# kepengxu/PGTFormer

Hardware: NVIDIA H100
Metric: clips_per_s (higher is better)
Workload: dtype bf16

## Files before the change

### include/pgt_b200.h

```cpp
#ifndef PGT_B200_H_
#define PGT_B200_H_

#include <stdint.h>

#ifdef __cplusplus
extern "C" {
#endif

typedef enum pgt_status {
  PGT_OK = 0,
  PGT_ERR_INVALID = -1,
  PGT_ERR_CUDA = -2,
  PGT_ERR_UNSUPPORTED = -3,
  PGT_ERR_DRIVER = -4
} pgt_status;

enum { PGT_BF16 = 0, PGT_F32 = 1 };
enum { PGT_ACT_NONE = 0, PGT_ACT_GELU = 1, PGT_ACT_SILU = 2, PGT_ACT_LRELU02 = 3, PGT_ACT_RELU = 4,
       PGT_ACT_SIGMOID = 5 };
enum { PGT_EPI_PLAIN = 0,
       PGT_EPI_SFT = 1 };
enum { PGT_OUT_NHWC = 0, PGT_OUT_NCHW = 1 };
enum { PGT_EPI_FLAG_RELU_AFTER_RESIDUAL = 1 };

typedef struct pgt_epilogue {
  const float* bias;
  int32_t act;
  int32_t mode;
  const void* residual;
  int32_t ldr;
  int32_t res_dtype;
  const void* aux;
  int32_t ldaux;
  float sft_w;
  void* out;
  int32_t ldo;
  int32_t out_dtype;
  int32_t out_layout;
  int32_t flags;
  float* gn_stats;
  const float* sft_wf;
} pgt_epilogue;

const char* pgt_strerror(int status);
const char* pgt_last_cuda_error(void);
int pgt_version(void);
int64_t pgt_launch_count(void);
void pgt_reset_launch_count(void);
void pgt_tmap_cache_stats(int64_t* hits, int64_t* misses);

enum { PGT_PROF_GEMM = 0, PGT_PROF_WINDOW_ATTN = 1, PGT_PROF_MHA = 2, PGT_PROF_ARGMAX = 3, PGT_PROF_ARGMIN = 4,
       PGT_PROF_NORM = 5, PGT_PROF_MOVE = 6, PGT_PROF_LAYERNORM = 7, PGT_PROF_CLASSES = 8 };
int pgt_profile_begin(void);
int pgt_profile_end(double* work, double* ms, int64_t* launches);
int pgt_profile_end_csv(const char* path, double* work, double* ms, int64_t* launches);

int pgt_linear_bf16(const void* A, int lda, const void* W, int ldw, int M, int N, int K,
                    const pgt_epilogue* ep, void* stream);

int pgt_conv_bf16(const void* x, int F, int Hin, int Win, int Cin, int ldx, const void* Wp, int ldw,
                  int Cout, int ksize, int stride, int pad_lo, const pgt_epilogue* ep, void* stream);

int pgt_conv_out_gn(const void* x, int F, int H, int W, int Cin, int ldx, const float* gn_ab, const void* Wp, int ldw,
                    int Cout, const float* bias, float* out, void* stream);
int pgt_conv_out_gn_act(const void* x, int F, int H, int W, int Cin, int ldx, const float* gn_ab, const void* Wp, int ldw,
                        int Cout, const float* bias, float* out, int silu, void* stream);

int pgt_conv_up2x_bf16(const void* x, int F, int Hin, int Win, int Cin, int ldx, const void* Wp4, int ldw,
                       int Cout, const pgt_epilogue* ep, void* stream);

int pgt_conv_rgb_bf16(const float* x_nchw, int F, int H, int W, int ksize, int stride, int pad, const float* mean3,
                      const float* std3, const void* Wp, int ldw, int Cout, const float* bias, int act, void* out,
                      int ldo, float* gn_stats, void* stream);

int64_t pgt_groupnorm_ws_floats(int F, int HW, int C);
int pgt_conv_tiles_per_frame(int Hin, int Win, int Cout, int ksize, int stride, int pad_lo);
int pgt_conv_tiles_exact(int Hin, int Win, int Cout, int ksize, int stride, int pad_lo);
int pgt_groupnorm_apply_stats(const void* x, int ldx, int F, int HW, int C, const float* gamma, const float* beta,
                              float eps, int apply_silu, void* y, int ldy, const float* stats, int chunks_per_frame,
                              float* ws, void* stream);

int pgt_groupnorm_ab(const void* x, int ldx, int F, int HW, int C, const float* gamma, const float* beta, float eps,
                     const float* stats, int chunks_per_frame, float* ws, float* ab, void* stream);
int pgt_groupnorm_silu(const void* x, int ldx, int F, int HW, int C, const float* gamma, const float* beta,
                       float eps, int apply_silu, void* y, int ldy, float* ws, void* stream);

int pgt_layernorm(const void* x, int ldx, int x_dtype, int T, int C, const float* gamma, const float* beta,
                  float eps, void* y, int ldy, const void* pos, int ldpos, void* y2, int ldy2, void* stream);

int pgt_ln_linear_bf16(const void* x, int ldx, int T, int C, const float* ln_g, const float* ln_b, float eps,
                       const void* W, int ldw, int N, const float* bias, void* out, int ldo, void* stream);

int pgt_swin_mlp_bf16(const void* x, int ldx, int T, int C, const float* ln_g, const float* ln_b, float eps,
                      const void* W1, const float* b1, const void* W2, const float* b2, void* out, int ldo,
                      float* gn_stats, void* stream);

int pgt_window_attention(const void* qkv, int ldqkv, int clips, int H, int W, int C, int heads, int shift,
                         const float* bias_tab, void* out, int ldo, void* stream);

int pgt_window_attention_tc(const void* qkv, int ldqkv, int clips, int H, int W, int C, int heads, int shift,
                            const void* tab, void* out, int ldo, void* stream);

int pgt_window3d_attention(const void* qkv, int ldqkv, const void* pad_qkv, int B, int D, int H, int W, int C, int heads,
                           int wd, int wh, int ww, int sd, int sh, int sw, const float* bias, void* out, int ldo,
                           void* stream);

int pgt_mha_fwd(const void* q, int ldq, const void* k, int ldk, const void* v, int ldv, int clips, int L,
                int heads, int d, void* out, int ldo, void* stream);

int pgt_argmax_gather(const float* logits, int T, int K, const float* codebook, int E, const int64_t* idx_in,
                      int64_t* idx, void* quant, int ldq, int quant_dtype, void* stream);
int pgt_l2_argmin(const float* z, int T, int E, const float* codebook, int K, int64_t* idx, float* quant,
                  void* stream);
int pgt_codebook_pack(const float* codebook, int K, int E, void* cb_bf16, float* cb_norm, void* stream);
int64_t pgt_l2_argmin_ws_ints(int T);
int pgt_l2_argmin_tc(const float* z, int T, int E, const float* codebook, const void* cb_bf16, const float* cb_norm,
                     int K, int64_t* idx, float* quant, int32_t* workspace, void* stream);
int64_t pgt_l2_argmin_split_ws_ints(int T, int splits);
int pgt_l2_argmin_tc_split(const float* z, int T, int E, const float* codebook, const void* cb_bf16, const float* cb_norm,
                           int K, int splits, int64_t* idx, float* quant, int32_t* workspace, void* stream);

int pgt_soft_codes(const float* z, int T, int E, const float* codebook, const float* cb_norm, int K, float temp,
                   float* out, int ldo, void* stream);
int pgt_sample_codes(const float* p, int T, int K, int ldp, const int64_t* seed, int64_t* idx, void* stream);

int pgt_rq_residual(const float* r_in, float* r_out, const int64_t* idx, int T, int E, const float* codebook_d,
                    float* agg, int first, void* stream);
int pgt_rq_embed(const int64_t* idx, long long ldi, long long ldd, int T, int d0, int d1, const float* codebooks,
                 long long cb_stride, int E, void* out, int ldo, int out_dtype, void* stream);

long long pgt_vq_stats_ws_doubles(int T, int E);
int pgt_vq_stats(const float* z, int T, int E, int HW, const float* codebook, int K, const int64_t* idx, float beta,
                 float* zq_nchw, void* zq_bf16, float* min_enc, float* scores, int* usage, int* hist, double* ws,
                 float* scalars, void* stream);

int pgt_adain(const void* q, int ldq, int q_dtype, const void* l, int ldl, int F, int HW, int C, float eps,
              void* y, int ldy, void* stream);
int pgt_adain_frames(const void* q, int ldq, int q_dtype, const void* l, int ldl, int F, int HW, int C, float eps,
                     const int32_t* flags, void* y, int ldy, void* stream);

int pgt_maxpool3x3s2(const void* x, int ldx, int F, int H, int W, int C, void* y, int ldy, void* stream);
int pgt_global_avgpool(const void* x, int ldx, int F, int HW, int C, void* y, int ldy, void* stream);
int pgt_channel_affine(const void* x, int ldx, int F, int HW, int C, const void* scale, int lds, int plus_one,
                       const void* addv, int ldv, const void* addm, int ldm, void* y, int ldy, void* stream);
int pgt_assemble_cond(const void* o0, int ld0, const void* o1, int ld1, const void* o2, int ld2, int F, int h8, int w8,
                      int h16, int w16, int ncls, void* cond, int ldc, void* stream);

int pgt_copy2d(const void* x, int ldx, int T, int C, void* y, int ldy, void* stream);
int pgt_regroup_frames(const void* x, int ldx, int clips, int P, int C, void* y, int ldy, int dir, void* stream);
int pgt_nchw_f32_to_nhwc_bf16(const float* x, int F, int C, int HW, const float* mean, const float* stdv, void* y,
                              int ldy, void* stream);
int pgt_nhwc_bf16_to_f32(const void* x, int ldx, int F, int HW, int C, float* y, int to_nchw, void* stream);

int pgt_u8hwc_to_f32nchw(const void* x_u8, int F, int H, int W, float* y, void* stream);
int pgt_u8hwc_resize_to_f32nchw(const void* x_u8, int F, int h, int w, const int32_t* sizes_dev, int H, int W, float* y,
                                void* stream);
int pgt_f32nchw_to_u8hwc(const float* x, int first, int step, int n, int H, int W, void* y_u8, void* stream);
int pgt_gather_frames(const void* x, long long frame_bytes, const int* idx_dev, int n, void* y, void* stream);
int pgt_scatter_frames(const void* x, long long frame_bytes, const int* idx_dev, int n, void* y, void* stream);

#ifdef __cplusplus
}
#endif
#endif
```

### pgtformer_b200/_lib.py

```python
import ctypes
import os
from ctypes import POINTER, Structure, c_char_p, c_float, c_int, c_int32, c_int64, c_void_p

HERE = os.path.dirname(os.path.abspath(__file__))
LIB_PATH = os.path.join(HERE, 'lib', 'libpgt_b200.so')

BF16, F32 = 0, 1
ACT_NONE, ACT_GELU, ACT_SILU, ACT_LRELU02, ACT_RELU, ACT_SIGMOID = 0, 1, 2, 3, 4, 5
EPI_PLAIN, EPI_SFT = 0, 1
OUT_NHWC, OUT_NCHW = 0, 1


class Epilogue(Structure):
    _fields_ = [('bias', c_void_p), ('act', c_int32), ('mode', c_int32), ('residual', c_void_p),
                ('ldr', c_int32), ('res_dtype', c_int32), ('aux', c_void_p), ('ldaux', c_int32),
                ('sft_w', c_float), ('out', c_void_p), ('ldo', c_int32), ('out_dtype', c_int32),
                ('out_layout', c_int32), ('flags', c_int32), ('gn_stats', c_void_p), ('sft_wf', c_void_p)]


SIGNATURES = {
    'pgt_strerror': (c_char_p, [c_int]),
    'pgt_last_cuda_error': (c_char_p, []),
    'pgt_version': (c_int, []),
    'pgt_launch_count': (c_int64, []),
    'pgt_reset_launch_count': (None, []),
    'pgt_tmap_cache_stats': (None, [c_void_p, c_void_p]),
    'pgt_profile_begin': (c_int, []),
    'pgt_profile_end': (c_int, [c_void_p, c_void_p, c_void_p]),
    'pgt_profile_end_csv': (c_int, [c_char_p, c_void_p, c_void_p, c_void_p]),
    'pgt_linear_bf16': (c_int, [c_void_p, c_int, c_void_p, c_int, c_int, c_int, c_int, POINTER(Epilogue), c_void_p]),
    'pgt_conv_bf16': (c_int, [c_void_p, c_int, c_int, c_int, c_int, c_int, c_void_p, c_int, c_int, c_int, c_int,
                              c_int, POINTER(Epilogue), c_void_p]),
    'pgt_conv_out_gn': (c_int, [c_void_p, c_int, c_int, c_int, c_int, c_int, c_void_p, c_void_p, c_int, c_int, c_void_p,
                                c_void_p, c_void_p]),
    'pgt_conv_out_gn_act': (c_int, [c_void_p, c_int, c_int, c_int, c_int, c_int, c_void_p, c_void_p, c_int, c_int,
                                    c_void_p, c_void_p, c_int, c_void_p]),
    'pgt_groupnorm_ab': (c_int, [c_void_p, c_int, c_int, c_int, c_int, c_void_p, c_void_p, c_float, c_void_p, c_int,
                                 c_void_p, c_void_p, c_void_p]),
    'pgt_conv_up2x_bf16': (c_int, [c_void_p, c_int, c_int, c_int, c_int, c_int, c_void_p, c_int, c_int,
                                   POINTER(Epilogue), c_void_p]),
    'pgt_conv_rgb_bf16': (c_int, [c_void_p, c_int, c_int, c_int, c_int, c_int, c_int, c_void_p, c_void_p, c_void_p, c_int,
                                  c_int, c_void_p, c_int, c_void_p, c_int, c_void_p, c_void_p]),
    'pgt_groupnorm_ws_floats': (c_int64, [c_int, c_int, c_int]),
    'pgt_conv_tiles_per_frame': (c_int, [c_int, c_int, c_int, c_int, c_int, c_int]),
    'pgt_conv_tiles_exact': (c_int, [c_int, c_int, c_int, c_int, c_int, c_int]),
    'pgt_groupnorm_apply_stats': (c_int, [c_void_p, c_int, c_int, c_int, c_int, c_void_p, c_void_p, c_float, c_int,
                                          c_void_p, c_int, c_void_p, c_int, c_void_p, c_void_p]),
    'pgt_groupnorm_silu': (c_int, [c_void_p, c_int, c_int, c_int, c_int, c_void_p, c_void_p, c_float, c_int,
                                   c_void_p, c_int, c_void_p, c_void_p]),
    'pgt_layernorm': (c_int, [c_void_p, c_int, c_int, c_int, c_int, c_void_p, c_void_p, c_float, c_void_p, c_int,
                              c_void_p, c_int, c_void_p, c_int, c_void_p]),
    'pgt_ln_linear_bf16': (c_int, [c_void_p, c_int, c_int, c_int, c_void_p, c_void_p, c_float, c_void_p, c_int, c_int,
                                   c_void_p, c_void_p, c_int, c_void_p]),
    'pgt_swin_mlp_bf16': (c_int, [c_void_p, c_int, c_int, c_int, c_void_p, c_void_p, c_float, c_void_p, c_void_p, c_void_p,
                                  c_void_p, c_void_p, c_int, c_void_p, c_void_p]),
    'pgt_window_attention': (c_int, [c_void_p, c_int, c_int, c_int, c_int, c_int, c_int, c_int, c_void_p, c_void_p,
                                     c_int, c_void_p]),
    'pgt_window_attention_tc': (c_int, [c_void_p, c_int, c_int, c_int, c_int, c_int, c_int, c_int, c_void_p, c_void_p,
                                        c_int, c_void_p]),
    'pgt_window3d_attention': (c_int, [c_void_p, c_int, c_void_p, c_int, c_int, c_int, c_int, c_int, c_int, c_int, c_int,
                                       c_int, c_int, c_int, c_int, c_void_p, c_void_p, c_int, c_void_p]),
    'pgt_mha_fwd': (c_int, [c_void_p, c_int, c_void_p, c_int, c_void_p, c_int, c_int, c_int, c_int, c_int, c_void_p,
                            c_int, c_void_p]),
    'pgt_argmax_gather': (c_int, [c_void_p, c_int, c_int, c_void_p, c_int, c_void_p, c_void_p, c_void_p, c_int,
                                  c_int, c_void_p]),
    'pgt_l2_argmin': (c_int, [c_void_p, c_int, c_int, c_void_p, c_int, c_void_p, c_void_p, c_void_p]),
    'pgt_codebook_pack': (c_int, [c_void_p, c_int, c_int, c_void_p, c_void_p, c_void_p]),
    'pgt_l2_argmin_ws_ints': (c_int64, [c_int]),
    'pgt_l2_argmin_tc': (c_int, [c_void_p, c_int, c_int, c_void_p, c_void_p, c_void_p, c_int, c_void_p, c_void_p,
                                 c_void_p, c_void_p]),
    'pgt_l2_argmin_split_ws_ints': (c_int64, [c_int, c_int]),
    'pgt_l2_argmin_tc_split': (c_int, [c_void_p, c_int, c_int, c_void_p, c_void_p, c_void_p, c_int, c_int, c_void_p,
                                       c_void_p, c_void_p, c_void_p]),
    'pgt_soft_codes': (c_int, [c_void_p, c_int, c_int, c_void_p, c_void_p, c_int, c_float, c_void_p, c_int, c_void_p]),
    'pgt_sample_codes': (c_int, [c_void_p, c_int, c_int, c_int, c_void_p, c_void_p, c_void_p]),
    'pgt_rq_residual': (c_int, [c_void_p, c_void_p, c_void_p, c_int, c_int, c_void_p, c_void_p, c_int, c_void_p]),
    'pgt_rq_embed': (c_int, [c_void_p, c_int64, c_int64, c_int, c_int, c_int, c_void_p, c_int64, c_int, c_void_p, c_int,
                             c_int, c_void_p]),
    'pgt_vq_stats_ws_doubles': (c_int64, [c_int, c_int]),
    'pgt_vq_stats': (c_int, [c_void_p, c_int, c_int, c_int, c_void_p, c_int, c_void_p, c_float, c_void_p, c_void_p,
                             c_void_p, c_void_p, c_void_p, c_void_p, c_void_p, c_void_p, c_void_p]),
    'pgt_adain': (c_int, [c_void_p, c_int, c_int, c_void_p, c_int, c_int, c_int, c_int, c_float, c_void_p, c_int,
                          c_void_p]),
    'pgt_adain_frames': (c_int, [c_void_p, c_int, c_int, c_void_p, c_int, c_int, c_int, c_int, c_float, c_void_p,
                                 c_void_p, c_int, c_void_p]),
    'pgt_maxpool3x3s2': (c_int, [c_void_p, c_int, c_int, c_int, c_int, c_int, c_void_p, c_int, c_void_p]),
    'pgt_global_avgpool': (c_int, [c_void_p, c_int, c_int, c_int, c_int, c_void_p, c_int, c_void_p]),
    'pgt_channel_affine': (c_int, [c_void_p, c_int, c_int, c_int, c_int, c_void_p, c_int, c_int, c_void_p, c_int,
                                   c_void_p, c_int, c_void_p, c_int, c_void_p]),
    'pgt_assemble_cond': (c_int, [c_void_p, c_int, c_void_p, c_int, c_void_p, c_int, c_int, c_int, c_int, c_int, c_int,
                                  c_int, c_void_p, c_int, c_void_p]),
    'pgt_u8hwc_to_f32nchw': (c_int, [c_void_p, c_int, c_int, c_int, c_void_p, c_void_p]),
    'pgt_u8hwc_resize_to_f32nchw': (c_int, [c_void_p, c_int, c_int, c_int, c_void_p, c_int, c_int, c_void_p,
                                            c_void_p]),
    'pgt_f32nchw_to_u8hwc': (c_int, [c_void_p, c_int, c_int, c_int, c_int, c_int, c_void_p, c_void_p]),
    'pgt_gather_frames': (c_int, [c_void_p, c_int64, c_void_p, c_int, c_void_p, c_void_p]),
    'pgt_scatter_frames': (c_int, [c_void_p, c_int64, c_void_p, c_int, c_void_p, c_void_p]),
    'pgt_copy2d': (c_int, [c_void_p, c_int, c_int, c_int, c_void_p, c_int, c_void_p]),
    'pgt_regroup_frames': (c_int, [c_void_p, c_int, c_int, c_int, c_int, c_void_p, c_int, c_int, c_void_p]),
    'pgt_nchw_f32_to_nhwc_bf16': (c_int, [c_void_p, c_int, c_int, c_int, c_void_p, c_void_p, c_void_p, c_int,
                                          c_void_p]),
    'pgt_nhwc_bf16_to_f32': (c_int, [c_void_p, c_int, c_int, c_int, c_int, c_void_p, c_int, c_void_p]),
}

_lib = None


def load(build_if_missing=True):
    global _lib
    if _lib is not None:
        return _lib
    if build_if_missing:
        from . import build as _build
        _build.build()
    if not os.path.exists(LIB_PATH):
        raise RuntimeError('libpgt_b200.so not built: run `python -m pgtformer_b200.build`')
    lib = ctypes.CDLL(LIB_PATH)
    for name, (res, args) in SIGNATURES.items():
        try:
            fn = getattr(lib, name)
        except AttributeError as e:
            raise RuntimeError('libpgt_b200.so does not export %s (stale build?)' % name) from e
        fn.restype = res
        fn.argtypes = args
    _lib = lib
    return lib


def check(status):
    if status != 0:
        lib = load()
        msg = lib.pgt_strerror(status).decode()
        if status == -2:
            msg += ': ' + lib.pgt_last_cuda_error().decode()
        raise RuntimeError('libpgt_b200: ' + msg)
```

### pgtformer_b200/csrc/gemm_tc.cu

```cuda
#include <cudaTypedefs.h>
#include <cstdio>
#include <cstdlib>

#include "common.cuh"
#include "tmap.cuh"
#include "ptx.cuh"
#include "epi_common.cuh"

namespace pgt {

constexpr int BM = 128;
constexpr int BK = 64;
constexpr int EPI_WARPS = 8;
constexpr int GEMM_THREADS = EPI_WARPS * 32 + 128;
constexpr int PRODUCER_WARP = EPI_WARPS;
constexpr int DMA_WARP = EPI_WARPS + 1;
constexpr int CONSUMER_REGS = 232;
constexpr int PRODUCER_REGS = 40;
static_assert(2 * 128 * CONSUMER_REGS + 128 * PRODUCER_REGS <= 65536, "register file");
constexpr int XCH_LD = 68;
constexpr int XCH_BYTES = BM * XCH_LD * 4;
constexpr int XCH_WG_LD = 36;
constexpr int XCH_WG_BYTES = BM * XCH_WG_LD * 4;
constexpr int EPI_BAR = 1;
constexpr int PP_XCH_BAR = 2;
constexpr int PP_MMA_BAR = 4;
constexpr int PP_EPI_BAR = 6;
constexpr int A_STAGE_BYTES = BM * BK * 2;
constexpr int PANEL_BYTES = BM * 128;
template <int BN>
constexpr int staging_slots() { return BN == 256 ? 2 : 4; }
constexpr int PREFETCH_TILES = 2;

enum { MODE_LINEAR = 0, MODE_CONV_S1 = 1, MODE_CONV_S2 = 2 };

struct GemmParams {
  int mode;
  int M, N, K;
  int num_kb, m_tiles, n_tiles;
  int F, H, W;
  int tw, th, tn, tiles_x, tiles_y;
  int cin_blocks, ksize, pad_lo, cin_ld;
  int pad_x, pad_y;
  long long o_sx, o_sy, o_sf;
  int b_resident;
  int fast_epi;
  int has_res_map;
  const float* bias;
  int act, epi_mode;
  float* gn_stats;
  int gn_cpg;
  int ntaps, tap_kw, tap_oy, tap_ox;
  int gn_tpf;
  int gn_fstride;
  int relu_after_res;
  const void* residual;
  int ldr, res_dtype;
  const void* aux;
  int ldaux;
  float sft_w;
  const float* sft_wf;
  void* out;
  int ldo, out_dtype, out_layout;
  double flops;
};

template <int BN>
struct GemmCfg {
  static constexpr int B_STAGE_BYTES = BN * BK * 2;
  static constexpr int STAGE_BYTES = A_STAGE_BYTES + B_STAGE_BYTES;
  static constexpr int SLOTS = staging_slots<BN>();
  static constexpr int STAGING_BYTES = SLOTS * PANEL_BYTES;
  static constexpr int BUDGET = 232448 - 1024  - STAGING_BYTES - XCH_BYTES - 256 ;
  static constexpr int STAGES = (BUDGET / STAGE_BYTES) > 6 ? 6 : (BUDGET / STAGE_BYTES);
  static constexpr int SMEM_BYTES = STAGES * STAGE_BYTES + STAGING_BYTES + XCH_BYTES + 256 + 1024;
  static_assert(SMEM_BYTES <= 232448, "gemm smem budget");
};

__device__ __forceinline__ void tile_mn(const GemmParams& p, int tile, int& m_blk, int& n_blk) {
  n_blk = tile % p.n_tiles;
  m_blk = tile / p.n_tiles;
}


__device__ __forceinline__ void decode_conv_tile(const GemmParams& p, int m_blk, int& n0, int& y0, int& x0) {
  const int tx = m_blk % p.tiles_x;
  const int t2 = m_blk / p.tiles_x;
  const int ty = t2 % p.tiles_y;
  const int tf = t2 / p.tiles_y;
  x0 = tx * p.tw;
  y0 = ty * p.th;
  n0 = tf * p.tn;
}

template <int N>
__device__ __forceinline__ void act_chunk(float (&f)[N], int act) {
  switch (act) {
    case PGT_ACT_GELU:
#pragma unroll
      for (int j = 0; j < N; ++j) f[j] = gelu_erf(f[j]);
      break;
    case PGT_ACT_SILU:
#pragma unroll
      for (int j = 0; j < N; ++j) f[j] = apply_act(f[j], PGT_ACT_SILU);
      break;
    case PGT_ACT_LRELU02:
#pragma unroll
      for (int j = 0; j < N; ++j) f[j] = fmaxf(f[j], 0.2f * f[j]);
      break;
    case PGT_ACT_RELU:
#pragma unroll
      for (int j = 0; j < N; ++j) f[j] = fmaxf(f[j], 0.f);
      break;
    case PGT_ACT_SIGMOID:
#pragma unroll
      for (int j = 0; j < N; ++j) f[j] = apply_act(f[j], PGT_ACT_SIGMOID);
      break;
    default: break;
  }
}

struct EpiCtx {
  uint8_t* staging;
  float* xch;
  uint64_t* res_bar;
  uint64_t* slot_ready;
};

__device__ __forceinline__ uint4 lds128(uint32_t a) {
  uint4 u;
  asm volatile("ld.shared.v4.b32 {%0, %1, %2, %3}, [%4];" : "=r"(u.x), "=r"(u.y), "=r"(u.z), "=r"(u.w) : "r"(a) : "memory");
  return u;
}
__device__ __forceinline__ void sts128(uint32_t a, const uint4& u) {
  asm volatile("st.shared.v4.b32 [%0], {%1, %2, %3, %4};" ::"r"(a), "r"(u.x), "r"(u.y), "r"(u.z), "r"(u.w) : "memory");
}

__device__ __forceinline__ float sft_weight(const GemmParams& p, int m_blk, int r) {
  if (p.sft_wf == nullptr) return p.sft_w;
  const int f = m_blk / (p.tiles_x * p.tiles_y) * p.tn + r / (p.tw * p.th);
  return __ldg(p.sft_wf + min(f, p.F - 1));
}

template <bool kSft>
__device__ __forceinline__ void epi_finish(const GemmParams& p, const uint32_t (&v)[32], const float* bias32, uint32_t srow,
                                           int r, int sub, int esize, bool has_res, float* gq, int gcol,
                                           const float4 (&pre)[8], bool use_pre, float sw = 0.f) {
  float f[32];
  if (use_pre) {
#pragma unroll
    for (int q = 0; q < 8; ++q) {
      f[4 * q + 0] = __uint_as_float(v[4 * q + 0]) + pre[q].x;
      f[4 * q + 1] = __uint_as_float(v[4 * q + 1]) + pre[q].y;
      f[4 * q + 2] = __uint_as_float(v[4 * q + 2]) + pre[q].z;
      f[4 * q + 3] = __uint_as_float(v[4 * q + 3]) + pre[q].w;
    }
  } else if (bias32 != nullptr) {
    const float4* b4 = reinterpret_cast<const float4*>(bias32);
#pragma unroll
    for (int q = 0; q < 8; ++q) {
      const float4 bb = __ldg(b4 + q);
      f[4 * q + 0] = __uint_as_float(v[4 * q + 0]) + bb.x;
      f[4 * q + 1] = __uint_as_float(v[4 * q + 1]) + bb.y;
      f[4 * q + 2] = __uint_as_float(v[4 * q + 2]) + bb.z;
      f[4 * q + 3] = __uint_as_float(v[4 * q + 3]) + bb.w;
    }
  } else {
#pragma unroll
    for (int i = 0; i < 32; ++i) f[i] = __uint_as_float(v[i]);
    if (p.bias != nullptr) {
#pragma unroll
      for (int i = 0; i < 32; ++i)
        if (gcol + i < p.N) f[i] += __ldg(p.bias + gcol + i);
    }
  }
  if (p.act != PGT_ACT_NONE && !p.relu_after_res) act_chunk(f, p.act);
  if (esize == 2) {
    uint32_t off[4];
#pragma unroll
    for (int q = 0; q < 4; ++q) off[q] = srow + ((((sub << 2) + q) ^ (r & 7)) << 4);
    if (has_res) {
      uint4 ur[4];
#pragma unroll
      for (int q = 0; q < 4; ++q) ur[q] = lds128(off[q]);
      if (kSft) {
        uint4 ux[4];
#pragma unroll
        for (int q = 0; q < 4; ++q) ux[q] = lds128(off[q] + PANEL_BYTES);
#pragma unroll
        for (int q = 0; q < 4; ++q) {
          const float2 a = unpack_bf16x2(ur[q].x), b = unpack_bf16x2(ur[q].y), c = unpack_bf16x2(ur[q].z), d = unpack_bf16x2(ur[q].w);
          const float rr[8] = {a.x, a.y, b.x, b.y, c.x, c.y, d.x, d.y};
          const float2 sa = unpack_bf16x2(ux[q].x), sb = unpack_bf16x2(ux[q].y), sc = unpack_bf16x2(ux[q].z), sd = unpack_bf16x2(ux[q].w);
          const float ss[8] = {sa.x, sa.y, sb.x, sb.y, sc.x, sc.y, sd.x, sd.y};
#pragma unroll
          for (int e = 0; e < 8; ++e) f[8 * q + e] = rr[e] + sw * (rr[e] * ss[e] + f[8 * q + e]);
        }
      } else {
#pragma unroll
        for (int q = 0; q < 4; ++q) {
          const float2 a = unpack_bf16x2(ur[q].x), b = unpack_bf16x2(ur[q].y), c = unpack_bf16x2(ur[q].z), d = unpack_bf16x2(ur[q].w);
          f[8 * q + 0] += a.x; f[8 * q + 1] += a.y; f[8 * q + 2] += b.x; f[8 * q + 3] += b.y;
          f[8 * q + 4] += c.x; f[8 * q + 5] += c.y; f[8 * q + 6] += d.x; f[8 * q + 7] += d.y;
        }
      }
    }
    if (p.relu_after_res) {
#pragma unroll
      for (int e = 0; e < 32; ++e) f[e] = fmaxf(f[e], 0.f);
    }
#pragma unroll
    for (int q = 0; q < 4; ++q) {
      uint4 o;
      o.x = pack_bf16x2(f[8 * q + 0], f[8 * q + 1]);
      o.y = pack_bf16x2(f[8 * q + 2], f[8 * q + 3]);
      o.z = pack_bf16x2(f[8 * q + 4], f[8 * q + 5]);
      o.w = pack_bf16x2(f[8 * q + 6], f[8 * q + 7]);
      sts128(off[q], o);
    }
    if (gq != nullptr) {
      const int lane = lane_id();
      switch (p.gn_cpg) {
        case 2: gn_chunk_stats<2>(f, gq, 0, lane); break;
        case 4: gn_chunk_stats<4>(f, gq, 0, lane); break;
        case 8: gn_chunk_stats<8>(f, gq, 0, lane); break;
        case 16: gn_chunk_stats<16>(f, gq, 0, lane); break;
        default: gn_chunk_stats<32>(f, gq, 0, lane); break;
      }
    }
  } else {
    if (has_res) {
      uint4 ur[8];
#pragma unroll
      for (int q = 0; q < 8; ++q) ur[q] = lds128(srow + ((q ^ (r & 7)) << 4));
#pragma unroll
      for (int q = 0; q < 8; ++q) {
        f[4 * q + 0] += __uint_as_float(ur[q].x); f[4 * q + 1] += __uint_as_float(ur[q].y);
        f[4 * q + 2] += __uint_as_float(ur[q].z); f[4 * q + 3] += __uint_as_float(ur[q].w);
      }
    }
    if (p.relu_after_res) {
#pragma unroll
      for (int e = 0; e < 32; ++e) f[e] = fmaxf(f[e], 0.f);
    }
#pragma unroll
    for (int q = 0; q < 8; ++q) {
      uint4 o;
      o.x = __float_as_uint(f[4 * q]); o.y = __float_as_uint(f[4 * q + 1]);
      o.z = __float_as_uint(f[4 * q + 2]); o.w = __float_as_uint(f[4 * q + 3]);
      sts128(srow + ((q ^ (r & 7)) << 4), o);
    }
  }
}

struct ItemCursor {
  int tile, pnl;
};

template <int BN>
struct ItemStream {
  const GemmParams& p;
  int num_tiles, PW, panels_total;
  __device__ ItemStream(const GemmParams& pp, int nt) : p(pp), num_tiles(nt) {
    PW = 128 / (pp.out_dtype == PGT_BF16 ? 2 : 4);
    panels_total = BN / PW;
  }
  __device__ int panels_in_tile(int t) const {
    int mb, nb;
    tile_mn(p, t, mb, nb);
    const int cb = nb * BN;
    const int n = (p.N - cb + PW - 1) / PW;
    return n > panels_total ? panels_total : n;
  }
  __device__ bool valid(const ItemCursor& c) const { return c.tile < num_tiles; }
  __device__ void next(ItemCursor& c) const {
    if (++c.pnl >= panels_in_tile(c.tile)) { c.tile += gridDim.x; c.pnl = 0; }
  }
};

template <int BN>
__device__ __forceinline__ void epilogue_dma_loop(const GemmParams& p, const EpiCtx& ctx, const CUtensorMap& tmO,
                                                  const CUtensorMap& tmR, const CUtensorMap& tmX, int lane, int num_tiles) {
  if (!p.fast_epi) return;
  const ItemStream<BN> is(p, num_tiles);
  constexpr int SLOTS = staging_slots<BN>();
  static_assert(SLOTS == 4 || SLOTS == 2, "ring positions are computed with shifts");
  const bool sft = SLOTS == 4 && p.epi_mode == PGT_EPI_SFT;
  const int S = sft ? 2 : 1;
  const int R = SLOTS / S;
  auto coords = [&](const ItemCursor& c, int& col, int& m_blk, int& n0, int& y0, int& x0) {
    int nb;
    tile_mn(p, c.tile, m_blk, nb);
    col = nb * BN + c.pnl * is.PW;
    n0 = y0 = x0 = 0;
    if (p.mode != MODE_LINEAR) decode_conv_tile(p, m_blk, n0, y0, x0);
  };
  auto prepare = [&](const ItemCursor& c, int pos) {
    uint64_t* bar = &ctx.res_bar[pos];
    if (!p.has_res_map) { mbar_arrive(bar); return; }
    int col, m_blk, n0, y0, x0;
    coords(c, col, m_blk, n0, y0, x0);
    uint8_t* dst = ctx.staging + pos * S * PANEL_BYTES;
    mbar_arrive_expect_tx(bar, S * PANEL_BYTES);
    if (p.mode == MODE_LINEAR) {
      tma_load_2d(dst, &tmR, bar, col, m_blk * BM);
      if (sft) tma_load_2d(dst + PANEL_BYTES, &tmX, bar, col, m_blk * BM);
    } else {
      tma_load_4d(dst, &tmR, bar, col, x0, y0, n0);
      if (sft) tma_load_4d(dst + PANEL_BYTES, &tmX, bar, col, x0, y0, n0);
    }
  };
  ItemCursor cp{(int)blockIdx.x, 0}, cs{(int)blockIdx.x, 0};
  if (lane == 0) {
    for (int i = 0; i < R && is.valid(cp); ++i) { prepare(cp, i); is.next(cp); }
  }
  __syncwarp();
  const int rshift = R == 4 ? 2 : 1;
  for (int k = 0; is.valid(cs); ++k, is.next(cs)) {
    const int pos = k & (R - 1);
    mbar_wait(&ctx.slot_ready[pos], (k >> rshift) & 1);
    if (lane == 0) {
      int col, m_blk, n0, y0, x0;
      coords(cs, col, m_blk, n0, y0, x0);
      const uint8_t* src = ctx.staging + pos * S * PANEL_BYTES;
      if (p.mode == MODE_LINEAR) tma_store_2d(&tmO, src, col, m_blk * BM);
      else tma_store_4d(&tmO, src, col, x0, y0, n0);
      bulk_commit();
      if (k >= 1 && is.valid(cp)) {
        bulk_wait_read<1>();
        prepare(cp, (k - 1) & (R - 1));
        is.next(cp);
      }
    }
    __syncwarp();
  }
  if (lane == 0) bulk_wait0();
}

struct DirectRow {
  bool valid;
  long long orow;
  int pn, py, px;
};

__device__ __forceinline__ DirectRow direct_row(const GemmParams& p, int m_blk, int r) {
  DirectRow d{false, 0, 0, 0, 0};
  if (p.mode == MODE_LINEAR) {
    d.orow = (long long)m_blk * BM + r;
    d.valid = d.orow < p.M;
  } else {
    int n0, y0, x0;
    decode_conv_tile(p, m_blk, n0, y0, x0);
    const int ix = r % p.tw;
    const int t2 = r / p.tw;
    const int iy = t2 % p.th;
    const int in = t2 / p.th;
    d.pn = n0 + in; d.py = y0 + iy; d.px = x0 + ix;
    d.valid = (d.pn < p.F) && (d.py < p.H) && (d.px < p.W);
    d.orow = ((long long)d.pn * p.H + d.py) * p.W + d.px;
  }
  return d;
}

template <bool kVec>
__device__ __forceinline__ void epi_direct16(const GemmParams& p, const DirectRow& d, const float* xs, int col0) {
  const int ncol = min(16, p.N - col0);
  const long long orow = d.orow;
  float f[16];
#pragma unroll
  for (int j = 0; j < 16; ++j) f[j] = xs[j] + ((p.bias != nullptr && j < ncol) ? __ldg(p.bias + col0 + j) : 0.f);
  if (p.act != PGT_ACT_NONE && !p.relu_after_res) act_chunk(f, p.act);
  if (p.residual != nullptr) {
    if (p.res_dtype == PGT_BF16) {
      const __nv_bfloat16* rp = reinterpret_cast<const __nv_bfloat16*>(p.residual) + orow * p.ldr + col0;
      float rr[16];
#pragma unroll
      for (int j = 0; j < 16; ++j) rr[j] = (j < ncol) ? __bfloat162float(rp[j]) : 0.f;
      if (p.epi_mode == PGT_EPI_SFT) {
        const __nv_bfloat16* ap = reinterpret_cast<const __nv_bfloat16*>(p.aux) + orow * p.ldaux + col0;
        const float sw = p.sft_wf != nullptr ? __ldg(p.sft_wf + d.pn) : p.sft_w;
#pragma unroll
        for (int j = 0; j < 16; ++j) {
          const float sc = (j < ncol) ? __bfloat162float(ap[j]) : 0.f;
          f[j] = rr[j] + sw * (rr[j] * sc + f[j]);
        }
      } else {
#pragma unroll
        for (int j = 0; j < 16; ++j) f[j] += rr[j];
      }
    } else {
      const float* rp = reinterpret_cast<const float*>(p.residual) + orow * p.ldr + col0;
#pragma unroll
      for (int j = 0; j < 16; ++j)
        if (j < ncol) f[j] += __ldg(rp + j);
    }
  }
  if (p.relu_after_res) act_chunk(f, PGT_ACT_RELU);
  if (p.out_layout == PGT_OUT_NCHW) {
    float* op = reinterpret_cast<float*>(p.out);
#pragma unroll
    for (int j = 0; j < 16; ++j)
      if (j < ncol) op[(((long long)d.pn * p.N + (col0 + j)) * p.H + d.py) * p.W + d.px] = f[j];
  } else if (p.out_dtype == PGT_BF16) {
    __nv_bfloat16* op = reinterpret_cast<__nv_bfloat16*>(p.out) + orow * p.ldo + col0;
    if (kVec && ncol == 16 && ((p.ldo & 7) == 0)) {
#pragma unroll
      for (int q = 0; q < 2; ++q) {
        uint4 u;
        u.x = pack_bf16x2(f[q * 8 + 0], f[q * 8 + 1]);
        u.y = pack_bf16x2(f[q * 8 + 2], f[q * 8 + 3]);
        u.z = pack_bf16x2(f[q * 8 + 4], f[q * 8 + 5]);
        u.w = pack_bf16x2(f[q * 8 + 6], f[q * 8 + 7]);
        reinterpret_cast<uint4*>(op)[q] = u;
      }
    } else {
#pragma unroll
      for (int j = 0; j < 16; ++j)
        if (j < ncol) op[j] = __float2bfloat16_rn(f[j]);
    }
  } else {
    float* op = reinterpret_cast<float*>(p.out) + orow * p.ldo + col0;
#pragma unroll
    for (int j = 0; j < 16; ++j)
      if (j < ncol) op[j] = f[j];
  }
}

__device__ __forceinline__ float* gn_stats_ptr(const GemmParams& p, int m_blk, int quad, int col0) {
  if (p.gn_stats == nullptr) return nullptr;
  const size_t chunk = p.gn_tpf > 0 ? (size_t)(m_blk / p.gn_tpf) * p.gn_fstride + (m_blk % p.gn_tpf) * 4 + quad
                                    : (size_t)m_blk * 4 + quad;
  return p.gn_stats + (chunk * 32 + col0 / p.gn_cpg) * 2;
}

template <int BN, bool kVec>
__device__ __forceinline__ void epilogue_tile(const GemmParams& p, const EpiCtx& ctx, int warp, int lane, int tile, int& k,
                                              const float (&acc)[BN / 2]) {
  const int quad = warp & 3;
  const int half = warp >> 2;
  const int r = quad * 32 + lane;
  const int esize = (p.out_dtype == PGT_BF16) ? 2 : 4;
  const ItemStream<BN> is(p, 0);
  const int PW = is.PW;
  const int nsub = PW / 32;
  constexpr int SLOTS = staging_slots<BN>();
  constexpr int SLOT_SHIFT = SLOTS == 4 ? 2 : 1;
  const bool sft = SLOTS == 4 && p.epi_mode == PGT_EPI_SFT;
  const bool bias_vec = kVec && p.bias != nullptr && (p.N % 32) == 0;
  const float* xrow = ctx.xch + r * XCH_LD;

  int n_blk, m_blk;
  tile_mn(p, tile, m_blk, n_blk);
  const int col_base = n_blk * BN;
  const int npan = p.fast_epi ? is.panels_in_tile(tile) : 0;
  const uint32_t stg = smem_u32(ctx.staging) + r * 128;
  auto gn_ptr = [&](int col0) -> float* { return gn_stats_ptr(p, m_blk, quad, col0); };
  const DirectRow drow = p.fast_epi ? DirectRow{false, 0, 0, 0, 0} : direct_row(p, m_blk, r);

  static_for<0, BN / 64>([&](auto gc) {
    constexpr int g = decltype(gc)::value;
    if (col_base + g * 64 >= p.N) return;
    named_bar_sync(EPI_BAR, EPI_WARPS * 32);
    acc_to_smem<g * 64, 64>(acc, ctx.xch + half * 64 * XCH_LD, XCH_LD, quad, lane);
    named_bar_sync(EPI_BAR, EPI_WARPS * 32);

    if (p.fast_epi) {
      if (sft) {
        const int pnl = g;
        if (pnl < npan) {
          const int pos = k & 1;
          mbar_wait_spin(&ctx.res_bar[pos], (k >> 1) & 1);
          const int col0 = col_base + pnl * PW + half * 32;
          uint32_t v[32];
          smem_row_32(xrow + half * 32, v);
          float4 nb[8];
          epi_finish<true>(p, v, bias_vec ? p.bias + col0 : nullptr, stg + pos * 2 * PANEL_BYTES, r, half, esize, true,
                           gn_ptr(col0), col0, nb, false, sft_weight(p, m_blk, r));
          fence_proxy_async();
          mbar_arrive(&ctx.slot_ready[pos]);
          ++k;
        }
      } else {
        for (int pp = 0; pp < 64 / PW; ++pp) {
          const int pnl = g * (64 / PW) + pp;
          if (pnl >= npan) break;
          const int pos = k & (SLOTS - 1);
          const bool mine = (nsub == 2) || ((pnl & 1) == half);
          const int sb = (nsub == 2) ? half : 0;
          const int col0 = col_base + pnl * PW + sb * 32;
          float4 b[8];
          const bool pre = BN < 256 && bias_vec;
          if (mine && pre) {
            const float4* gb = reinterpret_cast<const float4*>(p.bias + col0);
#pragma unroll
            for (int q = 0; q < 8; ++q) b[q] = __ldg(gb + q);
          }
          mbar_wait_spin(&ctx.res_bar[pos], (k >> SLOT_SHIFT) & 1);
          if (mine) {
            uint32_t v[32];
            smem_row_32(xrow + pnl * PW + sb * 32 - g * 64, v);
            epi_finish<false>(p, v, bias_vec && !pre ? p.bias + col0 : nullptr, stg + pos * PANEL_BYTES, r, sb, esize,
                              p.has_res_map != 0, gn_ptr(col0), col0, b, pre);
          }
          fence_proxy_async();
          mbar_arrive(&ctx.slot_ready[pos]);
          ++k;
        }
      }
    } else {
      const int c0 = g * 64 + half * 32;
      if (drow.valid) {
#pragma unroll 1
        for (int sc16 = 0; sc16 < 32; sc16 += 16) {
          const int col0 = col_base + c0 + sc16;
          if (col0 >= p.N) break;
          epi_direct16<kVec>(p, drow, xrow + half * 32 + sc16, col0);
        }
      }
      __syncwarp();
    }
  });
}

template <int BN, bool kVec>
__device__ __forceinline__ void epilogue_tile_wg(const GemmParams& p, const EpiCtx& ctx, int wq, int bar, int tile, int k,
                                                 const float (&acc)[2][BN / 2]) {
  const int lane = lane_id();
  const int r = wq * 32 + lane;
  const int esize = (p.out_dtype == PGT_BF16) ? 2 : 4;
  const ItemStream<BN> is(p, 0);
  const int nsub = is.PW / 32;
  constexpr int SLOTS = staging_slots<BN>();
  constexpr int SLOT_SHIFT = SLOTS == 4 ? 2 : 1;
  const bool sft = SLOTS == 4 && p.epi_mode == PGT_EPI_SFT;
  const bool bias_vec = kVec && p.bias != nullptr && (p.N % 32) == 0;
  const float* xrow = ctx.xch + r * XCH_WG_LD;

  int n_blk, m_blk;
  tile_mn(p, tile, m_blk, n_blk);
  const int col_base = n_blk * BN;
  const int npan = p.fast_epi ? is.panels_in_tile(tile) : 0;
  const uint32_t stg = smem_u32(ctx.staging) + r * 128;
  const DirectRow drow = p.fast_epi ? DirectRow{false, 0, 0, 0, 0} : direct_row(p, m_blk, r);

  static_for<0, BN / 32>([&](auto cc) {
    constexpr int c = decltype(cc)::value;
    const int pnl = c / nsub, sub = c - pnl * nsub;
    if (p.fast_epi && pnl >= npan) return;
    const int col0 = col_base + c * 32;
    if (col0 < p.N) {
      named_bar_sync(bar, 128);
      acc_to_smem<c * 32, 32>(acc[0], ctx.xch, XCH_WG_LD, wq, lane);
      acc_to_smem<c * 32, 32>(acc[1], ctx.xch + 64 * XCH_WG_LD, XCH_WG_LD, wq, lane);
      named_bar_sync(bar, 128);
    }
    if (p.fast_epi) {
      const int item = k + pnl;
      const int pos = sft ? (item & 1) : (item & (SLOTS - 1));
      if (sub == 0) mbar_wait_spin(&ctx.res_bar[pos], sft ? ((item >> 1) & 1) : ((item >> SLOT_SHIFT) & 1));
      if (col0 < p.N) {
        uint32_t v[32];
        smem_row_32(xrow, v);
        float4 nb[8];
        if (sft)
          epi_finish<true>(p, v, bias_vec ? p.bias + col0 : nullptr, stg + pos * 2 * PANEL_BYTES, r, sub, esize, true,
                           gn_stats_ptr(p, m_blk, wq, col0), col0, nb, false, sft_weight(p, m_blk, r));
        else
          epi_finish<false>(p, v, bias_vec ? p.bias + col0 : nullptr, stg + pos * PANEL_BYTES, r, sub, esize,
                            p.has_res_map != 0, gn_stats_ptr(p, m_blk, wq, col0), col0, nb, false);
      }
      if (sub == nsub - 1) {
        fence_proxy_async();
        mbar_arrive(&ctx.slot_ready[pos]);
      }
    } else if (col0 < p.N) {
      if (drow.valid) {
#pragma unroll 1
        for (int sc16 = 0; sc16 < 32; sc16 += 16) {
          if (col0 + sc16 >= p.N) break;
          epi_direct16<kVec>(p, drow, xrow + sc16, col0 + sc16);
        }
      }
      __syncwarp();
    }
  });
}

__device__ __forceinline__ void release_stage(uint64_t* bar, int lane) {
  __syncwarp();
  if (lane == 0) mbar_arrive(bar);
}

template <int BN, bool kVec>
__global__ void __launch_bounds__(GEMM_THREADS, 1)
gemm_tc_kernel(const __grid_constant__ CUtensorMap tmA, const __grid_constant__ CUtensorMap tmB,
               const __grid_constant__ CUtensorMap tmO, const __grid_constant__ CUtensorMap tmR,
               const __grid_constant__ CUtensorMap tmX, const GemmParams p) {
  using Cfg = GemmCfg<BN>;
  constexpr int STAGES = Cfg::STAGES;
  extern __shared__ uint8_t smem_raw[];
  uint8_t* smem = reinterpret_cast<uint8_t*>((reinterpret_cast<uintptr_t>(smem_raw) + 1023) & ~uintptr_t(1023));
  uint8_t* smem_a = smem;
  uint8_t* smem_b = smem + STAGES * A_STAGE_BYTES;
  uint8_t* staging = smem + STAGES * Cfg::STAGE_BYTES;
  float* xch = reinterpret_cast<float*>(staging + Cfg::STAGING_BYTES);
  uint64_t* bars = reinterpret_cast<uint64_t*>(staging + Cfg::STAGING_BYTES + XCH_BYTES);
  uint64_t* full_bar = bars;
  uint64_t* empty_bar = bars + STAGES;
  uint64_t* res_bar = bars + 2 * STAGES;
  uint64_t* slot_ready = res_bar + Cfg::SLOTS;

  const int warp = threadIdx.x >> 5;
  const int lane = threadIdx.x & 31;
  const int num_tiles = p.m_tiles * p.n_tiles;

  if (warp == PRODUCER_WARP && lane == 0) {
    tma_prefetch_desc(&tmA);
    tma_prefetch_desc(&tmB);
    if (p.fast_epi) tma_prefetch_desc(&tmO);
    if (p.has_res_map) tma_prefetch_desc(&tmR);
    if (p.fast_epi && p.epi_mode == PGT_EPI_SFT) tma_prefetch_desc(&tmX);
    for (int i = 0; i < STAGES; ++i) {
      mbar_init(&full_bar[i], 1);
      mbar_init(&empty_bar[i], EPI_WARPS);
    }
    for (int i = 0; i < Cfg::SLOTS; ++i) {
      mbar_init(&res_bar[i], 1);
      mbar_init(&slot_ready[i], EPI_WARPS * 32);
    }
    fence_barrier_init();
  }
  __syncthreads();

  if (warp >= EPI_WARPS) {
    setmaxnreg_dec<PRODUCER_REGS>();
    if (warp == PRODUCER_WARP) {
      int stage = 0;
      uint32_t phase = 0;
      for (int tile = blockIdx.x; tile < num_tiles; tile += gridDim.x) {
        int n_blk, m_blk;
        tile_mn(p, tile, m_blk, n_blk);
        int n0 = 0, y0 = 0, x0 = 0;
        if (p.mode != MODE_LINEAR) decode_conv_tile(p, m_blk, n0, y0, x0);
        for (int kb = 0; kb < p.num_kb; ++kb) {
          mbar_wait(&empty_bar[stage], phase ^ 1);
          if (elect_one()) {
            void* dst_a = smem_a + stage * A_STAGE_BYTES;
            void* dst_b = smem_b + stage * Cfg::B_STAGE_BYTES;
            int cb = 0, ax = 0, ay = 0, a5 = 0;
            if (p.mode != MODE_LINEAR) {
              const int tap = kb / p.cin_blocks;
              cb = kb - tap * p.cin_blocks;
              const int dy = tap / p.ksize;
              const int dx = tap - dy * p.ksize;
              if (p.mode == MODE_CONV_S1) {
                ax = x0 + dx - p.pad_x; ay = y0 + dy - p.pad_y;
              } else {
                const int oy = dy - p.pad_lo, ox = dx - p.pad_lo;
                const int qy = (oy < 0) ? -((1 - oy) >> 1) : (oy >> 1);
                const int qx = (ox < 0) ? -((1 - ox) >> 1) : (ox >> 1);
                const int py = oy - 2 * qy, px = ox - 2 * qx;
                cb = px * p.cin_ld + cb * BK;
                ax = x0 + qx; ay = y0 + qy; a5 = py;
              }
            }
            mbar_arrive_expect_tx(&full_bar[stage], Cfg::STAGE_BYTES);
            if (p.mode == MODE_LINEAR) tma_load_2d(dst_a, &tmA, &full_bar[stage], kb * BK, m_blk * BM);
            else if (p.mode == MODE_CONV_S1) tma_load_4d(dst_a, &tmA, &full_bar[stage], cb * BK, ax, ay, n0);
            else tma_load_5d(dst_a, &tmA, &full_bar[stage], cb, ax, a5, ay, n0);
            tma_load_2d(dst_b, &tmB, &full_bar[stage], kb * BK, n_blk * BN);
          }
          __syncwarp();
          if (++stage == STAGES) { stage = 0; phase ^= 1; }
        }
      }
      for (int i = 0; i < STAGES; ++i) {
        mbar_wait(&empty_bar[stage], phase ^ 1);
        if (++stage == STAGES) { stage = 0; phase ^= 1; }
      }
    } else if (warp == DMA_WARP) {
      const EpiCtx ctx{staging, xch, res_bar, slot_ready};
      epilogue_dma_loop<BN>(p, ctx, tmO, tmR, tmX, lane, num_tiles);
    }
  } else {
    setmaxnreg_inc<CONSUMER_REGS>();
    const EpiCtx ctx{staging, xch, res_bar, slot_ready};
    const int wg = warp >> 2;
    const uint32_t a_rows = smem_u32(smem_a) + wg * 64 * 128;
    const uint32_t b_base = smem_u32(smem_b);
    int stage = 0;
    uint32_t phase = 0;
    int k = 0;
    for (int tile = blockIdx.x; tile < num_tiles; tile += gridDim.x) {
      float acc[BN / 2];
      int prev = -1;
      for (int kb = 0; kb < p.num_kb; ++kb) {
        mbar_wait_spin(&full_bar[stage], phase);
        const uint64_t da = wgmma_desc_k_sw128(a_rows + stage * A_STAGE_BYTES);
        const uint64_t db = wgmma_desc_k_sw128(b_base + stage * Cfg::B_STAGE_BYTES);
        wgmma_fence();
#pragma unroll
        for (int kk = 0; kk < BK / 16; ++kk)
          wgmma_bf16<BN>(acc, da + 2 * kk, db + 2 * kk, (kb | kk) != 0 ? 1u : 0u);
        wgmma_commit();
        wgmma_wait<1>();
        if (prev >= 0) release_stage(&empty_bar[prev], lane);
        prev = stage;
        if (++stage == STAGES) { stage = 0; phase ^= 1; }
      }
      wgmma_wait<0>();
      release_stage(&empty_bar[prev], lane);
      epilogue_tile<BN, kVec>(p, ctx, warp, lane, tile, k, acc);
    }
  }
}


constexpr int HALO_TW = 8, HALO_TH = 16;
constexpr int HALO_PITCH = (HALO_TW + 2) * 128;
constexpr int HALO_A_BYTES = (HALO_TH + 2) * HALO_PITCH;
constexpr int HALO_A_STRIDE = ((HALO_A_BYTES + 1023) / 1024) * 1024;

template <int BN>
struct HaloCfg {
  static constexpr int B_BYTES = BN * 128;
  static constexpr int A_STAGES = 2;
  static constexpr int B_STAGES = (BN == 64) ? 9 : 4;
  static constexpr int SLOTS = staging_slots<BN>();
  static constexpr int STAGING_BYTES = SLOTS * PANEL_BYTES;
  static constexpr int XCH = 2 * XCH_WG_BYTES;
  static constexpr int SMEM_BYTES = A_STAGES * HALO_A_STRIDE + B_STAGES * B_BYTES + STAGING_BYTES + XCH + 512 + 1024;
  static_assert(SMEM_BYTES <= 232448, "halo conv smem budget");
};

template <int S>
__device__ __forceinline__ void ring_skip(int& s, uint32_t& ph, int n) {
  const int t = s + n;
  ph ^= (uint32_t)(t / S) & 1u;
  s = t % S;
}

template <int BN, bool kVec>
__global__ void __launch_bounds__(GEMM_THREADS, 1)
conv_halo_kernel(const __grid_constant__ CUtensorMap tmA, const __grid_constant__ CUtensorMap tmB,
                 const __grid_constant__ CUtensorMap tmO, const __grid_constant__ CUtensorMap tmR,
                 const __grid_constant__ CUtensorMap tmX, const GemmParams p) {
  using Cfg = HaloCfg<BN>;
  constexpr int AS = Cfg::A_STAGES, BS = Cfg::B_STAGES;
  constexpr int RELEASERS = 4;
  extern __shared__ uint8_t smem_raw[];
  uint8_t* smem = reinterpret_cast<uint8_t*>((reinterpret_cast<uintptr_t>(smem_raw) + 1023) & ~uintptr_t(1023));
  uint8_t* smem_a = smem;
  uint8_t* smem_b = smem + AS * HALO_A_STRIDE;
  uint8_t* staging = smem_b + BS * Cfg::B_BYTES;
  float* xch = reinterpret_cast<float*>(staging + Cfg::STAGING_BYTES);
  uint64_t* bars = reinterpret_cast<uint64_t*>(staging + Cfg::STAGING_BYTES + Cfg::XCH);
  uint64_t* a_full = bars;
  uint64_t* a_empty = bars + AS;
  uint64_t* b_full = bars + 2 * AS;
  uint64_t* b_empty = bars + 2 * AS + BS;
  uint64_t* res_bar = bars + 2 * AS + 2 * BS;
  uint64_t* slot_ready = res_bar + Cfg::SLOTS;

  const int warp = threadIdx.x >> 5;
  const int lane = threadIdx.x & 31;
  const int num_tiles = p.m_tiles * p.n_tiles;
  const int cin_pad = p.cin_blocks * BK;

  if (warp == PRODUCER_WARP && lane == 0) {
    tma_prefetch_desc(&tmA);
    tma_prefetch_desc(&tmB);
    if (p.fast_epi) tma_prefetch_desc(&tmO);
    if (p.has_res_map) tma_prefetch_desc(&tmR);
    if (p.fast_epi && p.epi_mode == PGT_EPI_SFT) tma_prefetch_desc(&tmX);
    for (int i = 0; i < AS; ++i) { mbar_init(&a_full[i], 1); mbar_init(&a_empty[i], RELEASERS); }
    for (int i = 0; i < BS; ++i) { mbar_init(&b_full[i], 1); mbar_init(&b_empty[i], RELEASERS); }
    for (int i = 0; i < Cfg::SLOTS; ++i) {
      mbar_init(&res_bar[i], 1);
      mbar_init(&slot_ready[i], RELEASERS * 32);
    }
    fence_barrier_init();
  }
  __syncthreads();

  if (warp >= EPI_WARPS) {
    setmaxnreg_dec<PRODUCER_REGS>();
    if (warp == PRODUCER_WARP) {
      int as = 0, bs = 0;
      uint32_t aph = 0, bph = 0;
      for (int tile = blockIdx.x; tile < num_tiles; tile += gridDim.x) {
        const int n_blk = tile % p.n_tiles;
        const int m_blk = tile / p.n_tiles;
        int n0, y0, x0;
        decode_conv_tile(p, m_blk, n0, y0, x0);
        {
          const int pt = tile + PREFETCH_TILES * (int)gridDim.x;
          if (BN == 64 && pt < num_tiles && elect_one()) {
            int pn0, py0, px0;
            decode_conv_tile(p, pt / p.n_tiles, pn0, py0, px0);
            for (int cb = 0; cb < p.cin_blocks; ++cb) tma_prefetch_4d(&tmA, cb * BK, px0 - 1, py0 - 1, pn0);
            if (p.has_res_map) {
              const int c0 = (pt % p.n_tiles) * BN;
              const int rw = p.out_dtype == PGT_BF16 ? 64 : 32;
              for (int c = 0; c < BN && c0 + c < p.N; c += rw) {
                tma_prefetch_4d(&tmR, c0 + c, px0, py0, pn0);
                if (p.epi_mode == PGT_EPI_SFT) tma_prefetch_4d(&tmX, c0 + c, px0, py0, pn0);
              }
            }
          }
          __syncwarp();
        }
        for (int cb = 0; cb < p.cin_blocks; ++cb) {
          mbar_wait(&a_empty[as], aph ^ 1);
          if (elect_one()) {
            mbar_arrive_expect_tx(&a_full[as], HALO_A_BYTES);
            tma_load_4d(smem_a + as * HALO_A_STRIDE, &tmA, &a_full[as], cb * BK, x0 - 1, y0 - 1, n0);
          }
          __syncwarp();
          if (++as == AS) { as = 0; aph ^= 1; }
          if (p.b_resident && tile != (int)blockIdx.x) continue;
          for (int t = 0; t < p.ntaps; ++t) {
            mbar_wait(&b_empty[bs], bph ^ 1);
            if (elect_one()) {
              mbar_arrive_expect_tx(&b_full[bs], Cfg::B_BYTES);
              tma_load_2d(smem_b + bs * Cfg::B_BYTES, &tmB, &b_full[bs], t * cin_pad + cb * BK, n_blk * BN);
            }
            __syncwarp();
            if (++bs == BS) { bs = 0; bph ^= 1; }
          }
        }
      }
      for (int i = 0; i < AS; ++i) {
        mbar_wait(&a_empty[as], aph ^ 1);
        if (++as == AS) { as = 0; aph ^= 1; }
      }
    } else if (warp == DMA_WARP) {
      const EpiCtx ctx{staging, xch, res_bar, slot_ready};
      epilogue_dma_loop<BN>(p, ctx, tmO, tmR, tmX, lane, num_tiles);
    }
  } else {
    setmaxnreg_inc<CONSUMER_REGS>();
    const int wg = warp >> 2;
    const EpiCtx ctx{staging, xch + wg * (XCH_WG_BYTES / 4), res_bar, slot_ready};
    const uint32_t a_base = smem_u32(smem_a);
    const uint32_t b_base = smem_u32(smem_b);
    constexpr uint64_t ROW_BLOCK = 8 * HALO_PITCH / 16;
    const ItemStream<BN> is(p, num_tiles);
    const int b_per_tile = p.b_resident ? 0 : p.ntaps * p.cin_blocks;
    int as = 0, bs = 0;
    uint32_t aph = 0, bph = 0;
    int k = 0;
    bool first = true;
    for (int tile = blockIdx.x, j = 0; tile < num_tiles; tile += gridDim.x, ++j) {
      const bool has_next = tile + (int)gridDim.x < num_tiles;
      const int items = p.fast_epi ? is.panels_in_tile(tile) : 0;
      if ((j & 1) != wg) {
        ring_skip<AS>(as, aph, p.cin_blocks);
        ring_skip<BS>(bs, bph, b_per_tile);
        k += items;
        continue;
      }
      if (j > 0) named_bar_sync(PP_MMA_BAR + wg, 256);
      float acc[2][BN / 2];
      for (int cb = 0; cb < p.cin_blocks; ++cb) {
        const bool hand_over = has_next && cb == p.cin_blocks - 1;
        mbar_wait_spin(&a_full[as], aph);
        const uint64_t da0 = wgmma_desc_k_sw128(a_base + as * HALO_A_STRIDE, HALO_PITCH);
        auto tap_desc = [&](int t) -> uint64_t {
          const int dy = t / p.tap_kw, dx = t - dy * p.tap_kw;
          return da0 + (uint64_t)(((dy + p.tap_oy) * (HALO_TW + 2) + dx + p.tap_ox) * 8);
        };
        if (p.b_resident && first) {
          for (int t = 0; t < p.ntaps * p.cin_blocks; ++t) mbar_wait_spin(&b_full[t], 0);
          first = false;
        }
        int prev = -1;
        for (int t = 0; t < p.ntaps; ++t) {
          int bst = cb * p.ntaps + t;
          if (!p.b_resident) {
            mbar_wait_spin(&b_full[bs], bph);
            bst = bs;
          }
          const uint64_t da = tap_desc(t);
          const uint64_t db = wgmma_desc_k_sw128(b_base + bst * Cfg::B_BYTES);
          wgmma_fence();
#pragma unroll
          for (int kk = 0; kk < BK / 16; ++kk) {
            const uint32_t accum = (cb | t | kk) != 0 ? 1u : 0u;
            wgmma_bf16<BN>(acc[0], da + 2 * kk, db + 2 * kk, accum);
            wgmma_bf16<BN>(acc[1], da + ROW_BLOCK + 2 * kk, db + 2 * kk, accum);
          }
          wgmma_commit();
          if (hand_over && t == p.ntaps - 1) named_bar_arrive(PP_MMA_BAR + (wg ^ 1), 256);
          wgmma_wait<1>();
          if (!p.b_resident) {
            if (prev >= 0) release_stage(&b_empty[prev], lane);
            prev = bs;
            if (++bs == BS) { bs = 0; bph ^= 1; }
          }
        }
        wgmma_wait<0>();
        if (!p.b_resident) release_stage(&b_empty[prev], lane);
        release_stage(&a_empty[as], lane);
        if (++as == AS) { as = 0; aph ^= 1; }
      }
      if (j > 0) named_bar_sync(PP_EPI_BAR + wg, 256);
      epilogue_tile_wg<BN, kVec>(p, ctx, warp & 3, PP_XCH_BAR + wg, tile, k, acc);
      if (has_next) named_bar_arrive(PP_EPI_BAR + (wg ^ 1), 256);
      k += items;
    }
  }
}

static int encode_map(CUtensorMap* map, const void* base, int rank, const uint64_t* dims, const uint64_t* strides_bytes,
                      const uint32_t* box, int dtype = PGT_BF16) {
  return tmap_encode(map, base, rank, dims, strides_bytes, box, dtype);
}

static inline bool aligned16(const void* p) { return (reinterpret_cast<uintptr_t>(p) & 15) == 0; }

static int encode_out_map(CUtensorMap* map, const GemmParams& p, const void* base, int ld, int dtype) {
  const int esize = dtype == PGT_BF16 ? 2 : 4;
  const uint32_t pw = 128 / esize;
  if (p.mode == MODE_LINEAR) {
    uint64_t dims[2] = {(uint64_t)p.N, (uint64_t)p.M};
    uint64_t str[1] = {(uint64_t)ld * esize};
    uint32_t box[2] = {pw, BM};
    return encode_map(map, base, 2, dims, str, box, dtype);
  }
  uint64_t dims[4] = {(uint64_t)p.N, (uint64_t)p.W, (uint64_t)p.H, (uint64_t)p.F};
  uint64_t str[3] = {(uint64_t)ld * esize, (uint64_t)p.W * ld * esize, (uint64_t)p.H * p.W * ld * esize};
  if (p.o_sx != 0 && base == p.out) {
    str[0] = (uint64_t)p.o_sx * esize; str[1] = (uint64_t)p.o_sy * esize; str[2] = (uint64_t)p.o_sf * esize;
  }
  uint32_t box[4] = {pw, (uint32_t)p.tw, (uint32_t)p.th, (uint32_t)p.tn};
  return encode_map(map, base, 4, dims, str, box, dtype);
}

static int setup_epilogue_maps(GemmParams& p, const CUtensorMap& placeholder, CUtensorMap& tmO, CUtensorMap& tmR,
                               CUtensorMap& tmX) {
  const int esize = p.out_dtype == PGT_BF16 ? 2 : 4;
  p.fast_epi = (p.out_layout == PGT_OUT_NHWC && aligned16(p.out) && ((long long)p.ldo * esize) % 16 == 0) ? 1 : 0;
  if (p.epi_mode == PGT_EPI_SFT &&
      !(p.out_dtype == PGT_BF16 && aligned16(p.aux) && ((long long)p.ldaux * 2) % 16 == 0 && p.o_sx == 0))
    p.fast_epi = 0;
  p.has_res_map = 0;
  if (p.fast_epi && p.residual != nullptr) {
    if (p.res_dtype == p.out_dtype && aligned16(p.residual) && ((long long)p.ldr * esize) % 16 == 0) p.has_res_map = 1;
    else p.fast_epi = 0;
  }
  if (p.gn_stats != nullptr) {
    const int cpg = p.N / 32;
    const bool ok = p.fast_epi && p.out_dtype == PGT_BF16 && (p.N % 32) == 0 &&
                    (cpg == 2 || cpg == 4 || cpg == 8 || cpg == 16 || cpg == 32) &&
                    (p.mode == MODE_LINEAR || p.tn == 1);
    if (!ok) return PGT_ERR_UNSUPPORTED;
    p.gn_cpg = cpg;
  }
  tmO = placeholder;
  tmR = placeholder;
  tmX = placeholder;
  if (p.fast_epi) {
    int rc = encode_out_map(&tmO, p, p.out, p.ldo, p.out_dtype);
    if (rc != PGT_OK) return rc;
    if (p.has_res_map) {
      rc = encode_out_map(&tmR, p, p.residual, p.ldr, p.res_dtype);
      if (rc != PGT_OK) return rc;
    }
    if (p.epi_mode == PGT_EPI_SFT) {
      if (!p.has_res_map) { p.fast_epi = 0; return p.gn_stats ? PGT_ERR_UNSUPPORTED : PGT_OK; }
      rc = encode_out_map(&tmX, p, p.aux, p.ldaux, PGT_BF16);
      if (rc != PGT_OK) return rc;
    }
  }
  return PGT_OK;
}

static bool vector_views(const GemmParams& p) {
  if (p.bias != nullptr && (p.N % 32) == 0 && !aligned16(p.bias)) return false;
  if (!p.fast_epi && p.out_layout == PGT_OUT_NHWC && p.out_dtype == PGT_BF16 && (p.ldo % 8) == 0 && !aligned16(p.out))
    return false;
  return true;
}

template <int BN, bool kVec>
static cudaError_t gemm_smem_once() {
  static PerDeviceOnce once;
  return once.run([] {
    return cudaFuncSetAttribute(gemm_tc_kernel<BN, kVec>, cudaFuncAttributeMaxDynamicSharedMemorySize, GemmCfg<BN>::SMEM_BYTES);
  });
}

template <int BN, bool kVec>
static cudaError_t halo_smem_once() {
  static PerDeviceOnce once;
  return once.run([] {
    return cudaFuncSetAttribute(conv_halo_kernel<BN, kVec>, cudaFuncAttributeMaxDynamicSharedMemorySize, HaloCfg<BN>::SMEM_BYTES);
  });
}

static int encode_weight_map(CUtensorMap* tmB, const void* W, int ldw, int K, int N, int BN) {
  uint64_t dims[2] = {(uint64_t)K, (uint64_t)N};
  uint64_t str[1] = {(uint64_t)ldw * 2};
  uint32_t box[2] = {BK, (uint32_t)BN};
  return encode_map(tmB, W, 2, dims, str, box);
}

template <int BN>
static int launch_gemm(const CUtensorMap& tmA, const void* W, int ldw, GemmParams& p, cudaStream_t stream) {
  using Cfg = GemmCfg<BN>;
  static_assert(Cfg::STAGES >= 3, "pipeline too shallow");
  CUtensorMap tmB, tmO, tmR, tmX;
  int rc = encode_weight_map(&tmB, W, ldw, p.K, p.N, BN);
  if (rc != PGT_OK) return rc;
  rc = setup_epilogue_maps(p, tmA, tmO, tmR, tmX);
  if (rc != PGT_OK) return rc;
  p.n_tiles = ceil_div(p.N, BN);
  const bool vec = vector_views(p);
  PGT_CUDA_OK((vec ? gemm_smem_once<BN, true>() : gemm_smem_once<BN, false>()));
  const int tiles = p.m_tiles * p.n_tiles;
  const int grid = tiles < num_sms() ? tiles : num_sms();
  {
    char desc[96];
    if (prof_enabled()) {
      if (p.mode == MODE_LINEAR) snprintf(desc, sizeof(desc), "linear M%d N%d K%d BN%d e%d", p.M, p.N, p.K, BN, p.fast_epi);
      else snprintf(desc, sizeof(desc), "conv%d s%d F%d H%d W%d K%d N%d BN%d t%dx%dx%d e%d", p.ksize, p.mode, p.F, p.H, p.W, p.K, p.N, BN, p.tn, p.th, p.tw, p.fast_epi);
    }
    ProfScope ps(PGT_PROF_GEMM, p.flops, stream, desc);
    if (vec) gemm_tc_kernel<BN, true><<<grid, GEMM_THREADS, Cfg::SMEM_BYTES, stream>>>(tmA, tmB, tmO, tmR, tmX, p);
    else gemm_tc_kernel<BN, false><<<grid, GEMM_THREADS, Cfg::SMEM_BYTES, stream>>>(tmA, tmB, tmO, tmR, tmX, p);
  }
  PGT_LAUNCH_OK();
  return PGT_OK;
}

template <int BN>
static int launch_halo(const CUtensorMap& tmA, const void* W, int ldw, GemmParams& p, cudaStream_t stream) {
  using Cfg = HaloCfg<BN>;
  CUtensorMap tmB, tmO, tmR, tmX;
  int rc = encode_weight_map(&tmB, W, ldw, p.K, p.N, BN);
  if (rc != PGT_OK) return rc;
  rc = setup_epilogue_maps(p, tmA, tmO, tmR, tmX);
  if (rc != PGT_OK) return rc;
  p.n_tiles = ceil_div(p.N, BN);
  p.b_resident = (p.ntaps * p.cin_blocks <= Cfg::B_STAGES && p.n_tiles == 1) ? 1 : 0;
  const bool vec = vector_views(p);
  PGT_CUDA_OK((vec ? halo_smem_once<BN, true>() : halo_smem_once<BN, false>()));
  const int tiles = p.m_tiles * p.n_tiles;
  const int grid = tiles < num_sms() ? tiles : num_sms();
  {
    char desc[96];
    if (prof_enabled())
      snprintf(desc, sizeof(desc), "halo3 F%d H%d W%d K%d N%d BN%d e%d r%d", p.F, p.H, p.W, p.K, p.N, BN, p.fast_epi,
               p.b_resident);
    ProfScope ps(PGT_PROF_GEMM, p.flops, stream, desc);
    if (vec) conv_halo_kernel<BN, true><<<grid, GEMM_THREADS, Cfg::SMEM_BYTES, stream>>>(tmA, tmB, tmO, tmR, tmX, p);
    else conv_halo_kernel<BN, false><<<grid, GEMM_THREADS, Cfg::SMEM_BYTES, stream>>>(tmA, tmB, tmO, tmR, tmX, p);
  }
  PGT_LAUNCH_OK();
  return PGT_OK;
}

static bool wide_tiles(const GemmParams& p) {
  if (p.N <= 128 || p.num_kb < 8 || p.epi_mode == PGT_EPI_SFT) return false;
  if (ceil_div(p.N, 256) * 256 > ceil_div(p.N, 128) * 128) return false;
  return p.m_tiles * ceil_div(p.N, 256) >= num_sms();
}

static int dispatch_gemm(const CUtensorMap& tmA, const void* W, int ldw, GemmParams& p, cudaStream_t stream) {
  if (p.N <= 64) return launch_gemm<64>(tmA, W, ldw, p, stream);
  if (wide_tiles(p)) return launch_gemm<256>(tmA, W, ldw, p, stream);
  return launch_gemm<128>(tmA, W, ldw, p, stream);
}

static int fill_epilogue(GemmParams& p, const pgt_epilogue* ep) {
  if (ep == nullptr || ep->out == nullptr) return PGT_ERR_INVALID;
  p.bias = ep->bias;
  p.act = ep->act;
  p.epi_mode = ep->mode;
  p.residual = ep->residual;
  p.ldr = ep->ldr;
  p.res_dtype = ep->res_dtype;
  p.aux = ep->aux;
  p.ldaux = ep->ldaux;
  p.sft_w = ep->sft_w;
  p.sft_wf = ep->mode == PGT_EPI_SFT ? ep->sft_wf : nullptr;
  p.out = ep->out;
  p.ldo = ep->ldo;
  p.out_dtype = ep->out_dtype;
  p.out_layout = ep->out_layout;
  p.relu_after_res = (ep->flags & PGT_EPI_FLAG_RELU_AFTER_RESIDUAL) ? 1 : 0;
  p.gn_stats = ep->gn_stats;
  p.gn_cpg = 0;
  if (p.relu_after_res && (p.act != PGT_ACT_RELU || p.epi_mode != PGT_EPI_PLAIN)) return PGT_ERR_INVALID;
  if (p.epi_mode == PGT_EPI_SFT && (p.residual == nullptr || p.aux == nullptr || p.res_dtype != PGT_BF16))
    return PGT_ERR_INVALID;
  if (p.sft_wf != nullptr && p.mode == MODE_LINEAR) return PGT_ERR_INVALID;
  if (p.out_layout == PGT_OUT_NCHW && (p.out_dtype != PGT_F32 || p.mode == MODE_LINEAR)) return PGT_ERR_INVALID;
  return PGT_OK;
}

}

using namespace pgt;

extern "C" int pgt_linear_bf16(const void* A, int lda, const void* W, int ldw, int M, int N, int K,
                               const pgt_epilogue* ep, void* stream) {
  PGT_CHECK_ARG(A && W && M > 0 && N > 0 && K > 0);
  PGT_CHECK_ARG((lda % 8) == 0 && (ldw % 8) == 0 && aligned16(A) && aligned16(W));
  GemmParams p{};
  p.mode = MODE_LINEAR;
  p.M = M; p.N = N; p.K = K;
  p.num_kb = ceil_div(K, BK);
  p.m_tiles = ceil_div(M, BM);
  p.flops = 2.0 * M * (double)N * K;
  int rc = fill_epilogue(p, ep);
  if (rc != PGT_OK) return rc;
  CUtensorMap tmA;
  uint64_t dims[2] = {(uint64_t)K, (uint64_t)M};
  uint64_t str[1] = {(uint64_t)lda * 2};
  uint32_t box[2] = {BK, BM};
  rc = encode_map(&tmA, A, 2, dims, str, box);
  if (rc != PGT_OK) return rc;
  return dispatch_gemm(tmA, W, ldw, p, static_cast<cudaStream_t>(stream));
}

static bool conv_tile_shape(int Hin, int Win, int Cout, int ksize, int stride, int pad_lo, int& tw, int& th) {
  static const bool no_halo = getenv("PGT_NO_HALO") != nullptr;
  const int H = Hin / stride, W = Win / stride;
  const bool halo = !no_halo && stride == 1 && ((ksize == 3 && pad_lo == 1) || ksize == 2) && Cout <= 128 && Hin >= HALO_TH &&
                    Win >= HALO_TW;
  tw = 1; th = 1;
  if (halo) { tw = HALO_TW; th = HALO_TH; }
  else {
    while (tw * 2 <= W && tw * 2 <= BM) tw *= 2;
    while (th * 2 <= H && tw * th * 2 <= BM) th *= 2;
  }
  return halo;
}

static int conv_impl(const void* x, int F, int Hin, int Win, int Cin, int ldx, const void* Wp, int ldw, int Cout,
                     int ksize, int stride, int pad_y, int pad_x, int up_phase, const pgt_epilogue* ep, void* stream) {
  const int pad_lo = pad_y;
  PGT_CHECK_ARG(x && Wp && F > 0 && Hin > 0 && Win > 0 && Cin > 0 && Cout > 0);
  PGT_CHECK_ARG((ksize >= 1 && ksize <= 3) && (stride == 1 || stride == 2) && pad_y >= 0 && pad_y <= 1 && pad_x >= 0 && pad_x <= 1);
  PGT_CHECK_ARG(stride == 1 || (ksize != 2 && pad_x == pad_y));
  PGT_CHECK_ARG((ldx % 8) == 0 && (ldw % 8) == 0 && aligned16(x) && aligned16(Wp) && ldx >= Cin);
  const int cin_pad = ceil_div(Cin, BK) * BK;
  PGT_CHECK_ARG(ldw >= ksize * ksize * cin_pad);
  GemmParams p{};
  p.N = Cout;
  p.ksize = ksize;
  p.pad_lo = pad_lo;
  p.pad_x = pad_x; p.pad_y = pad_y;
  p.cin_blocks = cin_pad / BK;
  p.K = ksize * ksize * cin_pad;
  p.num_kb = ksize * ksize * p.cin_blocks;
  p.F = F;
  CUtensorMap tmA;
  int rc;
  if (stride == 1) {
    p.mode = MODE_CONV_S1;
    p.H = Hin; p.W = Win;
  } else {
    if ((Hin & 1) || (Win & 1) || (Cin % BK) != 0 || ldx < Cin) return PGT_ERR_UNSUPPORTED;
    p.mode = MODE_CONV_S2;
    p.H = Hin / 2; p.W = Win / 2;
    p.cin_ld = ldx;
  }
  rc = fill_epilogue(p, ep);
  if (rc != PGT_OK) return rc;
  if (up_phase >= 0) {
    if (stride != 1 || p.out_layout != PGT_OUT_NHWC || p.epi_mode != PGT_EPI_PLAIN || p.residual != nullptr)
      return PGT_ERR_UNSUPPORTED;
    const int py = up_phase >> 1, px = up_phase & 1;
    const int esz = p.out_dtype == PGT_BF16 ? 2 : 4;
    const long long Wo = 2LL * Win;
    p.out = static_cast<char*>(p.out) + ((long long)py * Wo + px) * p.ldo * esz;
    p.o_sx = 2LL * p.ldo; p.o_sy = 2LL * Wo * p.ldo; p.o_sf = 4LL * Hin * Win * p.ldo;
  }
  int tw, th;
  const bool halo = conv_tile_shape(Hin, Win, Cout, ksize, stride, pad_y, tw, th);
  p.ntaps = ksize * ksize; p.tap_kw = ksize;
  p.tap_oy = up_phase >= 0 ? (up_phase >> 1) : 0;
  p.tap_ox = up_phase >= 0 ? (up_phase & 1) : 0;
  const int tn = BM / (tw * th);
  p.tw = tw; p.th = th; p.tn = tn;
  p.tiles_x = ceil_div(p.W, tw);
  p.tiles_y = ceil_div(p.H, th);
  p.m_tiles = p.tiles_x * p.tiles_y * ceil_div(F, tn);
  p.M = F * p.H * p.W;
  p.flops = 2.0 * p.M * (double)Cout * (ksize * ksize * Cin);
  if (up_phase >= 0 && p.gn_stats != nullptr) {
    if (tn != 1) return PGT_ERR_UNSUPPORTED;
    const int tpf = p.tiles_x * p.tiles_y;
    p.gn_tpf = tpf;
    p.gn_fstride = 16 * tpf;
    p.gn_stats += (size_t)up_phase * tpf * 4 * 64;
  }
  if (p.mode == MODE_CONV_S1) {
    uint64_t dims[4] = {(uint64_t)Cin, (uint64_t)Win, (uint64_t)Hin, (uint64_t)F};
    uint64_t str[3] = {(uint64_t)ldx * 2, (uint64_t)Win * ldx * 2, (uint64_t)Hin * Win * ldx * 2};
    uint32_t box[4] = {BK, (uint32_t)(halo ? tw + 2 : tw), (uint32_t)(halo ? th + 2 : th), (uint32_t)tn};
    rc = encode_map(&tmA, x, 4, dims, str, box);
    if (rc == PGT_OK && halo) {
      cudaStream_t st = static_cast<cudaStream_t>(stream);
      return Cout <= 64 ? launch_halo<64>(tmA, Wp, ldw, p, st) : launch_halo<128>(tmA, Wp, ldw, p, st);
    }
  } else {
    uint64_t dims[5] = {(uint64_t)2 * ldx, (uint64_t)Win / 2, 2, (uint64_t)Hin / 2, (uint64_t)F};
    uint64_t str[4] = {(uint64_t)2 * ldx * 2, (uint64_t)Win * ldx * 2, (uint64_t)2 * Win * ldx * 2,
                       (uint64_t)Hin * Win * ldx * 2};
    uint32_t box[5] = {BK, (uint32_t)tw, 1, (uint32_t)th, (uint32_t)tn};
    rc = encode_map(&tmA, x, 5, dims, str, box);
  }
  if (rc != PGT_OK) return rc;
  if (up_phase >= 0) {
    const int esz = p.out_dtype == PGT_BF16 ? 2 : 4;
    if (!aligned16(p.out) || ((long long)p.ldo * esz) % 16 != 0) return PGT_ERR_UNSUPPORTED;
  }
  return dispatch_gemm(tmA, Wp, ldw, p, static_cast<cudaStream_t>(stream));
}

extern "C" int pgt_conv_tiles_per_frame(int Hin, int Win, int Cout, int ksize, int stride, int pad_lo) {
  int tw, th;
  conv_tile_shape(Hin, Win, Cout, ksize, stride, pad_lo, tw, th);
  if (tw * th != BM) return 0;
  return ceil_div(Win / stride, tw) * ceil_div(Hin / stride, th);
}

extern "C" int pgt_conv_tiles_exact(int Hin, int Win, int Cout, int ksize, int stride, int pad_lo) {
  int tw, th;
  conv_tile_shape(Hin, Win, Cout, ksize, stride, pad_lo, tw, th);
  if (tw * th != BM) return 0;
  const int H = Hin / stride, W = Win / stride;
  return (W % tw == 0 && H % th == 0) ? (W / tw) * (H / th) : 0;
}

extern "C" int pgt_conv_bf16(const void* x, int F, int Hin, int Win, int Cin, int ldx, const void* Wp, int ldw,
                             int Cout, int ksize, int stride, int pad_lo, const pgt_epilogue* ep, void* stream) {
  PGT_CHECK_ARG(ksize == 1 || ksize == 3);
  return conv_impl(x, F, Hin, Win, Cin, ldx, Wp, ldw, Cout, ksize, stride, pad_lo, pad_lo, -1, ep, stream);
}

extern "C" int pgt_conv_up2x_bf16(const void* x, int F, int Hin, int Win, int Cin, int ldx, const void* Wp4, int ldw,
                                  int Cout, const pgt_epilogue* ep, void* stream) {
  PGT_CHECK_ARG(Wp4 != nullptr && ldw > 0);
  const int cin_pad = ceil_div(Cin, BK) * BK;
  PGT_CHECK_ARG(ldw >= 4 * cin_pad);
  for (int ph = 0; ph < 4; ++ph) {
    const int py = ph >> 1, px = ph & 1;
    const void* w = static_cast<const char*>(Wp4) + (size_t)ph * Cout * ldw * 2;
    int rc = conv_impl(x, F, Hin, Win, Cin, ldx, w, ldw, Cout, 2, 1, 1 - py, 1 - px, ph, ep, stream);
    if (rc != PGT_OK) return rc;
  }
  return PGT_OK;
}
```

### pgtformer_b200/engine.py

```python
import torch
import torch.nn.functional as F

from . import ops
from .spec import Arch
from .swin3d import pack_blocks

BF = torch.bfloat16


def _on_device(fn):
    import functools

    @functools.wraps(fn)
    def wrapper(self, *a, **k):
        with torch.cuda.device(self.dev):
            return fn(self, *a, **k)
    return wrapper


def _fusing(feats, wgt):
    return feats is not None and (torch.is_tensor(wgt) or wgt > 0)


def _pack_conv(w):
    co, ci, kh, kw = w.shape
    cp = (ci + 63) // 64 * 64
    wp = torch.zeros(co, kh * kw, cp, dtype=torch.float32, device=w.device)
    wp[:, :, :ci] = w.permute(0, 2, 3, 1).reshape(co, kh * kw, ci)
    return wp.reshape(co, kh * kw * cp).to(BF).contiguous()


def fold_layernorm_affine(weight, bias, gamma, beta):
    wf = weight.float()
    return wf * gamma.float()[None, :], (bias.float() + wf @ beta.float()).contiguous()


def _pack_up2x(w):
    co, ci, _, _ = w.shape
    cp = (ci + 63) // 64 * 64
    sets = {0: ((0,), (1, 2)), 1: ((0, 1), (2,))}
    out = torch.zeros(4, co, 4, cp, dtype=torch.float32, device=w.device)
    for py in range(2):
        for px in range(2):
            for ty in range(2):
                for tx in range(2):
                    acc = torch.zeros(co, ci, dtype=torch.float32, device=w.device)
                    for dy in sets[py][ty]:
                        for dx in sets[px][tx]:
                            acc += w[:, :, dy, dx]
                    out[py * 2 + px, :, ty * 2 + tx, :ci] = acc
    return out.reshape(4, co, 4 * cp).to(BF).contiguous()


def _pack_lin(w):
    w = w.reshape(w.shape[0], -1)
    n, k = w.shape
    kp = (k + 7) // 8 * 8
    if kp != k:
        w = F.pad(w, (0, kp - k))
    return w.to(BF).contiguous()


def _pack_rgb(w):
    return _pack_lin(w.permute(0, 2, 3, 1).reshape(w.shape[0], -1))


class Engine:
    arch_class = Arch

    def __init__(self, network_g, state_dict, device):
        ops.L.load()
        self.arch = self.arch_class(network_g)
        self.dev = torch.device(device)
        if self.dev.type != 'cuda':
            raise RuntimeError('pgtformer_b200 has no CPU path: the engine needs a CUDA (sm_90a) device')
        self.w = {}
        with torch.cuda.device(self.dev):
            self._sd = {k: v.detach().to(self.dev) for k, v in state_dict.items()}
            self._repack()

    def _f32(self, name):
        return self._sd[name].float().contiguous()

    def _repack(self):
        a, sd, w = self.arch, self._sd, self.w
        names = [n for n in sd if not n.startswith(a.packed_apart)]
        for name in names:
            t = sd[name]
            if name == a.stem:
                w[name] = _pack_rgb(t.float())
            elif name in a.upsample_convs:
                w[name] = _pack_up2x(t.float())
            elif name.endswith('.weight') and t.dim() == 4:
                w[name] = _pack_conv(t.float()) if t.shape[2] == 3 else _pack_lin(t.float())
            elif name.endswith('.weight') and t.dim() == 2 and name not in a.codebooks:
                w[name] = _pack_lin(t.float())
            elif t.dtype.is_floating_point and t.dim() == 1:
                w[name] = t.float().contiguous()
        w['codebook'] = self._f32(a.codebooks[0])
        if self.depth > 1:
            cbs = [self._f32(k) for k in a.codebooks[:1 if a.shared_codebook else self.depth]]
            w['codebooks'] = torch.zeros(len(cbs), max(c.shape[0] for c in cbs), cbs[0].shape[1], dtype=torch.float32,
                                         device=self.dev)
            for d, cb in enumerate(cbs):
                w['codebooks'][d, :cb.shape[0]] = cb
        for name in names:
            if name.endswith('.attn.relative_position_bias_table'):
                p = name[:-len('.relative_position_bias_table')]
                heads = sd[name].shape[1]
                idx = sd[p + '.relative_position_index'].view(-1).long()
                w[p + '.bias_tab'] = sd[name].float()[idx].view(48, 48, heads).permute(2, 0, 1).contiguous()
                w[p + '.tab16'] = ops.window_tables(w[p + '.bias_tab'])
                w[p + '.qkv.weight'] = _pack_lin(torch.cat([sd[p + '.q.weight'], sd[p + '.kv.weight']], 0).float())
                w[p + '.qkv.bias'] = torch.cat([sd[p + '.q.bias'], sd[p + '.kv.bias']], 0).float().contiguous()
                blk = p[:-len('.attn')]
                if sd[p + '.q.weight'].shape[1] == 256 and (blk + '.norm1.weight') in sd:
                    wf = torch.cat([sd[p + '.q.weight'], sd[p + '.kv.weight']], 0)
                    wg, bg = fold_layernorm_affine(wf, w[p + '.qkv.bias'], sd[blk + '.norm1.weight'], sd[blk + '.norm1.bias'])
                    w[p + '.qkv_ln.weight'], w[p + '.qkv_ln.bias'] = _pack_lin(wg), bg
        for name in names:
            if name.endswith('.proj_out.weight'):
                p = name[:-len('.proj_out.weight')]
                w[p + '.qkv.weight'] = _pack_lin(torch.cat([sd[p + '.%s.weight' % n] for n in 'qkv'], 0).float())
                w[p + '.qkv.bias'] = torch.cat([sd[p + '.%s.bias' % n] for n in 'qkv'], 0).float().contiguous()
        for name in names:
            if name.endswith('.self_attn.in_proj_weight'):
                p = name[:-len('.in_proj_weight')]
                wi, bi = sd[name].float(), sd[p + '.in_proj_bias'].float()
                E = wi.shape[1]
                w[p + '.qk.weight'], w[p + '.qk.bias'] = _pack_lin(wi[:2 * E]), bi[:2 * E].contiguous()
                w[p + '.v.weight'], w[p + '.v.bias'] = _pack_lin(wi[2 * E:]), bi[2 * E:].contiguous()
        for name in names:
            if name.endswith('.mlp.fc1.weight') and sd[name].shape == (256, 256):
                blk = name[:-len('.mlp.fc1.weight')]
                if (blk + '.norm2.weight') not in sd:
                    continue
                wg, bg = fold_layernorm_affine(sd[name], sd[blk + '.mlp.fc1.bias'], sd[blk + '.norm2.weight'],
                                               sd[blk + '.norm2.bias'])
                w[blk + '.mlp.fc1_ln.weight'], w[blk + '.mlp.fc1_ln.bias'] = _pack_lin(wg), bg
        self.swin = {}
        for prefix in a.packed_apart:
            if prefix == 'conditionnet.':
                self._repack_parsing()
            else:
                self.swin[prefix[:-1]] = pack_blocks(lambda k, p=prefix: sd.get(p + k), a.stages_atten)
        if 'position_emb' in sd:
            w['position_emb'] = sd['position_emb'].to(BF).contiguous()

    @property
    def depth(self):
        return int(self.arch.code_shape[2])

    def _new(self, *shape, dtype=BF):
        return torch.empty(*shape, dtype=dtype, device=self.dev)

    def _stats_tiles(self, H, W, cout, ksize, stride, pad_lo):
        return ops.conv_tiles_exact(H, W, cout, ksize, stride, pad_lo)

    def _gn_stats(self, out, chunks_per_frame, into=None):
        if chunks_per_frame <= 0 or not ops.gn_stats_supported(out.shape[-1]) or not out.is_contiguous():
            return None
        stats = self._new(out.shape[0] * chunks_per_frame * 64, dtype=torch.float32) if into is None else into
        assert stats.numel() == out.shape[0] * chunks_per_frame * 64
        out._pgt_gn = (stats, chunks_per_frame)
        return stats

    def _gn(self, x, p, silu=True):
        gn = getattr(x, '_pgt_gn', None)
        if gn is not None:
            return ops.groupnorm_apply_stats(x, self.w[p + '.weight'], self.w[p + '.bias'], self._new(*x.shape), gn[0], gn[1],
                                             silu=silu)
        return ops.groupnorm_silu(x, self.w[p + '.weight'], self.w[p + '.bias'], self._new(*x.shape), silu=silu)

    def _conv3(self, x, p, cout, out=None, gn_out=False, gn=None, gn_silu=True, gn_into=None, **kw):
        Fr, H, W, _ = x.shape
        stride = kw.get('stride', 1)
        if gn is not None:
            x = self._gn(x, gn, silu=gn_silu)
        if out is None:
            out = self._new(Fr, H // stride, W // stride, cout)
        stats = None
        if gn_out:
            stats = self._gn_stats(out, 4 * self._stats_tiles(H, W, cout, kw.get('ksize', 3), stride, kw.get('pad_lo', 1)),
                                   gn_into)
        return ops.conv(x, self.w[p + '.weight'], cout, out, bias=self.w.get(p + '.bias'), gn_stats=stats, **kw)

    def _lin(self, x, p, n, out=None, out_dtype=BF, gn_out=False, **kw):
        if out is None:
            out = self._new(*x.shape[:-1], n, dtype=out_dtype)
        stats = None
        if gn_out and out.dim() == 4 and out.dtype == BF and (out.shape[1] * out.shape[2]) % 128 == 0:
            stats = self._gn_stats(out, out.shape[1] * out.shape[2] // 32)
        return ops.linear(x, self.w[p + '.weight'], out, bias=self.w.get(p + '.bias'), N=n, gn_stats=stats, **kw)

    def td_resblock(self, x, p, cout, gn_next=False, out=None, shortcut='nin_shortcut'):
        h = self._conv3(x, p + '.conv1', cout, gn=p + '.norm1', gn_out=True)
        sc = self._lin(x, p + '.' + shortcut, cout) if (p + '.' + shortcut + '.weight') in self.w else x
        return self._conv3(h, p + '.conv2', cout, gn=p + '.norm2', residual=sc, gn_out=gn_next, out=out)

    def swin_block(self, x, p, heads, shift, gn_next=False, out=None):
        Fr, H, W, C = x.shape
        w = self.w
        if C == 256:
            qkv = ops.ln_linear(x, None, None, w[p + '.attn.qkv_ln.weight'], w[p + '.attn.qkv_ln.bias'],
                                self._new(Fr, H, W, 3 * C))
        else:
            y = ops.layernorm(x, w[p + '.norm1.weight'], w[p + '.norm1.bias'], self._new(Fr, H, W, C))
            qkv = self._lin(y, p + '.attn.qkv', 3 * C)
        a = self._new(Fr, H, W, C)
        if ops.window_attention_tc(qkv, Fr // 3, H, W, C, heads, shift, w[p + '.attn.tab16'], a) is None:
            ops.window_attention(qkv, Fr // 3, H, W, C, heads, shift, w[p + '.attn.bias_tab'], a)
        x = self._lin(a, p + '.attn.proj', C, residual=x)
        if C == 256:
            out = self._new(Fr, H, W, C) if out is None else out
            stats = self._gn_stats(out, H * W // 32) if gn_next and (H * W) % 128 == 0 else None
            return ops.swin_mlp(x, None, None, w[p + '.mlp.fc1_ln.weight'], w[p + '.mlp.fc1_ln.bias'],
                                w[p + '.mlp.fc2.weight'], w[p + '.mlp.fc2.bias'], out, gn_stats=stats)
        y = ops.layernorm(x, w[p + '.norm2.weight'], w[p + '.norm2.bias'], self._new(Fr, H, W, C))
        m = self._lin(y, p + '.mlp.fc1', C, act=ops.ACT_GELU)
        return self._lin(m, p + '.mlp.fc2', C, residual=x, gn_out=gn_next, out=out)

    def attn_block(self, x, p, gn_next=False):
        Fr, H, W, C = x.shape
        y = self._gn(x, p + '.norm', silu=False)
        qkv = self._lin(y, p + '.qkv', 3 * C)
        a = ops.mha(qkv[..., :C], qkv[..., C:2 * C], qkv[..., 2 * C:], Fr, H * W, 1, C, self._new(Fr, H, W, C))
        return self._lin(a, p + '.proj_out', C, residual=x, gn_out=gn_next)

    def encoder_layer(self, x, p, heads, depth, gn_next=False, out=None):
        for i in range(depth):
            x = self.swin_block(x, '%s.blocks.%d' % (p, i), heads, 2 if i % 2 == 1 else 0,
                                gn_next=gn_next and i == depth - 1, out=out if i == depth - 1 else None)
        return x

    def _cat_slot(self, Fr, H, W, C):
        return self._new(Fr, H, W, 2 * C + 32)

    def fuse_sft(self, enc, dec, key, wgt, gn_next=False):
        p = 'fuse_convs_dict.' + key
        Fr, H, W, C = dec.shape
        b, P = Fr // 3, H * W
        cat = getattr(enc, '_pgt_cat', None)
        if cat is None or getattr(dec, '_pgt_cat', None) is not cat:
            cat = self._new(Fr, H, W, 2 * C + 32)
            ops.copy2d(enc, cat[..., :C])
            ops.copy2d(dec, cat[..., C:2 * C])
        tcat = self._new(b, P, 192)
        ops.regroup_frames(self._lin(enc, p + '.tconvenc', 32), tcat[..., :96], b, P, 32, 0)
        ops.regroup_frames(self._lin(dec, p + '.tconvdec', 32), tcat[..., 96:], b, P, 32, 0)
        fut = ops.regroup_frames(self._lin(tcat, p + '.tfusion0', 96), self._new(Fr, P, 32), b, P, 32, 1)
        self._lin(fut, p + '.tfusion1', 32, out=cat.view(Fr, P, 2 * C + 32)[..., 2 * C:])
        return self.sft_tail(cat, dec, p, wgt, gn_next)

    def sft_tail(self, cat, dec, p, wgt, gn_next=False):
        C = dec.shape[-1]
        e = p + '.encode_enc'
        h = self._conv3(cat, e + '.conv1', C, gn=e + '.norm1', gn_out=True)
        sc = self._lin(cat, e + '.conv_out', C)
        ef = self._conv3(h, e + '.conv2', C, gn=e + '.norm2', residual=sc)
        scale = self._conv3(self._conv3(ef, p + '.scale.0', C, act=ops.ACT_LRELU02), p + '.scale.2', C)
        sh = self._conv3(ef, p + '.shift.0', C, act=ops.ACT_LRELU02)
        return self._conv3(sh, p + '.shift.2', C, residual=dec, sft_scale=scale, sft_w=wgt, gn_out=gn_next)

    def _repack_parsing(self):
        sd, w = self._sd, self.w
        P = 'conditionnet.'

        def fold(conv, bn):
            wt = sd[P + conv + '.weight'].float()
            if bn is None:
                return wt, None
            g, b = sd[P + bn + '.weight'].float(), sd[P + bn + '.bias'].float()
            m, v = sd[P + bn + '.running_mean'].float(), sd[P + bn + '.running_var'].float()
            s = g / torch.sqrt(v + 1e-5)
            return wt * s.view(-1, 1, 1, 1), (b - m * s).contiguous()

        def put(key, conv, bn, kind):
            wt, bias = fold(conv, bn)
            w['bn.' + key + '.weight'] = {'c3': _pack_conv, 'up': _pack_up2x, 'lin': _pack_lin,
                                          'rgb': _pack_rgb}[kind](wt)
            if bias is not None:
                w['bn.' + key + '.bias'] = bias

        put('stem', 'cp.resnet.conv1', 'cp.resnet.bn1', 'rgb')
        for li in (1, 2, 3, 4):
            for bi in (0, 1):
                p = 'cp.resnet.layer%d.%d' % (li, bi)
                put(p + '.c1', p + '.conv1', p + '.bn1', 'c3')
                put(p + '.c2', p + '.conv2', p + '.bn2', 'c3')
                if (P + p + '.downsample.0.weight') in sd:
                    put(p + '.ds', p + '.downsample.0', p + '.downsample.1', 'lin')
        for a in ('arm16', 'arm32'):
            put(a + '.conv', 'cp.%s.conv.conv' % a, 'cp.%s.conv.bn' % a, 'c3')
            put(a + '.att', 'cp.%s.conv_atten' % a, 'cp.%s.bn_atten' % a, 'lin')
        put('head32', 'cp.conv_head32.conv', 'cp.conv_head32.bn', 'up')
        put('head16', 'cp.conv_head16.conv', 'cp.conv_head16.bn', 'up')
        put('avg', 'cp.conv_avg.conv', 'cp.conv_avg.bn', 'lin')
        put('ffm.blk', 'ffm.convblk.conv', 'ffm.convblk.bn', 'lin')
        put('ffm.c1', 'ffm.conv1', None, 'lin')
        put('ffm.c2', 'ffm.conv2', None, 'lin')
        for o in ('conv_out', 'conv_out16', 'conv_out32'):
            put(o + '.conv', o + '.conv.conv', o + '.conv.bn', 'c3')
            put(o + '.out', o + '.conv_out', None, 'lin')

    def _pconv(self, x, key, cout, stride=1, **kw):
        Fr, H, W, _ = x.shape
        out = self._new(Fr, H // stride, W // stride, cout)
        return ops.conv(x, self.w['bn.' + key + '.weight'], cout, out, stride=stride, pad_lo=1,
                        bias=self.w.get('bn.' + key + '.bias'), **kw)

    def _plin(self, x, key, n, act=ops.ACT_NONE, out=None):
        if out is None:
            out = self._new(*x.shape[:-1], n)
        return ops.linear(x, self.w['bn.' + key + '.weight'], out, bias=self.w.get('bn.' + key + '.bias'), N=n, act=act)

    def _basic_block(self, x, p, cout, stride):
        r = self._pconv(x, p + '.c1', cout, stride, act=ops.ACT_RELU)
        if ('bn.' + p + '.ds.weight') in self.w:
            Fr, H, W, cin = x.shape
            sc = self._new(Fr, H // stride, W // stride, cout)
            ops.conv(x, self.w['bn.' + p + '.ds.weight'], cout, sc, ksize=1, stride=stride, pad_lo=0,
                     bias=self.w['bn.' + p + '.ds.bias'])
        else:
            sc = x
        return self._pconv(r, p + '.c2', cout, 1, act=ops.ACT_RELU, residual=sc, relu_after_res=True)

    def parsing_net(self, x):
        Fr, _, H, W = x.shape
        w = self.w
        t = ops.conv_rgb(x, w['bn.stem.weight'], w['bn.stem.bias'], self._new(Fr, H // 2, W // 2, 64), 7, 2, 3,
                         act=ops.ACT_RELU, mean3=(0.485, 0.456, 0.406), std3=(0.229, 0.224, 0.225))
        t = ops.maxpool3x3s2(t, self._new(Fr, H // 4, W // 4, 64))
        feats = []
        for li, cout, stride in ((1, 64, 1), (2, 128, 2), (3, 256, 2), (4, 512, 2)):
            t = self._basic_block(t, 'cp.resnet.layer%d.0' % li, cout, stride)
            t = self._basic_block(t, 'cp.resnet.layer%d.1' % li, cout, 1)
            feats.append(t)
        f8, f16, f32 = feats[1], feats[2], feats[3]
        avg = self._plin(ops.global_avgpool(f32, self._new(Fr, 512)), 'avg', 128, act=ops.ACT_RELU)
        a32 = self._pconv(f32, 'arm32.conv', 128, act=ops.ACT_RELU)
        att = self._plin(ops.global_avgpool(a32, self._new(Fr, 128)), 'arm32.att', 128, act=ops.ACT_SIGMOID)
        s32 = ops.channel_affine(a32, att, self._new(*a32.shape), addv=avg)
        u32 = ops.conv_up2x(s32, w['bn.head32.weight'], 128, self._new(Fr, H // 16, W // 16, 128), bias=w['bn.head32.bias'],
                            act=ops.ACT_RELU)
        a16 = self._pconv(f16, 'arm16.conv', 128, act=ops.ACT_RELU)
        att = self._plin(ops.global_avgpool(a16, self._new(Fr, 128)), 'arm16.att', 128, act=ops.ACT_SIGMOID)
        s16 = ops.channel_affine(a16, att, self._new(*a16.shape), addm=u32)
        u16 = ops.conv_up2x(s16, w['bn.head16.weight'], 128, self._new(Fr, H // 8, W // 8, 128), bias=w['bn.head16.bias'],
                            act=ops.ACT_RELU)
        cat = self._new(Fr, H // 8, W // 8, 256)
        ops.copy2d(f8, cat[..., :128])
        ops.copy2d(u16, cat[..., 128:])
        fc = self._plin(cat, 'ffm.blk', 256, act=ops.ACT_RELU)
        at = self._plin(self._plin(ops.global_avgpool(fc, self._new(Fr, 256)), 'ffm.c1', 64, act=ops.ACT_RELU),
                        'ffm.c2', 256, act=ops.ACT_SIGMOID)
        fuse = ops.channel_affine(fc, at, self._new(*fc.shape), plus_one=True)
        o0 = self._plin(self._pconv(fuse, 'conv_out.conv', 256, act=ops.ACT_RELU), 'conv_out.out', 19,
                        out=self._new(Fr, H // 8, W // 8, 32))
        o1 = self._plin(self._pconv(u16, 'conv_out16.conv', 64, act=ops.ACT_RELU), 'conv_out16.out', 19,
                        out=self._new(Fr, H // 8, W // 8, 32))
        o2 = self._plin(self._pconv(u32, 'conv_out32.conv', 64, act=ops.ACT_RELU), 'conv_out32.out', 19,
                        out=self._new(Fr, H // 16, W // 16, 32))
        return ops.assemble_cond(o0, o1, o2, self._new(Fr, H // 16, W // 16, 64))

    def _walk(self, blocks, h, lo=0, hi=None, taps=None, outs=None, feats=None, wgt=0.0, gn_outs=None):
        fusing = _fusing(feats, wgt)
        hi = len(blocks) if hi is None else hi
        outs, gn_outs, found = outs or {}, gn_outs or {}, {}
        for i in range(lo, hi):
            blk = blocks[i]
            kind, p, cout = blk.kind, blk.prefix, blk.cout
            if kind == 'fuse' and not fusing:
                continue
            nxt = next((b.kind in ('res', 'attn', 'norm') for b in blocks[i + 1:] if fusing or b.kind != 'fuse'), False)
            if kind == 'conv_in':
                h = self.conv_in(h, p) if p + '.weight' == self.arch.stem else self._conv3(h, p, cout, gn_out=nxt)
            elif kind == 'res':
                h = self.td_resblock(h, p, cout, gn_next=nxt, out=outs.get(i), shortcut=self.arch.res_shortcut)
            elif kind == 'attn':
                h = self.attn_block(h, p, gn_next=nxt)
            elif kind == 'swin':
                h = self.encoder_layer(h, p, blk.heads, blk.depth, gn_next=nxt, out=outs.get(i))
            elif kind == 'down':
                h = self._conv3(h, p + '.conv', cout, stride=2, pad_lo=0, gn_out=nxt, out=outs.get(i),
                                gn_into=gn_outs.get(i))
            elif kind == 'up':
                h = self.up2x(h, p + '.conv')
            elif kind == 'fuse':
                h = self.fuse_sft(feats[blk.src], h, p[len('fuse_convs_dict.'):], wgt, gn_next=nxt)
            else:
                raise AssertionError(kind)
            if taps and i in taps:
                found[taps[i]] = h
        return h, found

    @staticmethod
    def _cat_half(cat, lo, C):
        half = cat[..., lo:lo + C]
        half._pgt_cat = cat
        return half

    def encoder_frames(self, x, outs=None, gn_outs=None):
        a = self.arch
        h, feats = self._walk(a.enc_blocks, x, 0, a.frame_blocks, a.enc_taps, outs, gn_outs=gn_outs)
        return h, feats, a.frame_blocks

    def conv_in(self, x, p='encoder.conv_in'):
        a = self.arch
        Fr, _, H, W = x.shape
        h = self._new(Fr, H, W, a.ch)
        stats = self._gn_stats(h, H * W // 32) if (H * W) % 128 == 0 and a.ch in (64, 128) else None
        ops.conv_rgb(x, self.w[p + '.weight'], self.w[p + '.bias'], h, 3, 1, 1, gn_stats=stats)
        return h

    def encoder_clips(self, h, feats, i, outs=None):
        a = self.arch
        h, more = self._walk(a.enc_blocks, h, i, len(a.enc_blocks) - 2, a.enc_taps, outs)
        norm, conv = a.enc_blocks[-2:]
        return self._conv3(h, conv.prefix, conv.cout, gn=norm.prefix), list(feats.values()) + list(more.values())

    def encoder(self, x, fusing=False):
        a = self.arch
        outs = {}
        if fusing:
            Fr, _, H, W = x.shape
            for i, lvl in a.enc_taps.items():
                C = a.level_ch[lvl]
                if lvl in a.fuse_level_key and lvl != a.num_levels - 1:
                    outs[i] = self._cat_half(self._cat_slot(Fr, H >> lvl, W >> lvl, C), 0, C)
        return self.encoder_clips(*self.encoder_frames(x, outs), outs)

    def _gather(self, t, idx):
        return ops.gather_frames(t, idx, self._new(idx.numel(), *t.shape[1:], dtype=t.dtype))

    def decoder(self, z, feats=None, wgt=0.0):
        blocks = self.arch.dec_blocks
        outs = {}
        for i, b in enumerate(blocks):
            cat = getattr(feats[b.src], '_pgt_cat', None) if b.kind == 'fuse' and _fusing(feats, wgt) else None
            if cat is not None:
                outs[i - 1] = self._cat_half(cat, b.cout, b.cout)
        h, _ = self._walk(blocks, z, 0, len(blocks) - 2, outs=outs, feats=feats, wgt=wgt)
        norm, conv = blocks[-2:]
        return self.decoder_out(h, norm.prefix, conv.prefix, conv.cout, self.arch.dec_tail_silu)

    def up2x(self, h, p):
        Fr, H, W, C = h.shape
        out = self._new(Fr, 2 * H, 2 * W, C)
        stats = self._gn_stats(out, 16 * self._stats_tiles(H, W, C, 2, 1, 1))
        return ops.conv_up2x(h, self.w[p + '.weight'], C, out, bias=self.w[p + '.bias'], gn_stats=stats)

    def decoder_out(self, h, norm, conv, out_ch, silu):
        Fr, H, W, _ = h.shape
        out = self._new(Fr, out_ch, H, W, dtype=torch.float32)
        st = getattr(h, '_pgt_gn', None)
        ab = ops.groupnorm_ab(h, self.w[norm + '.weight'], self.w[norm + '.bias'],
                              self._new(Fr * 2 * h.shape[-1], dtype=torch.float32),
                              stats=st[0] if st else None, chunks_per_frame=st[1] if st else 0)
        if ops.conv_out_gn(h, ab, self.w[conv + '.weight'], out_ch, self.w.get(conv + '.bias'), out,
                           silu=silu) is not None:
            return out
        self._conv3(h, conv, out_ch, out=out, gn=norm, gn_silu=silu, nchw=True)
        return out

    def parse_pos(self, x, out=None):
        Fr, _, H, W = x.shape
        cond = self.parsing_net(x)
        return self._lin(cond.view(Fr * (H // 16) * (W // 16), 64), 'convpos', 512, K=57, out=out)

    def global_transformer(self, lq, pos, clips):
        a, wd = self.arch, self.w
        T, E = lq.shape[0], a.dim_embd
        L = T // clips
        q = self._lin(lq, 'feat_emb', E, out_dtype=torch.float32)
        for i in range(a.n_layers):
            p = 'ft_layers.%d' % i
            y, y2 = self._new(T, E), self._new(T, E)
            ops.layernorm(q, wd[p + '.norm1.weight'], wd[p + '.norm1.bias'], y, pos=pos, out2=y2)
            qk = self._lin(y2, p + '.self_attn.qk', 2 * E)
            v = self._lin(y, p + '.self_attn.v', E)
            att = ops.mha(qk[:, :E], qk[:, E:], v, clips, L, a.n_head, E // a.n_head, self._new(T, E))
            q = self._lin(att, p + '.self_attn.out_proj', E, out_dtype=torch.float32, residual=q)
            y = ops.layernorm(q, wd[p + '.norm2.weight'], wd[p + '.norm2.bias'], self._new(T, E))
            m = self._lin(y, p + '.linear1', 2 * E, act=ops.ACT_GELU)
            q = self._lin(m, p + '.linear2', E, out_dtype=torch.float32, residual=q)
        y = ops.layernorm(q, wd['idx_pred_layer.0.weight'], wd['idx_pred_layer.0.bias'], self._new(T, E))
        return self._lin(y, 'idx_pred_layer.1', self.depth * a.n_embed, out_dtype=torch.float32)

    @_on_device
    @torch.no_grad()
    def forward(self, x, w=1.0, adain=True, code_only=False, force_codes=None, frame_index=None):
        a = self.arch
        x = x.to(self.dev, torch.float32).contiguous()
        Fr, _, H, W = x.shape
        if frame_index is not None:
            Fr = frame_index.numel()
        if Fr % a.tf != 0 or H % 64 != 0 or W % 64 != 0:
            raise ValueError('expected b*3 frames with H, W multiples of 64, got %s' % (tuple(x.shape),))
        if frame_index is not None:
            return self._window_tail(self._frame_pass(x, w), frame_index, w, adain, code_only, force_codes)
        pos = self.parse_pos(x)
        h, feats = self.encoder(x, fusing=not code_only and float(w) > 0)
        return self._restore(h, feats, pos, w, adain, code_only, force_codes)

    def _frame_pass(self, x, w=0.0, ring=None, slot=0):
        a = self.arch
        last, n = a.frame_blocks - 1, x.shape[0]
        outs, gn_outs = {}, {}
        if ring is None:
            levels = list(a.fuse_level_key) if float(w) > 0 else []
        else:
            rows = slice(slot, slot + n)
            levels = list(ring['feats'])
            outs = {i: ring['feats'][lvl][rows] for i, lvl in a.enc_taps.items() if lvl in levels}
            outs[last] = ring['h'][rows]
            if 'h_stats' in ring:
                gn_outs[last] = ring['h_stats'][rows].view(-1)
        pos = self.parse_pos(x, out=None if ring is None else ring['pos'][rows].flatten(0, 1))
        h, feats, _ = self.encoder_frames(x, outs, gn_outs)
        rec = {'pos': pos.view(n, -1, pos.shape[-1]), 'h': h,
               'feats': {lvl: f for lvl, f in feats.items() if lvl in levels}}
        gn = getattr(h, '_pgt_gn', None)
        if gn is not None:
            rec['h_stats'] = gn[0].view(n, -1)
        return rec

    def _window_tail(self, rec, index, w, adain, code_only=False, force_codes=None):
        a = self.arch
        pos = self._gather(rec['pos'], index)
        fusing = _fusing(rec['feats'], w)
        feats = {lvl: self._gather(rec['feats'][lvl], index) if fusing and lvl in rec['feats'] else None
                 for i, lvl in a.enc_taps.items() if i < a.frame_blocks}
        h = self._gather(rec['h'], index)
        if 'h_stats' in rec:
            h._pgt_gn = (self._gather(rec['h_stats'], index).view(-1), rec['h_stats'].shape[1] // 64)
        h, feats = self.encoder_clips(h, feats, a.frame_blocks)
        return self._restore(h, feats, pos.view(-1, pos.shape[-1]), w, adain, code_only, force_codes)

    def _restore(self, h, feats, pos, w, adain, code_only=False, force_codes=None):
        a = self.arch
        Fr, hh, ww, _ = h.shape
        T = Fr * hh * ww
        wd = self.w
        h = h.view(T, -1)
        lq32 = self._lin(h, 'quant_conv', a.embed_dim, out_dtype=torch.float32)
        lq = self._lin(h, 'quant_conv', a.embed_dim)
        logits = self.global_transformer(lq, pos, Fr // 3)
        D = self.depth
        logits5 = logits.view(Fr, hh, ww, D, a.n_embed)
        lq_nhwc = lq32.view(Fr, hh, ww, a.embed_dim)
        if code_only:
            return logits5, lq_nhwc
        codes = torch.empty(T * D, dtype=torch.int64, device=self.dev)
        quant = self._new(T, a.embed_dim, dtype=torch.float32)
        idx_in = force_codes.to(self.dev).reshape(T * D).contiguous() if force_codes is not None else None
        if D == 1:
            ops.argmax_gather(logits, wd['codebook'], codes, quant, idx_in=idx_in)
        else:
            if idx_in is None:
                ops.argmax_gather(logits.view(T * D, a.n_embed), wd['codebook'], codes, None)
            else:
                codes = idx_in
            ops.rq_embed(codes, 0, D - 1, wd['codebooks'], quant, ldi=D, ldd=1)
        self.last_codes = codes.view(Fr, hh, ww, D)
        if torch.is_tensor(adain):
            quant = ops.adain(quant.view(Fr, hh * ww, -1), lq.view(Fr, hh * ww, -1), self._new(Fr, hh * ww, a.embed_dim),
                              flags=adain)
        elif adain:
            quant = ops.adain(quant.view(Fr, hh * ww, -1), lq.view(Fr, hh * ww, -1), self._new(Fr, hh * ww, a.embed_dim))
        else:
            quant = quant.to(BF)
        z = self._lin(quant.reshape(T, a.embed_dim), 'post_quant_conv', a.z_channels)
        out = self.decoder(z.view(Fr, hh, ww, a.z_channels), feats, w if torch.is_tensor(w) else float(w))
        return out, logits5, lq_nhwc

    @_on_device
    @torch.no_grad()
    def graphed(self, method, tensors, writes=(), **scalars):
        tensors = [t.to(self.dev) for t in tensors]
        key = (method.__name__, tuple((tuple(t.shape), t.dtype) for t in tensors), tuple(sorted(scalars.items())))
        if not hasattr(self, '_graphs'):
            self._graphs = {}
        entry = self._graphs.get(key)
        if entry is None:
            static = [torch.empty(t.shape, dtype=t.dtype, device=self.dev) for t in tensors]
            for s, t in zip(static, tensors):
                s.copy_(t)
            entry = self._graphs[key] = (static,) + self._capture(lambda: method(*static, **scalars))
        static, graph, outs = entry
        for s, t in zip(static, tensors):
            s.copy_(t, non_blocking=True)
        graph.replay()
        for i in writes:
            tensors[i].copy_(static[i], non_blocking=True)
        return outs

    def _capture(self, run, pool=None):
        if not hasattr(self, 'capture_stream'):
            self.capture_stream = torch.cuda.Stream(device=self.dev)
        cur = torch.cuda.current_stream(self.dev)
        side = torch.cuda.Stream(device=self.dev)
        side.wait_stream(cur)
        try:
            with torch.cuda.stream(side):
                for _ in range(2):
                    run()
        finally:
            cur.wait_stream(side)
        graph = torch.cuda.CUDAGraph()
        with torch.cuda.graph(graph, pool=pool, stream=self.capture_stream):
            out = run()
        return graph, out

    def forward_graphed(self, x, w=1.0, adain=True):
        x = x.to(self.dev, torch.float32).contiguous()
        return self.graphed(self.forward, (x,), w=float(w), adain=bool(adain))

    @_on_device
    @torch.no_grad()
    def restore_windows(self, frames_u8, index, w=1.0, adain=True, reuse_frames=True, size=None):
        Fd, h, w_src, _ = frames_u8.shape
        if size is None:
            H, W = h, w_src
            x = ops.u8hwc_to_f32nchw(frames_u8, self._new(Fd, 3, H, W, dtype=torch.float32))
        else:
            H, W = size
            x = ops.u8hwc_resize_to_f32nchw(frames_u8, self._new(Fd, 3, H, W, dtype=torch.float32), (h, w_src))
        if reuse_frames:
            out = self.forward(x, w=w, adain=adain, frame_index=index)[0]
        else:
            xc = ops.gather_frames(x, index, self._new(index.numel(), 3, H, W, dtype=torch.float32))
            out = self.forward(xc, w=w, adain=adain)[0]
        n = index.numel() // 3
        return ops.f32nchw_to_u8hwc(out, torch.empty(n, H, W, 3, dtype=torch.uint8, device=self.dev), first=1, step=3)

    @_on_device
    @torch.no_grad()
    def live_ring(self, H, W, w, streams=1):
        if H % 64 or W % 64:
            raise ValueError('expected H, W multiples of 64, got %dx%d' % (H, W))
        rows = 4 * int(streams)
        rec = self._frame_pass(torch.zeros(1, 3, H, W, dtype=torch.float32, device=self.dev), w)
        ring = {k: self._new(rows, *t.shape[1:], dtype=t.dtype) for k, t in rec.items() if k != 'feats'}
        ring['feats'] = {lvl: self._new(rows, *f.shape[1:], dtype=f.dtype) for lvl, f in rec['feats'].items()}
        return ring

    @staticmethod
    def ring_entries(ring):
        return [ring[k] for k in ('pos', 'h', 'h_stats') if k in ring] + list(ring['feats'].values())

    @_on_device
    @torch.no_grad()
    def frame_step(self, x, slot, ring):
        self._frame_pass(x, ring=ring, slot=slot)

    @_on_device
    @torch.no_grad()
    def window_step(self, index, w, adain, ring, out_u8):
        out = self._window_tail(ring, index, w, adain)[0]
        return ops.f32nchw_to_u8hwc(out, out_u8, first=1, step=3)

    @_on_device
    @torch.no_grad()
    def pool_step(self, u8, x, ring, slots, index, w, adain, out_u8, sizes=None):
        if slots is not None:
            B, st = slots.numel(), u8.shape[0] // 4 * 3
            if sizes is None:
                xs = ops.u8hwc_to_f32nchw(u8[st:st + B], x[:B])
            else:
                xs = ops.u8hwc_resize_to_f32nchw(u8[st:st + B], x[:B], tuple(u8.shape[1:3]), sizes)
            self.frame_step(xs, st, ring)
            for t in self.ring_entries(ring) + [u8]:
                ops.scatter_frames(t[st:st + B], slots, t)
        if index is not None:
            self.window_step(index, w, adain, ring, out_u8)

    def _codebook(self, d=0):
        if d == 0 or self.arch.shared_codebook:
            return self.w['codebook']
        return self.w['codebooks'][d]

    def _n_embed(self, d=0):
        a = self.arch
        return a.n_embeds[d] if hasattr(a, 'n_embeds') else a.n_embed

    def _codebook_pack(self, d=0):
        key = 'codebook.pack' if d == 0 or self.arch.shared_codebook else 'codebook.pack.%d' % d
        if key not in self.w:
            self.w[key] = ops.codebook_pack(self._codebook(d), self._n_embed(d))
        return self.w[key]

    def _argmin(self, *a, **k):
        return ops.l2_argmin_tc(*a, **k)

    def quantize(self, z):
        T, E = z.shape
        D = self.depth
        z_q = self._new(T, E, dtype=torch.float32)
        if D == 1:
            codes = torch.empty(T, dtype=torch.int64, device=self.dev)
            self._argmin(z, self.w['codebook'], self._codebook_pack(), self._n_embed(0), codes, z_q)
            return codes.view(T, 1), z_q, (z - z_q).pow(2).mean()
        codes = torch.empty(D, T, dtype=torch.int64, device=self.dev)
        r = self._new(T, E, dtype=torch.float32)
        losses = []
        for d in range(D):
            src = z if d == 0 else r
            self._argmin(src, self._codebook(d), self._codebook_pack(d), self._n_embed(d), codes[d])
            ops.rq_residual(src, r if d < D - 1 else None, codes[d], self._codebook(d), z_q, d == 0)
            losses.append((z - z_q).pow(2).mean())
        return codes.t().contiguous(), z_q, torch.stack(losses).mean()

    @_on_device
    @torch.no_grad()
    def encode(self, x):
        a = self.arch
        x = x.to(self.dev, torch.float32).contiguous()
        h, _ = self.encoder(x)
        Fr, hh, ww, _ = h.shape
        z_e = self._lin(h.view(Fr * hh * ww, -1), 'quant_conv', a.embed_dim, out_dtype=torch.float32)
        return z_e.view(Fr, hh, ww, a.embed_dim)

    @_on_device
    @torch.no_grad()
    def decode(self, z_q):
        a = self.arch
        Fr, hh, ww, E = z_q.shape
        z = self._lin(z_q.to(self.dev, BF).reshape(Fr * hh * ww, E), 'post_quant_conv', a.z_channels)
        return self.decoder(z.view(Fr, hh, ww, a.z_channels))

    @_on_device
    @torch.no_grad()
    def embed_code(self, codes, d0=0, d1=None):
        D = self.depth
        codes = codes.to(self.dev, torch.int64).reshape(-1, D).contiguous()
        d1 = D - 1 if d1 is None else d1
        quant = self._new(codes.shape[0], self.arch.embed_dim, dtype=torch.float32)
        if D == 1:
            ops.argmax_gather(None, self.w['codebook'], None, quant, idx_in=codes.view(-1))
        else:
            ops.rq_embed(codes, d0, d1, self.w['codebooks'], quant, ldi=D, ldd=1)
        return quant

    @_on_device
    @torch.no_grad()
    def decode_code(self, codes):
        Fr, hh, ww, _ = codes.shape
        return self.decode(self.embed_code(codes).view(Fr, hh, ww, self.arch.embed_dim))

    @_on_device
    @torch.no_grad()
    def embed_code_with_depth(self, codes):
        D = self.depth
        if D == 1:
            return self.embed_code(codes).unsqueeze(1)
        codes = codes.to(self.dev, torch.int64).reshape(-1, D).contiguous()
        out = self._new(codes.shape[0], D, self.arch.embed_dim, dtype=torch.float32)
        for d in range(D):
            ops.rq_embed(codes, d, d, self.w['codebooks'], out[:, d], ldi=D, ldd=1)
        return out

    @_on_device
    @torch.no_grad()
    def soft_codes(self, z_e, temp, stochastic=False):
        a = self.arch
        z = z_e.to(self.dev, torch.float32).reshape(-1, a.embed_dim).contiguous()
        T, D, K = z.shape[0], self.depth, a.n_embed
        p = self._new(T, D, K, dtype=torch.float32)
        codes = torch.empty(D, T, dtype=torch.int64, device=self.dev)
        r = self._new(T, a.embed_dim, dtype=torch.float32) if D > 1 else None
        for d in range(D):
            src = z if d == 0 else r
            pack = self._codebook_pack(d)
            ops.soft_codes(src, self._codebook(d), pack[1], K, temp, p[:, d])
            if stochastic:
                seed = torch.randint(-2 ** 63, 2 ** 63 - 1, (2,), dtype=torch.int64, device=self.dev)
                ops.sample_codes(p[:, d], seed, codes[d])
            else:
                ops.l2_argmin_tc(src, self._codebook(d), pack, K, codes[d])
            if d < D - 1:
                ops.rq_residual(src, r, codes[d], self._codebook(d), None, d == 0)
        return p, codes.t().contiguous()

    @_on_device
    @torch.no_grad()
    def forward_vq(self, x, code_only=False):
        a = self.arch
        z_e = self.encode(x)
        Fr, hh, ww, _ = z_e.shape
        T = Fr * hh * ww
        z_e = z_e.view(T, a.embed_dim)
        codes, z_q, loss = self.quantize(z_e)
        codes = codes.view(Fr, hh, ww, self.depth)
        z_q = z_q.view(Fr, hh, ww, -1)
        if code_only:
            return z_q, loss, codes
        return self.decode(z_q), loss, codes
```

### pgtformer_b200/ops.py

```python
import ctypes

import torch

from . import _lib as L
from ._lib import (ACT_GELU, ACT_LRELU02, ACT_NONE, ACT_RELU, ACT_SIGMOID, ACT_SILU, BF16, EPI_PLAIN,
                   EPI_SFT, F32, OUT_NCHW, OUT_NHWC, Epilogue)


def _p(t):
    return ctypes.c_void_p(t.data_ptr()) if t is not None else None


def _stream(t=None):
    if t is not None:
        return ctypes.c_void_p(torch.cuda.current_stream(t.device).cuda_stream)
    return ctypes.c_void_p(torch.cuda.current_stream().cuda_stream)


def _dt(t):
    if t.dtype == torch.bfloat16:
        return BF16
    if t.dtype == torch.float32:
        return F32
    raise TypeError('unsupported dtype %s' % t.dtype)


def _rows(t):
    assert t.is_cuda and t.stride(-1) == 1, 'expected a CUDA channels-last tensor'
    C = t.shape[-1]
    ld = t.stride(-2) if t.dim() > 1 else C
    rows = 1
    exp = ld
    for d in range(t.dim() - 2, -1, -1):
        assert t.shape[d] == 1 or t.stride(d) == exp, 'non-uniform row stride'
        exp *= t.shape[d]
        rows *= t.shape[d]
    return rows, C, ld


def make_epilogue(out, bias=None, act=ACT_NONE, residual=None, sft_scale=None, sft_w=0.0, nchw=False,
                  relu_after_res=False, gn_stats=None):
    ep = Epilogue()
    ep.flags = 1 if relu_after_res else 0
    if gn_stats is not None:
        assert gn_stats.dtype == torch.float32 and gn_stats.is_contiguous()
        ep.gn_stats = gn_stats.data_ptr()
    ep.bias = bias.data_ptr() if bias is not None else None
    if bias is not None:
        assert bias.dtype == torch.float32 and bias.is_contiguous()
    ep.act = act
    ep.mode = EPI_SFT if sft_scale is not None else EPI_PLAIN
    if residual is not None:
        _, _, ldr = _rows(residual)
        ep.residual, ep.ldr, ep.res_dtype = residual.data_ptr(), ldr, _dt(residual)
    if sft_scale is not None:
        _, _, lda = _rows(sft_scale)
        assert sft_scale.dtype == torch.bfloat16
        ep.aux, ep.ldaux = sft_scale.data_ptr(), lda
        if torch.is_tensor(sft_w):
            assert sft_w.dtype == torch.float32 and sft_w.is_contiguous() and sft_w.device == out.device
            ep.sft_wf = sft_w.data_ptr()
        else:
            ep.sft_w = float(sft_w)
    ep.out = out.data_ptr()
    ep.out_dtype = _dt(out)
    if nchw:
        assert out.is_contiguous() and out.dtype == torch.float32
        ep.out_layout, ep.ldo = OUT_NCHW, 0
    else:
        ep.out_layout, ep.ldo = OUT_NHWC, _rows(out)[2]
    return ep


def gn_stats_supported(C):
    return C % 32 == 0 and C // 32 in (2, 4, 8, 16, 32)


def linear(a, w, out, bias=None, act=ACT_NONE, residual=None, K=None, N=None, relu_after_res=False, gn_stats=None):
    lib = L.load()
    M, Ka, lda = _rows(a)
    Nw, Kw = w.shape
    K = K if K is not None else min(Ka, Kw)
    N = N if N is not None else Nw
    assert a.dtype == torch.bfloat16 and w.dtype == torch.bfloat16 and w.stride(1) == 1
    assert _rows(out)[0] == M and out.shape[-1] >= N
    ep = make_epilogue(out, bias, act, residual, relu_after_res=relu_after_res, gn_stats=gn_stats)
    L.check(lib.pgt_linear_bf16(_p(a), lda, _p(w), w.stride(0), M, N, K, ctypes.byref(ep), _stream()))
    return out


def conv(x, wp, cout, out, ksize=3, stride=1, pad_lo=1, bias=None, act=ACT_NONE, residual=None, sft_scale=None,
         sft_w=0.0, nchw=False, relu_after_res=False, gn_stats=None):
    lib = L.load()
    F, H, W, Cin = x.shape
    assert not torch.is_tensor(sft_w) or sft_w.numel() == F
    assert x.dtype == torch.bfloat16 and x.stride(3) == 1 and x.stride(1) == W * x.stride(2) and \
        (F == 1 or x.stride(0) == H * x.stride(1))
    ep = make_epilogue(out, bias, act, residual, sft_scale, sft_w, nchw, relu_after_res, gn_stats)
    L.check(lib.pgt_conv_bf16(_p(x), F, H, W, Cin, x.stride(2), _p(wp), wp.stride(0), cout, ksize, stride, pad_lo,
                              ctypes.byref(ep), _stream()))
    return out


def conv_rgb(x_nchw, wp, bias, out, ksize, stride, pad, act=ACT_NONE, mean3=None, std3=None, gn_stats=None):
    lib = L.load()
    F, C, H, W = x_nchw.shape
    assert C == 3 and x_nchw.dtype == torch.float32 and x_nchw.is_contiguous() and wp.dtype == torch.bfloat16
    m = (ctypes.c_float * 3)(*[float(v) for v in mean3]) if mean3 is not None else None
    s = (ctypes.c_float * 3)(*[float(v) for v in std3]) if std3 is not None else None
    L.check(lib.pgt_conv_rgb_bf16(_p(x_nchw), F, H, W, ksize, stride, pad, m, s, _p(wp), wp.stride(0), wp.shape[0],
                                  _p(bias), act, _p(out), _rows(out)[2], _p(gn_stats), _stream()))
    return out


def conv_up2x(x, wp4, cout, out, bias=None, act=ACT_NONE, gn_stats=None):
    lib = L.load()
    F, H, W, Cin = x.shape
    assert x.dtype == torch.bfloat16 and wp4.dtype == torch.bfloat16 and wp4.is_contiguous() and wp4.dim() == 3
    assert tuple(out.shape) == (F, 2 * H, 2 * W, cout) and out.is_contiguous()
    ep = make_epilogue(out, bias, act, gn_stats=gn_stats)
    L.check(lib.pgt_conv_up2x_bf16(_p(x), F, H, W, Cin, x.stride(2), _p(wp4), wp4.stride(1), cout, ctypes.byref(ep),
                                   _stream()))
    return out


_gn_ws = {}


def _gn_workspace(kind, x, n):
    if torch.cuda.is_current_stream_capturing():
        return torch.empty(max(n, 1), dtype=torch.float32, device=x.device)
    key = (kind, x.device.index, torch.cuda.current_stream().cuda_stream)
    ws = _gn_ws.get(key)
    if ws is None or ws.numel() < n:
        ws = torch.empty(max(n, 1 << 16), dtype=torch.float32, device=x.device)
        _gn_ws[key] = ws
    return ws


def groupnorm_silu(x, gamma, beta, out, eps=1e-6, silu=True):
    lib = L.load()
    F = x.shape[0]
    C = x.shape[-1]
    HW = x.numel() // (F * C) if x.is_contiguous() else x.shape[1] * x.shape[2]
    _, _, ldx = _rows(x)
    _, _, ldy = _rows(out)
    ws = _gn_workspace('stats', x, lib.pgt_groupnorm_ws_floats(F, HW, C))
    L.check(lib.pgt_groupnorm_silu(_p(x), ldx, F, HW, C, _p(gamma), _p(beta), eps, int(silu), _p(out), ldy, _p(ws),
                                   _stream()))
    return out


def conv_tiles_per_frame(H, W, cout, ksize=3, stride=1, pad_lo=1):
    return int(L.load().pgt_conv_tiles_per_frame(H, W, cout, ksize, stride, pad_lo))


def conv_tiles_exact(H, W, cout, ksize=3, stride=1, pad_lo=1):
    return int(L.load().pgt_conv_tiles_exact(H, W, cout, ksize, stride, pad_lo))


def groupnorm_apply_stats(x, gamma, beta, out, stats, chunks_per_frame, eps=1e-6, silu=True):
    lib = L.load()
    F = x.shape[0]
    C = x.shape[-1]
    HW = x.shape[1] * x.shape[2]
    ws = _gn_workspace('ab', x, F * 2 * C)
    L.check(lib.pgt_groupnorm_apply_stats(_p(x), _rows(x)[2], F, HW, C, _p(gamma), _p(beta), eps, int(silu), _p(out),
                                          _rows(out)[2], _p(stats), chunks_per_frame, _p(ws), _stream()))
    return out


def groupnorm_ab(x, gamma, beta, ab, stats=None, chunks_per_frame=0, eps=1e-6):
    lib = L.load()
    F = x.shape[0]
    C = x.shape[-1]
    HW = x.shape[1] * x.shape[2]
    ws = None if stats is not None else _gn_workspace('stats', x, lib.pgt_groupnorm_ws_floats(F, HW, C))
    assert ab.dtype == torch.float32 and ab.numel() >= F * 2 * C and ab.is_contiguous()
    L.check(lib.pgt_groupnorm_ab(_p(x), _rows(x)[2], F, HW, C, _p(gamma), _p(beta), eps, _p(stats), chunks_per_frame,
                                 _p(ws), _p(ab), _stream()))
    return ab


def conv_out_gn(x, ab, wp, cout, bias, out, silu=True):
    lib = L.load()
    F, H, W, Cin = x.shape
    assert x.dtype == torch.bfloat16 and x.stride(3) == 1 and x.stride(1) == W * x.stride(2) and \
        (F == 1 or x.stride(0) == H * x.stride(1))
    assert out.dtype == torch.float32 and out.is_contiguous() and tuple(out.shape) == (F, cout, H, W)
    if silu:
        rc = lib.pgt_conv_out_gn(_p(x), F, H, W, Cin, x.stride(2), _p(ab), _p(wp), wp.stride(0), cout, _p(bias), _p(out),
                                 _stream(x))
    else:
        rc = lib.pgt_conv_out_gn_act(_p(x), F, H, W, Cin, x.stride(2), _p(ab), _p(wp), wp.stride(0), cout, _p(bias),
                                     _p(out), 0, _stream(x))
    if rc == -3:
        return None
    L.check(rc)
    return out


def layernorm(x, gamma, beta, out, eps=1e-5, pos=None, out2=None):
    lib = L.load()
    T, C, ldx = _rows(x)
    L.check(lib.pgt_layernorm(_p(x), ldx, _dt(x), T, C, _p(gamma), _p(beta), eps, _p(out), _rows(out)[2],
                              _p(pos), _rows(pos)[2] if pos is not None else 0,
                              _p(out2), _rows(out2)[2] if out2 is not None else 0, _stream()))
    return out


def ln_linear(x, ln_g, ln_b, w, bias, out, eps=1e-5):
    lib = L.load()
    T, C, ldx = _rows(x)
    assert x.dtype == torch.bfloat16 and w.dtype == torch.bfloat16 and w.stride(1) == 1 and out.dtype == torch.bfloat16
    L.check(lib.pgt_ln_linear_bf16(_p(x), ldx, T, C, _p(ln_g), _p(ln_b), eps, _p(w), w.stride(0), w.shape[0], _p(bias),
                                   _p(out), _rows(out)[2], _stream()))
    return out


def swin_mlp(x, ln_g, ln_b, w1, b1, w2, b2, out, eps=1e-5, gn_stats=None):
    lib = L.load()
    T, C, ldx = _rows(x)
    assert x.dtype == torch.bfloat16 and w1.dtype == torch.bfloat16 and w1.is_contiguous() and w2.is_contiguous()
    L.check(lib.pgt_swin_mlp_bf16(_p(x), ldx, T, C, _p(ln_g), _p(ln_b), eps, _p(w1), _p(b1), _p(w2), _p(b2), _p(out),
                                  _rows(out)[2], _p(gn_stats), _stream()))
    return out


def window_attention(qkv, clips, H, W, C, heads, shift, bias_tab, out):
    lib = L.load()
    assert qkv.dtype == torch.bfloat16 and bias_tab.dtype == torch.float32 and bias_tab.is_contiguous()
    L.check(lib.pgt_window_attention(_p(qkv), _rows(qkv)[2], clips, H, W, C, heads, shift, _p(bias_tab), _p(out),
                                     _rows(out)[2], _stream()))
    return out


LOG2E = 1.4426950408889634


def window_tables(bias):
    heads = bias.shape[0]
    dev = bias.device
    r = torch.arange(48, device=dev)
    tabs = []
    for t in range(4):
        if t == 0:
            f, iy, ix = r // 16, (r // 4) % 4, r % 4
        elif t == 1:
            rr = r % 24
            f, iy, ix = rr // 8, (rr % 8) // 2, rr % 2 + 2 * (r // 24)
        elif t == 2:
            rr = r % 24
            f, iy, ix = rr // 8, (rr % 8) // 4 + 2 * (r // 24), rr % 4
        else:
            pp, rr = r // 12, r % 12
            f, iy, ix = rr // 4, (rr % 4) // 2 + 2 * (pp // 2), rr % 2 + 2 * (pp % 2)
        canon = f * 16 + iy * 4 + ix
        tt = bias[:, canon][:, :, canon].float() * LOG2E
        tabs.append(tt.view(heads, 48, 6, 8).permute(0, 2, 1, 3))
    return torch.stack(tabs, 0).to(torch.float16).contiguous()


def window_attention_tc(qkv, clips, H, W, C, heads, shift, tab16, out):
    lib = L.load()
    assert qkv.dtype == torch.bfloat16 and tab16.dtype == torch.float16 and tab16.is_contiguous()
    rc = lib.pgt_window_attention_tc(_p(qkv), _rows(qkv)[2], clips, H, W, C, heads, shift, _p(tab16), _p(out),
                                     _rows(out)[2], _stream(qkv))
    if rc == -3:
        return None
    L.check(rc)
    return out


def window3d_attention(qkv, B, D, H, W, C, heads, window, shift, bias, out, pad_qkv=None):
    lib = L.load()
    assert qkv.dtype == torch.bfloat16 and bias.dtype == torch.float32 and bias.is_contiguous()
    L.check(lib.pgt_window3d_attention(_p(qkv), _rows(qkv)[2], _p(pad_qkv), B, D, H, W, C, heads, window[0], window[1],
                                       window[2], shift[0], shift[1], shift[2], _p(bias), _p(out), _rows(out)[2],
                                       _stream(qkv)))
    return out


def mha(q, k, v, clips, L_, heads, d, out):
    lib = L.load()
    L.check(lib.pgt_mha_fwd(_p(q), _rows(q)[2], _p(k), _rows(k)[2], _p(v), _rows(v)[2], clips, L_, heads, d, _p(out),
                            _rows(out)[2], _stream()))
    return out


def argmax_gather(logits, codebook, idx_out, quant, idx_in=None):
    lib = L.load()
    if logits is None:
        assert idx_in is not None and idx_in.dtype == torch.int64 and idx_in.is_contiguous()
        T, K = idx_in.numel(), 4
    else:
        T, K = logits.shape
        assert logits.dtype == torch.float32 and logits.is_contiguous()
    assert codebook.dtype == torch.float32
    assert idx_out is None or idx_out.dtype == torch.int64
    L.check(lib.pgt_argmax_gather(_p(logits), T, K, _p(codebook), codebook.shape[1], _p(idx_in), _p(idx_out),
                                  _p(quant), _rows(quant)[2] if quant is not None else 0,
                                  _dt(quant) if quant is not None else 0, _stream()))
    return idx_out, quant


def l2_argmin(z, codebook, K, idx_out, quant=None):
    lib = L.load()
    T, E = z.shape
    assert z.dtype == torch.float32 and z.is_contiguous() and codebook.is_contiguous()
    L.check(lib.pgt_l2_argmin(_p(z), T, E, _p(codebook), K, _p(idx_out), _p(quant), _stream()))
    return idx_out, quant


def codebook_pack(codebook, K):
    lib = L.load()
    E = codebook.shape[1]
    assert codebook.dtype == torch.float32 and codebook.is_contiguous() and codebook.shape[0] >= K
    cb16 = torch.empty(K, E, dtype=torch.bfloat16, device=codebook.device)
    norm = torch.empty(K + 2, dtype=torch.float32, device=codebook.device)
    L.check(lib.pgt_codebook_pack(_p(codebook), K, E, _p(cb16), _p(norm), _stream(codebook)))
    return cb16, norm


L2_ARGMIN_UNSUPPORTED = -3
_last_argmin_ws = None


def last_l2_argmin_fallbacks():
    return int(_last_argmin_ws[0].item()) if _last_argmin_ws is not None else 0


def l2_argmin_tc(z, codebook, pack, K, idx_out, quant=None):
    lib = L.load()
    T, E = z.shape
    assert z.dtype == torch.float32 and z.is_contiguous() and codebook.is_contiguous() and idx_out.dtype == torch.int64
    global _last_argmin_ws
    ws = torch.empty(int(lib.pgt_l2_argmin_ws_ints(T)), dtype=torch.int32, device=z.device)
    _last_argmin_ws = ws
    rc = lib.pgt_l2_argmin_tc(_p(z), T, E, _p(codebook), _p(pack[0]), _p(pack[1]), K, _p(idx_out), _p(quant), _p(ws),
                              _stream(z))
    if rc == L2_ARGMIN_UNSUPPORTED:
        return l2_argmin(z, codebook, K, idx_out, quant)
    L.check(rc)
    return idx_out, quant


ARGMIN_MIN_CODES_PER_SPLIT = 512


def argmin_splits(T, K, device=None):
    sms = torch.cuda.get_device_properties(device if device is not None else torch.cuda.current_device()).multi_processor_count
    tiles = (T + 127) // 128
    return max(1, min(K // 128, sms // tiles, K // ARGMIN_MIN_CODES_PER_SPLIT))


def l2_argmin_tc_split(z, codebook, pack, K, idx_out, quant=None, splits=None):
    lib = L.load()
    T, E = z.shape
    assert z.dtype == torch.float32 and z.is_contiguous() and codebook.is_contiguous() and idx_out.dtype == torch.int64
    if splits is None:
        splits = argmin_splits(T, K, z.device)
    ws = torch.empty(int(lib.pgt_l2_argmin_split_ws_ints(T, int(splits))), dtype=torch.int32, device=z.device)
    L.check(lib.pgt_l2_argmin_tc_split(_p(z), T, E, _p(codebook), _p(pack[0]), _p(pack[1]), K, int(splits), _p(idx_out),
                                       _p(quant), _p(ws), _stream(z)))
    return idx_out, quant


def soft_codes(z, codebook, norm, K, temp, out):
    lib = L.load()
    T, E = z.shape
    assert z.dtype == torch.float32 and z.is_contiguous() and codebook.dtype == torch.float32 and codebook.is_contiguous()
    assert codebook.shape[1] == E and codebook.shape[0] >= K and norm.dtype == torch.float32 and norm.numel() >= K
    assert out.dtype == torch.float32 and tuple(out.shape) == (T, K) and out.stride(1) == 1
    L.check(lib.pgt_soft_codes(_p(z), T, E, _p(codebook), _p(norm), K, float(temp), _p(out), out.stride(0), _stream(z)))
    return out


def sample_codes(p, seed, idx_out):
    lib = L.load()
    T, K = p.shape
    assert p.dtype == torch.float32 and p.stride(1) == 1 and idx_out.dtype == torch.int64 and idx_out.numel() == T
    assert idx_out.is_contiguous() and seed.dtype == torch.int64 and seed.numel() == 2 and seed.device == p.device
    assert idx_out.device == p.device
    L.check(lib.pgt_sample_codes(_p(p), T, K, p.stride(0), _p(seed), _p(idx_out), _stream(p)))
    return idx_out


def rq_residual(r_in, r_out, idx, codebook, agg, first):
    lib = L.load()
    ref = agg if agg is not None else r_out
    T, E = ref.shape
    assert codebook.dtype == torch.float32 and codebook.is_contiguous() and codebook.shape[1] == E
    assert idx.dtype == torch.int64 and idx.is_contiguous() and idx.numel() == T and idx.device == ref.device
    for r in (r_in, r_out, agg):
        assert r is None or (r.dtype == torch.float32 and r.is_contiguous() and tuple(r.shape) == (T, E))
    L.check(lib.pgt_rq_residual(_p(r_in), _p(r_out), _p(idx), T, E, _p(codebook), _p(agg), int(bool(first)),
                                _stream(ref)))
    return agg


def rq_embed(idx, d0, d1, codebooks, out, ldi, ldd):
    lib = L.load()
    T, E, ldo = _rows(out)
    assert codebooks.dtype == torch.float32 and codebooks.is_contiguous() and codebooks.dim() == 3 and codebooks.shape[2] == E
    assert idx.dtype == torch.int64 and idx.device == out.device and 0 <= d0 <= d1
    assert codebooks.shape[0] == 1 or d1 < codebooks.shape[0]
    assert idx.is_contiguous() and (T - 1) * ldi + d1 * ldd < idx.numel()
    cb_stride = 0 if codebooks.shape[0] == 1 else codebooks.shape[1] * E
    L.check(lib.pgt_rq_embed(_p(idx), ldi, ldd, T, d0, d1, _p(codebooks), cb_stride, E, _p(out), ldo, _dt(out),
                             _stream(out)))
    return out


def vq_stats(z, codebook, idx, HW, beta, scalars, zq_nchw=None, zq_bf16=None, min_enc=None, scores=None, usage=None):
    lib = L.load()
    T, E = z.shape
    K = codebook.shape[0]
    assert z.dtype == torch.float32 and z.is_contiguous() and codebook.dtype == torch.float32 and codebook.is_contiguous()
    assert codebook.shape[1] == E and idx.dtype == torch.int64 and idx.is_contiguous() and idx.numel() == T
    assert scalars.dtype == torch.float32 and scalars.numel() >= 3 and scalars.is_contiguous()
    assert zq_nchw is None or (zq_nchw.dtype == torch.float32 and zq_nchw.is_contiguous() and zq_nchw.numel() == T * E
                               and zq_nchw.shape[1] == E)
    assert zq_bf16 is None or (zq_bf16.dtype == torch.bfloat16 and zq_bf16.is_contiguous() and zq_bf16.numel() == T * E)
    assert min_enc is None or (min_enc.dtype == torch.float32 and min_enc.is_contiguous() and min_enc.numel() == T * K)
    assert scores is None or (scores.dtype == torch.float32 and scores.is_contiguous() and scores.numel() == T)
    assert usage is None or (usage.dtype == torch.int32 and usage.is_contiguous() and usage.numel() == K)
    for t in (idx, zq_nchw, zq_bf16, min_enc, scores, usage, scalars):
        assert t is None or t.device == z.device
    hist = torch.zeros(K, dtype=torch.int32, device=z.device)
    ws = torch.empty(max(int(lib.pgt_vq_stats_ws_doubles(T, E)), 1), dtype=torch.float64, device=z.device)
    L.check(lib.pgt_vq_stats(_p(z), T, E, int(HW), _p(codebook), K, _p(idx), float(beta), _p(zq_nchw), _p(zq_bf16),
                             _p(min_enc), _p(scores), _p(usage), _p(hist), _p(ws), _p(scalars), _stream(z)))
    return scalars


def adain(q, style, out, eps=1e-5, flags=None):
    lib = L.load()
    F = q.shape[0]
    C = q.shape[-1]
    HW = q.shape[1] * q.shape[2] if q.dim() == 4 else q.shape[1]
    if flags is None:
        L.check(lib.pgt_adain(_p(q), _rows(q)[2], _dt(q), _p(style), _rows(style)[2], F, HW, C, eps, _p(out),
                              _rows(out)[2], _stream()))
        return out
    assert flags.dtype == torch.int32 and flags.is_contiguous() and flags.numel() == F and flags.device == q.device
    L.check(lib.pgt_adain_frames(_p(q), _rows(q)[2], _dt(q), _p(style), _rows(style)[2], F, HW, C, eps, _p(flags),
                                 _p(out), _rows(out)[2], _stream()))
    return out


def maxpool3x3s2(x, out):
    lib = L.load()
    F, H, W, C = x.shape
    L.check(lib.pgt_maxpool3x3s2(_p(x), _rows(x)[2], F, H, W, C, _p(out), _rows(out)[2], _stream()))
    return out


def global_avgpool(x, out):
    lib = L.load()
    F, H, W, C = x.shape
    L.check(lib.pgt_global_avgpool(_p(x), _rows(x)[2], F, H * W, C, _p(out), out.stride(0), _stream()))
    return out


def channel_affine(x, scale, out, plus_one=False, addv=None, addm=None):
    lib = L.load()
    F, H, W, C = x.shape
    L.check(lib.pgt_channel_affine(_p(x), _rows(x)[2], F, H * W, C, _p(scale), scale.stride(0), int(plus_one),
                                   _p(addv), addv.stride(0) if addv is not None else 0,
                                   _p(addm), _rows(addm)[2] if addm is not None else 0, _p(out), _rows(out)[2], _stream()))
    return out


def assemble_cond(o0, o1, o2, cond, ncls=19):
    lib = L.load()
    F, h8, w8, _ = o0.shape
    _, h16, w16, _ = o2.shape
    L.check(lib.pgt_assemble_cond(_p(o0), _rows(o0)[2], _p(o1), _rows(o1)[2], _p(o2), _rows(o2)[2], F, h8, w8, h16, w16,
                                  ncls, _p(cond), _rows(cond)[2], _stream()))
    return cond


def u8hwc_to_f32nchw(x_u8, out):
    lib = L.load()
    F, H, W, C = x_u8.shape
    assert C == 3 and x_u8.dtype == torch.uint8 and x_u8.is_contiguous() and x_u8.is_cuda
    assert out.dtype == torch.float32 and tuple(out.shape) == (F, 3, H, W) and out.is_contiguous()
    L.check(lib.pgt_u8hwc_to_f32nchw(_p(x_u8), F, H, W, _p(out), _stream()))
    return out


def u8hwc_resize_to_f32nchw(x_u8, out, hw, sizes=None):
    lib = L.load()
    F, C, H, W = out.shape
    h, w = hw
    assert x_u8.dtype == torch.uint8 and x_u8.is_contiguous() and x_u8.is_cuda
    assert C == 3 and out.dtype == torch.float32 and out.is_contiguous() and out.device == x_u8.device
    if sizes is None:
        assert x_u8.numel() >= F * h * w * 3
    else:
        assert sizes.dtype == torch.int32 and sizes.is_contiguous() and sizes.numel() == 3 * F and \
            sizes.device == x_u8.device
    L.check(lib.pgt_u8hwc_resize_to_f32nchw(_p(x_u8), F, h, w, _p(sizes), H, W, _p(out), _stream()))
    return out


def f32nchw_to_u8hwc(x, out_u8, first=0, step=1):
    lib = L.load()
    n, H, W, C = out_u8.shape
    assert C == 3 and out_u8.dtype == torch.uint8 and out_u8.is_contiguous()
    assert x.dtype == torch.float32 and x.is_contiguous() and x.shape[1:] == (3, H, W) and first + (n - 1) * step < x.shape[0]
    L.check(lib.pgt_f32nchw_to_u8hwc(_p(x), first, step, n, H, W, _p(out_u8), _stream()))
    return out_u8


def gather_frames(x, idx_i32, out):
    lib = L.load()
    assert x.is_contiguous() and out.is_contiguous() and x.dtype == out.dtype and x.shape[1:] == out.shape[1:]
    assert idx_i32.dtype == torch.int32 and idx_i32.is_cuda and idx_i32.numel() == out.shape[0]
    fb = x[0].numel() * x.element_size()
    L.check(lib.pgt_gather_frames(_p(x), fb, _p(idx_i32), out.shape[0], _p(out), _stream()))
    return out


def scatter_frames(x, idx_i32, out):
    lib = L.load()
    assert x.is_contiguous() and out.is_contiguous() and x.dtype == out.dtype and x.shape[1:] == out.shape[1:]
    assert idx_i32.dtype == torch.int32 and idx_i32.is_cuda and idx_i32.numel() == x.shape[0]
    fb = x[0].numel() * x.element_size()
    L.check(lib.pgt_scatter_frames(_p(x), fb, _p(idx_i32), x.shape[0], _p(out), _stream()))
    return out


def copy2d(x, out):
    lib = L.load()
    T, C, ldx = _rows(x)
    L.check(lib.pgt_copy2d(_p(x), ldx, T, C, _p(out), _rows(out)[2], _stream()))
    return out


def regroup_frames(x, out, clips, P, C, direction):
    lib = L.load()
    L.check(lib.pgt_regroup_frames(_p(x), _rows(x)[2], clips, P, C, _p(out), _rows(out)[2], direction, _stream()))
    return out


def nchw_to_nhwc(x, out, mean=None, std=None):
    lib = L.load()
    F, C, H, W = x.shape
    assert x.dtype == torch.float32 and x.is_contiguous()
    L.check(lib.pgt_nchw_f32_to_nhwc_bf16(_p(x), F, C, H * W, _p(mean), _p(std), _p(out), _rows(out)[2], _stream()))
    return out


def nhwc_to_f32(x, out, to_nchw):
    lib = L.load()
    F, H, W, C = x.shape
    L.check(lib.pgt_nhwc_bf16_to_f32(_p(x), _rows(x)[2], F, H * W, C, _p(out), int(to_nchw), _stream()))
    return out


def launch_count():
    return int(L.load().pgt_launch_count())


def reset_launch_count():
    L.load().pgt_reset_launch_count()


PROF_CLASSES = ('gemm_tc', 'window_attn', 'mha', 'argmax_gather', 'l2_argmin', 'groupnorm', 'move', 'layernorm')


def profile_begin():
    L.check(L.load().pgt_profile_begin())


def profile_end(csv_path=None):
    n = len(PROF_CLASSES)
    work, ms, cnt = (ctypes.c_double * n)(), (ctypes.c_double * n)(), (ctypes.c_int64 * n)()
    if csv_path is None:
        L.check(L.load().pgt_profile_end(work, ms, cnt))
    else:
        L.check(L.load().pgt_profile_end_csv(csv_path.encode(), work, ms, cnt))
    return {PROF_CLASSES[i]: (work[i], ms[i], int(cnt[i])) for i in range(n)}
```

Baseline: 91.07.

## Fuse residual 1x1 shortcut GEMM into conv2 of resblocks

Adds a conv variant that first runs the 1x1 shortcut projection as extra K-blocks in the same kernel, packs that partial result (plus shortcut bias) to bf16 into the residual staging panel, then restarts accumulation for the 3x3 conv and adds it back as the residual in the epilogue. This removes a separate linear launch and the global write and read of the shortcut tensor for resblocks with more than 64 channels. In exchange it adds a mid-tile wait and smem stores in the MMA warps, extra template instances, and rounds the shortcut to bf16 before the add.

Result: no change. 91.91 (median of 6 runs) (+0.9%).

```diff
diff --git a/include/pgt_b200.h b/include/pgt_b200.h
--- a/include/pgt_b200.h
+++ b/include/pgt_b200.h
@@ -60,6 +60,9 @@
 
 int pgt_conv_bf16(const void* x, int F, int Hin, int Win, int Cin, int ldx, const void* Wp, int ldw,
                   int Cout, int ksize, int stride, int pad_lo, const pgt_epilogue* ep, void* stream);
+
+int pgt_conv_sc_bf16(const void* x, int F, int Hin, int Win, int Cin, int ldx, const void* xs, int Cs, int ldxs,
+                     const float* bsc, const void* Wp, int ldw, int Cout, const pgt_epilogue* ep, void* stream);
 
 int pgt_conv_out_gn(const void* x, int F, int H, int W, int Cin, int ldx, const float* gn_ab, const void* Wp, int ldw,
                     int Cout, const float* bias, float* out, void* stream);
diff --git a/pgtformer_b200/_lib.py b/pgtformer_b200/_lib.py
--- a/pgtformer_b200/_lib.py
+++ b/pgtformer_b200/_lib.py
@@ -31,6 +31,8 @@
     'pgt_linear_bf16': (c_int, [c_void_p, c_int, c_void_p, c_int, c_int, c_int, c_int, POINTER(Epilogue), c_void_p]),
     'pgt_conv_bf16': (c_int, [c_void_p, c_int, c_int, c_int, c_int, c_int, c_void_p, c_int, c_int, c_int, c_int,
                               c_int, POINTER(Epilogue), c_void_p]),
+    'pgt_conv_sc_bf16': (c_int, [c_void_p, c_int, c_int, c_int, c_int, c_int, c_void_p, c_int, c_int, c_void_p, c_void_p,
+                                 c_int, c_int, POINTER(Epilogue), c_void_p]),
     'pgt_conv_out_gn': (c_int, [c_void_p, c_int, c_int, c_int, c_int, c_int, c_void_p, c_void_p, c_int, c_int, c_void_p,
                                 c_void_p, c_void_p]),
     'pgt_conv_out_gn_act': (c_int, [c_void_p, c_int, c_int, c_int, c_int, c_int, c_void_p, c_void_p, c_int, c_int,
diff --git a/pgtformer_b200/csrc/gemm_tc.cu b/pgtformer_b200/csrc/gemm_tc.cu
--- a/pgtformer_b200/csrc/gemm_tc.cu
+++ b/pgtformer_b200/csrc/gemm_tc.cu
@@ -41,6 +41,8 @@
   int F, H, W;
   int tw, th, tn, tiles_x, tiles_y;
   int cin_blocks, ksize, pad_lo, cin_ld;
+  int sc_blocks;
+  const float* sc_bias;
   int pad_x, pad_y;
   long long o_sx, o_sy, o_sf;
   int b_resident;
@@ -249,6 +251,36 @@
       o.x = __float_as_uint(f[4 * q]); o.y = __float_as_uint(f[4 * q + 1]);
       o.z = __float_as_uint(f[4 * q + 2]); o.w = __float_as_uint(f[4 * q + 3]);
       sts128(srow + ((q ^ (r & 7)) << 4), o);
+    }
+  }
+}
+
+template <int R>
+__device__ __forceinline__ void sc_pack(const float (&d)[R], uint32_t (&pairs)[R / 2], const GemmParams& p, int col_base,
+                                        int lane) {
+  const float* b = p.sc_bias != nullptr ? p.sc_bias + col_base + 2 * (lane & 3) : nullptr;
+#pragma unroll
+  for (int f = 0; f < R / 4; ++f) {
+    if (b != nullptr) {
+      const float b0 = __ldg(b + 8 * f), b1 = __ldg(b + 8 * f + 1);
+      pairs[2 * f] = pack_bf16x2(d[4 * f] + b0, d[4 * f + 1] + b1);
+      pairs[2 * f + 1] = pack_bf16x2(d[4 * f + 2] + b0, d[4 * f + 3] + b1);
+    } else {
+      pairs[2 * f] = pack_bf16x2(d[4 * f], d[4 * f + 1]);
+      pairs[2 * f + 1] = pack_bf16x2(d[4 * f + 2], d[4 * f + 3]);
+    }
+  }
+}
+
+template <int F0, int R>
+__device__ __forceinline__ void sc_to_panel(const uint32_t (&pairs)[R / 2], uint32_t slot, int r0, int lane) {
+#pragma unroll
+  for (int j = 0; j < 8; ++j) {
+#pragma unroll
+    for (int h = 0; h < 2; ++h) {
+      const int r = r0 + (lane >> 2) + 8 * h;
+      const uint32_t a = slot + r * 128 + ((j ^ (r & 7)) << 4) + 4 * (lane & 3);
+      asm volatile("st.shared.b32 [%0], %1;" ::"r"(a), "r"(pairs[2 * (F0 + j) + h]) : "memory");
     }
   }
 }
@@ -433,9 +465,9 @@
   return p.gn_stats + (chunk * 32 + col0 / p.gn_cpg) * 2;
 }
 
-template <int BN, bool kVec>
+template <int BN, bool kVec, bool kSc = false>
 __device__ __forceinline__ void epilogue_tile(const GemmParams& p, const EpiCtx& ctx, int warp, int lane, int tile, int& k,
-                                              const float (&acc)[BN / 2]) {
+                                              const float (&acc)[BN / 2], const uint32_t (&scv)[BN / 4]) {
   const int quad = warp & 3;
   const int half = warp >> 2;
   const int r = quad * 32 + lane;
@@ -462,6 +494,11 @@
     if (col_base + g * 64 >= p.N) return;
     named_bar_sync(EPI_BAR, EPI_WARPS * 32);
     acc_to_smem<g * 64, 64>(acc, ctx.xch + half * 64 * XCH_LD, XCH_LD, quad, lane);
+    if constexpr (kSc) {
+      const int pos = k & (SLOTS - 1);
+      mbar_wait_spin(&ctx.res_bar[pos], (k >> SLOT_SHIFT) & 1);
+      sc_to_panel<g * 8, BN / 2>(scv, smem_u32(ctx.staging) + pos * PANEL_BYTES, half * 64 + quad * 16, lane);
+    }
     named_bar_sync(EPI_BAR, EPI_WARPS * 32);
 
     if (p.fast_epi) {
@@ -500,7 +537,7 @@
             uint32_t v[32];
             smem_row_32(xrow + pnl * PW + sb * 32 - g * 64, v);
             epi_finish<false>(p, v, bias_vec && !pre ? p.bias + col0 : nullptr, stg + pos * PANEL_BYTES, r, sb, esize,
-                              p.has_res_map != 0, gn_ptr(col0), col0, b, pre);
+                              p.has_res_map != 0 || kSc, gn_ptr(col0), col0, b, pre);
           }
           fence_proxy_async();
           mbar_arrive(&ctx.slot_ready[pos]);
@@ -522,7 +559,7 @@
   });
 }
 
-template <int BN, bool kVec>
+template <int BN, bool kVec, bool kSc = false>
 __device__ __forceinline__ void epilogue_tile_wg(const GemmParams& p, const EpiCtx& ctx, int wq, int bar, int tile, int k,
                                                  const float (&acc)[2][BN / 2]) {
   const int lane = lane_id();
@@ -567,7 +604,7 @@
                            gn_stats_ptr(p, m_blk, wq, col0), col0, nb, false, sft_weight(p, m_blk, r));
         else
           epi_finish<false>(p, v, bias_vec ? p.bias + col0 : nullptr, stg + pos * PANEL_BYTES, r, sub, esize,
-                            p.has_res_map != 0, gn_stats_ptr(p, m_blk, wq, col0), col0, nb, false);
+                            p.has_res_map != 0 || kSc, gn_stats_ptr(p, m_blk, wq, col0), col0, nb, false);
       }
       if (sub == nsub - 1) {
         fence_proxy_async();
@@ -591,11 +628,11 @@
   if (lane == 0) mbar_arrive(bar);
 }
 
-template <int BN, bool kVec>
+template <int BN, bool kVec, bool kSc = false>
 __global__ void __launch_bounds__(GEMM_THREADS, 1)
 gemm_tc_kernel(const __grid_constant__ CUtensorMap tmA, const __grid_constant__ CUtensorMap tmB,
                const __grid_constant__ CUtensorMap tmO, const __grid_constant__ CUtensorMap tmR,
-               const __grid_constant__ CUtensorMap tmX, const GemmParams p) {
+               const __grid_constant__ CUtensorMap tmX, const __grid_constant__ CUtensorMap tmS, const GemmParams p) {
   using Cfg = GemmCfg<BN>;
   constexpr int STAGES = Cfg::STAGES;
   extern __shared__ uint8_t smem_raw[];
@@ -620,6 +657,7 @@
     if (p.fast_epi) tma_prefetch_desc(&tmO);
     if (p.has_res_map) tma_prefetch_desc(&tmR);
     if (p.fast_epi && p.epi_mode == PGT_EPI_SFT) tma_prefetch_desc(&tmX);
+    if (p.sc_blocks) tma_prefetch_desc(&tmS);
     for (int i = 0; i < STAGES; ++i) {
       mbar_init(&full_bar[i], 1);
       mbar_init(&empty_bar[i], EPI_WARPS);
@@ -637,6 +675,7 @@
     if (warp == PRODUCER_WARP) {
       int stage = 0;
       uint32_t phase = 0;
+      const int conv_kb = p.num_kb - p.sc_blocks;
       for (int tile = blockIdx.x; tile < num_tiles; tile += gridDim.x) {
         int n_blk, m_blk;
         tile_mn(p, tile, m_blk, n_blk);
@@ -647,10 +686,12 @@
           if (elect_one()) {
             void* dst_a = smem_a + stage * A_STAGE_BYTES;
             void* dst_b = smem_b + stage * Cfg::B_STAGE_BYTES;
+            const bool sc = kb < p.sc_blocks;
+            const int kc = kb - p.sc_blocks;
             int cb = 0, ax = 0, ay = 0, a5 = 0;
-            if (p.mode != MODE_LINEAR) {
-              const int tap = kb / p.cin_blocks;
-              cb = kb - tap * p.cin_blocks;
+            if (p.mode != MODE_LINEAR && !sc) {
+              const int tap = kc / p.cin_blocks;
+              cb = kc - tap * p.cin_blocks;
               const int dy = tap / p.ksize;
               const int dx = tap - dy * p.ksize;
               if (p.mode == MODE_CONV_S1) {
@@ -666,9 +707,10 @@
             }
             mbar_arrive_expect_tx(&full_bar[stage], Cfg::STAGE_BYTES);
             if (p.mode == MODE_LINEAR) tma_load_2d(dst_a, &tmA, &full_bar[stage], kb * BK, m_blk * BM);
+            else if (sc) tma_load_4d(dst_a, &tmS, &full_bar[stage], kb * BK, x0, y0, n0);
             else if (p.mode == MODE_CONV_S1) tma_load_4d(dst_a, &tmA, &full_bar[stage], cb * BK, ax, ay, n0);
             else tma_load_5d(dst_a, &tmA, &full_bar[stage], cb, ax, a5, ay, n0);
-            tma_load_2d(dst_b, &tmB, &full_bar[stage], kb * BK, n_blk * BN);
+            tma_load_2d(dst_b, &tmB, &full_bar[stage], (sc ? conv_kb + kb : kc) * BK, n_blk * BN);
           }
           __syncwarp();
           if (++stage == STAGES) { stage = 0; phase ^= 1; }
@@ -693,6 +735,7 @@
     int k = 0;
     for (int tile = blockIdx.x; tile < num_tiles; tile += gridDim.x) {
       float acc[BN / 2];
+      uint32_t scv[BN / 4];
       int prev = -1;
       for (int kb = 0; kb < p.num_kb; ++kb) {
         mbar_wait_spin(&full_bar[stage], phase);
@@ -701,8 +744,15 @@
         wgmma_fence();
 #pragma unroll
         for (int kk = 0; kk < BK / 16; ++kk)
-          wgmma_bf16<BN>(acc, da + 2 * kk, db + 2 * kk, (kb | kk) != 0 ? 1u : 0u);
+          wgmma_bf16<BN>(acc, da + 2 * kk, db + 2 * kk,
+                         (kSc ? (kk != 0 || (kb != 0 && kb != p.sc_blocks)) : (kb | kk) != 0) ? 1u : 0u);
         wgmma_commit();
+        if (kSc && kb == p.sc_blocks - 1) {
+          wgmma_wait<0>();
+          int m_blk, n_blk;
+          tile_mn(p, tile, m_blk, n_blk);
+          sc_pack(acc, scv, p, n_blk * BN, lane);
+        }
         wgmma_wait<1>();
         if (prev >= 0) release_stage(&empty_bar[prev], lane);
         prev = stage;
@@ -710,7 +760,7 @@
       }
       wgmma_wait<0>();
       release_stage(&empty_bar[prev], lane);
-      epilogue_tile<BN, kVec>(p, ctx, warp, lane, tile, k, acc);
+      epilogue_tile<BN, kVec, kSc>(p, ctx, warp, lane, tile, k, acc, scv);
     }
   }
 }
@@ -740,11 +790,11 @@
   s = t % S;
 }
 
-template <int BN, bool kVec>
+template <int BN, bool kVec, bool kSc = false>
 __global__ void __launch_bounds__(GEMM_THREADS, 1)
 conv_halo_kernel(const __grid_constant__ CUtensorMap tmA, const __grid_constant__ CUtensorMap tmB,
                  const __grid_constant__ CUtensorMap tmO, const __grid_constant__ CUtensorMap tmR,
-                 const __grid_constant__ CUtensorMap tmX, const GemmParams p) {
+                 const __grid_constant__ CUtensorMap tmX, const __grid_constant__ CUtensorMap tmS, const GemmParams p) {
   using Cfg = HaloCfg<BN>;
   constexpr int AS = Cfg::A_STAGES, BS = Cfg::B_STAGES;
   constexpr int RELEASERS = 4;
@@ -766,6 +816,7 @@
   const int lane = threadIdx.x & 31;
   const int num_tiles = p.m_tiles * p.n_tiles;
   const int cin_pad = p.cin_blocks * BK;
+  const int slabs = p.cin_blocks + p.sc_blocks;
 
   if (warp == PRODUCER_WARP && lane == 0) {
     tma_prefetch_desc(&tmA);
@@ -773,6 +824,7 @@
     if (p.fast_epi) tma_prefetch_desc(&tmO);
     if (p.has_res_map) tma_prefetch_desc(&tmR);
     if (p.fast_epi && p.epi_mode == PGT_EPI_SFT) tma_prefetch_desc(&tmX);
+    if (p.sc_blocks) tma_prefetch_desc(&tmS);
     for (int i = 0; i < AS; ++i) { mbar_init(&a_full[i], 1); mbar_init(&a_empty[i], RELEASERS); }
     for (int i = 0; i < BS; ++i) { mbar_init(&b_full[i], 1); mbar_init(&b_empty[i], RELEASERS); }
     for (int i = 0; i < Cfg::SLOTS; ++i) {
@@ -799,6 +851,7 @@
             int pn0, py0, px0;
             decode_conv_tile(p, pt / p.n_tiles, pn0, py0, px0);
             for (int cb = 0; cb < p.cin_blocks; ++cb) tma_prefetch_4d(&tmA, cb * BK, px0 - 1, py0 - 1, pn0);
+            for (int sb = 0; sb < p.sc_blocks; ++sb) tma_prefetch_4d(&tmS, sb * BK, px0 - 1, py0 - 1, pn0);
             if (p.has_res_map) {
               const int c0 = (pt % p.n_tiles) * BN;
               const int rw = p.out_dtype == PGT_BF16 ? 64 : 32;
@@ -810,20 +863,24 @@
           }
           __syncwarp();
         }
-        for (int cb = 0; cb < p.cin_blocks; ++cb) {
+        for (int cb = 0; cb < slabs; ++cb) {
+          const bool sc = cb < p.sc_blocks;
+          const int cc = cb - p.sc_blocks;
           mbar_wait(&a_empty[as], aph ^ 1);
           if (elect_one()) {
             mbar_arrive_expect_tx(&a_full[as], HALO_A_BYTES);
-            tma_load_4d(smem_a + as * HALO_A_STRIDE, &tmA, &a_full[as], cb * BK, x0 - 1, y0 - 1, n0);
+            tma_load_4d(smem_a + as * HALO_A_STRIDE, sc ? &tmS : &tmA, &a_full[as], (sc ? cb : cc) * BK, x0 - 1, y0 - 1,
+                        n0);
           }
           __syncwarp();
           if (++as == AS) { as = 0; aph ^= 1; }
           if (p.b_resident && tile != (int)blockIdx.x) continue;
-          for (int t = 0; t < p.ntaps; ++t) {
+          for (int t = 0; t < (sc ? 1 : p.ntaps); ++t) {
             mbar_wait(&b_empty[bs], bph ^ 1);
             if (elect_one()) {
               mbar_arrive_expect_tx(&b_full[bs], Cfg::B_BYTES);
-              tma_load_2d(smem_b + bs * Cfg::B_BYTES, &tmB, &b_full[bs], t * cin_pad + cb * BK, n_blk * BN);
+              tma_load_2d(smem_b + bs * Cfg::B_BYTES, &tmB, &b_full[bs], sc ? p.ntaps * cin_pad + cb * BK : t * cin_pad + cc * BK,
+                          n_blk * BN);
             }
             __syncwarp();
             if (++bs == BS) { bs = 0; bph ^= 1; }
@@ -846,7 +903,8 @@
     const uint32_t b_base = smem_u32(smem_b);
     constexpr uint64_t ROW_BLOCK = 8 * HALO_PITCH / 16;
     const ItemStream<BN> is(p, num_tiles);
-    const int b_per_tile = p.b_resident ? 0 : p.ntaps * p.cin_blocks;
+    const int b_blocks = p.ntaps * p.cin_blocks + p.sc_blocks;
+    const int b_per_tile = p.b_resident ? 0 : b_blocks;
     int as = 0, bs = 0;
     uint32_t aph = 0, bph = 0;
     int k = 0;
@@ -855,15 +913,19 @@
       const bool has_next = tile + (int)gridDim.x < num_tiles;
       const int items = p.fast_epi ? is.panels_in_tile(tile) : 0;
       if ((j & 1) != wg) {
-        ring_skip<AS>(as, aph, p.cin_blocks);
+        ring_skip<AS>(as, aph, slabs);
         ring_skip<BS>(bs, bph, b_per_tile);
         k += items;
         continue;
       }
       if (j > 0) named_bar_sync(PP_MMA_BAR + wg, 256);
       float acc[2][BN / 2];
-      for (int cb = 0; cb < p.cin_blocks; ++cb) {
-        const bool hand_over = has_next && cb == p.cin_blocks - 1;
+      int wb = 0;
+      for (int cb = 0; cb < slabs; ++cb) {
+        const bool hand_over = has_next && cb == slabs - 1;
+        const bool sc = cb < p.sc_blocks;
+        const int t0 = sc ? p.ntaps / 2 : 0;
+        const int t1 = sc ? t0 + 1 : p.ntaps;
         mbar_wait_spin(&a_full[as], aph);
         const uint64_t da0 = wgmma_desc_k_sw128(a_base + as * HALO_A_STRIDE, HALO_PITCH);
         auto tap_desc = [&](int t) -> uint64_t {
@@ -871,12 +933,12 @@
           return da0 + (uint64_t)(((dy + p.tap_oy) * (HALO_TW + 2) + dx + p.tap_ox) * 8);
         };
         if (p.b_resident && first) {
-          for (int t = 0; t < p.ntaps * p.cin_blocks; ++t) mbar_wait_spin(&b_full[t], 0);
+          for (int t = 0; t < b_blocks; ++t) mbar_wait_spin(&b_full[t], 0);
           first = false;
         }
         int prev = -1;
-        for (int t = 0; t < p.ntaps; ++t) {
-          int bst = cb * p.ntaps + t;
+        for (int t = t0; t < t1; ++t) {
+          int bst = wb++;
           if (!p.b_resident) {
             mbar_wait_spin(&b_full[bs], bph);
             bst = bs;
@@ -886,12 +948,12 @@
           wgmma_fence();
 #pragma unroll
           for (int kk = 0; kk < BK / 16; ++kk) {
-            const uint32_t accum = (cb | t | kk) != 0 ? 1u : 0u;
+            const uint32_t accum = (kSc ? (kk != 0 || t != t0 || (cb != 0 && cb != p.sc_blocks)) : (cb | t | kk) != 0) ? 1u : 0u;
             wgmma_bf16<BN>(acc[0], da + 2 * kk, db + 2 * kk, accum);
             wgmma_bf16<BN>(acc[1], da + ROW_BLOCK + 2 * kk, db + 2 * kk, accum);
           }
           wgmma_commit();
-          if (hand_over && t == p.ntaps - 1) named_bar_arrive(PP_MMA_BAR + (wg ^ 1), 256);
+          if (hand_over && t == t1 - 1) named_bar_arrive(PP_MMA_BAR + (wg ^ 1), 256);
           wgmma_wait<1>();
           if (!p.b_resident) {
             if (prev >= 0) release_stage(&b_empty[prev], lane);
@@ -900,12 +962,29 @@
           }
         }
         wgmma_wait<0>();
+        if (kSc && cb == p.sc_blocks - 1) {
+          static_for<0, BN / 64>([&](auto pc) {
+            constexpr int pn = decltype(pc)::value;
+            if (pn < items) {
+              const int item = k + pn;
+              const int pos = item & (Cfg::SLOTS - 1);
+              mbar_wait_spin(&res_bar[pos], (item >> (Cfg::SLOTS == 4 ? 2 : 1)) & 1);
+              const uint32_t slot = smem_u32(staging) + pos * PANEL_BYTES;
+              static_for<0, 2>([&](auto rc) {
+                constexpr int rb = decltype(rc)::value;
+                uint32_t pairs[BN / 4];
+                sc_pack(acc[rb], pairs, p, (tile % p.n_tiles) * BN, lane);
+                sc_to_panel<pn * 8, BN / 2>(pairs, slot, rb * 64 + (warp & 3) * 16, lane);
+              });
+            }
+          });
+        }
         if (!p.b_resident) release_stage(&b_empty[prev], lane);
         release_stage(&a_empty[as], lane);
         if (++as == AS) { as = 0; aph ^= 1; }
       }
       if (j > 0) named_bar_sync(PP_EPI_BAR + wg, 256);
-      epilogue_tile_wg<BN, kVec>(p, ctx, warp & 3, PP_XCH_BAR + wg, tile, k, acc);
+      epilogue_tile_wg<BN, kVec, kSc>(p, ctx, warp & 3, PP_XCH_BAR + wg, tile, k, acc);
       if (has_next) named_bar_arrive(PP_EPI_BAR + (wg ^ 1), 256);
       k += items;
     }
@@ -949,6 +1028,7 @@
     if (p.res_dtype == p.out_dtype && aligned16(p.residual) && ((long long)p.ldr * esize) % 16 == 0) p.has_res_map = 1;
     else p.fast_epi = 0;
   }
+  if (p.sc_blocks && !p.fast_epi) return PGT_ERR_UNSUPPORTED;
   if (p.gn_stats != nullptr) {
     const int cpg = p.N / 32;
     const bool ok = p.fast_epi && p.out_dtype == PGT_BF16 && (p.N % 32) == 0 &&
@@ -983,19 +1063,19 @@
   return true;
 }
 
-template <int BN, bool kVec>
+template <int BN, bool kVec, bool kSc = false>
 static cudaError_t gemm_smem_once() {
   static PerDeviceOnce once;
   return once.run([] {
-    return cudaFuncSetAttribute(gemm_tc_kernel<BN, kVec>, cudaFuncAttributeMaxDynamicSharedMemorySize, GemmCfg<BN>::SMEM_BYTES);
+    return cudaFuncSetAttribute(gemm_tc_kernel<BN, kVec, kSc>, cudaFuncAttributeMaxDynamicSharedMemorySize, GemmCfg<BN>::SMEM_BYTES);
   });
 }
 
-template <int BN, bool kVec>
+template <int BN, bool kVec, bool kSc = false>
 static cudaError_t halo_smem_once() {
   static PerDeviceOnce once;
   return once.run([] {
-    return cudaFuncSetAttribute(conv_halo_kernel<BN, kVec>, cudaFuncAttributeMaxDynamicSharedMemorySize, HaloCfg<BN>::SMEM_BYTES);
+    return cudaFuncSetAttribute(conv_halo_kernel<BN, kVec, kSc>, cudaFuncAttributeMaxDynamicSharedMemorySize, HaloCfg<BN>::SMEM_BYTES);
   });
 }
 
@@ -1007,7 +1087,8 @@
 }
 
 template <int BN>
-static int launch_gemm(const CUtensorMap& tmA, const void* W, int ldw, GemmParams& p, cudaStream_t stream) {
+static int launch_gemm(const CUtensorMap& tmA, const CUtensorMap& tmS, const void* W, int ldw, GemmParams& p,
+                       cudaStream_t stream) {
   using Cfg = GemmCfg<BN>;
   static_assert(Cfg::STAGES >= 3, "pipeline too shallow");
   CUtensorMap tmB, tmO, tmR, tmX;
@@ -1017,7 +1098,8 @@
   if (rc != PGT_OK) return rc;
   p.n_tiles = ceil_div(p.N, BN);
   const bool vec = vector_views(p);
-  PGT_CUDA_OK((vec ? gemm_smem_once<BN, true>() : gemm_smem_once<BN, false>()));
+  if (p.sc_blocks && !vec) return PGT_ERR_UNSUPPORTED;
+  PGT_CUDA_OK((p.sc_blocks ? gemm_smem_once<BN, true, true>() : vec ? gemm_smem_once<BN, true>() : gemm_smem_once<BN, false>()));
   const int tiles = p.m_tiles * p.n_tiles;
   const int grid = tiles < num_sms() ? tiles : num_sms();
   {
@@ -1027,15 +1109,17 @@
       else snprintf(desc, sizeof(desc), "conv%d s%d F%d H%d W%d K%d N%d BN%d t%dx%dx%d e%d", p.ksize, p.mode, p.F, p.H, p.W, p.K, p.N, BN, p.tn, p.th, p.tw, p.fast_epi);
     }
     ProfScope ps(PGT_PROF_GEMM, p.flops, stream, desc);
-    if (vec) gemm_tc_kernel<BN, true><<<grid, GEMM_THREADS, Cfg::SMEM_BYTES, stream>>>(tmA, tmB, tmO, tmR, tmX, p);
-    else gemm_tc_kernel<BN, false><<<grid, GEMM_THREADS, Cfg::SMEM_BYTES, stream>>>(tmA, tmB, tmO, tmR, tmX, p);
+    if (p.sc_blocks) gemm_tc_kernel<BN, true, true><<<grid, GEMM_THREADS, Cfg::SMEM_BYTES, stream>>>(tmA, tmB, tmO, tmR, tmX, tmS, p);
+    else if (vec) gemm_tc_kernel<BN, true><<<grid, GEMM_THREADS, Cfg::SMEM_BYTES, stream>>>(tmA, tmB, tmO, tmR, tmX, tmS, p);
+    else gemm_tc_kernel<BN, false><<<grid, GEMM_THREADS, Cfg::SMEM_BYTES, stream>>>(tmA, tmB, tmO, tmR, tmX, tmS, p);
   }
   PGT_LAUNCH_OK();
   return PGT_OK;
 }
 
 template <int BN>
-static int launch_halo(const CUtensorMap& tmA, const void* W, int ldw, GemmParams& p, cudaStream_t stream) {
+static int launch_halo(const CUtensorMap& tmA, const CUtensorMap& tmS, const void* W, int ldw, GemmParams& p,
+                       cudaStream_t stream) {
   using Cfg = HaloCfg<BN>;
   CUtensorMap tmB, tmO, tmR, tmX;
   int rc = encode_weight_map(&tmB, W, ldw, p.K, p.N, BN);
@@ -1043,9 +1127,10 @@
   rc = setup_epilogue_maps(p, tmA, tmO, tmR, tmX);
   if (rc != PGT_OK) return rc;
   p.n_tiles = ceil_div(p.N, BN);
-  p.b_resident = (p.ntaps * p.cin_blocks <= Cfg::B_STAGES && p.n_tiles == 1) ? 1 : 0;
+  p.b_resident = (p.ntaps * p.cin_blocks + p.sc_blocks <= Cfg::B_STAGES && p.n_tiles == 1) ? 1 : 0;
   const bool vec = vector_views(p);
-  PGT_CUDA_OK((vec ? halo_smem_once<BN, true>() : halo_smem_once<BN, false>()));
+  if (p.sc_blocks && !vec) return PGT_ERR_UNSUPPORTED;
+  PGT_CUDA_OK((p.sc_blocks ? halo_smem_once<BN, true, true>() : vec ? halo_smem_once<BN, true>() : halo_smem_once<BN, false>()));
   const int tiles = p.m_tiles * p.n_tiles;
   const int grid = tiles < num_sms() ? tiles : num_sms();
   {
@@ -1054,8 +1139,9 @@
       snprintf(desc, sizeof(desc), "halo3 F%d H%d W%d K%d N%d BN%d e%d r%d", p.F, p.H, p.W, p.K, p.N, BN, p.fast_epi,
                p.b_resident);
     ProfScope ps(PGT_PROF_GEMM, p.flops, stream, desc);
-    if (vec) conv_halo_kernel<BN, true><<<grid, GEMM_THREADS, Cfg::SMEM_BYTES, stream>>>(tmA, tmB, tmO, tmR, tmX, p);
-    else conv_halo_kernel<BN, false><<<grid, GEMM_THREADS, Cfg::SMEM_BYTES, stream>>>(tmA, tmB, tmO, tmR, tmX, p);
+    if (p.sc_blocks) conv_halo_kernel<BN, true, true><<<grid, GEMM_THREADS, Cfg::SMEM_BYTES, stream>>>(tmA, tmB, tmO, tmR, tmX, tmS, p);
+    else if (vec) conv_halo_kernel<BN, true><<<grid, GEMM_THREADS, Cfg::SMEM_BYTES, stream>>>(tmA, tmB, tmO, tmR, tmX, tmS, p);
+    else conv_halo_kernel<BN, false><<<grid, GEMM_THREADS, Cfg::SMEM_BYTES, stream>>>(tmA, tmB, tmO, tmR, tmX, tmS, p);
   }
   PGT_LAUNCH_OK();
   return PGT_OK;
@@ -1067,10 +1153,11 @@
   return p.m_tiles * ceil_div(p.N, 256) >= num_sms();
 }
 
-static int dispatch_gemm(const CUtensorMap& tmA, const void* W, int ldw, GemmParams& p, cudaStream_t stream) {
-  if (p.N <= 64) return launch_gemm<64>(tmA, W, ldw, p, stream);
-  if (wide_tiles(p)) return launch_gemm<256>(tmA, W, ldw, p, stream);
-  return launch_gemm<128>(tmA, W, ldw, p, stream);
+static int dispatch_gemm(const CUtensorMap& tmA, const CUtensorMap& tmS, const void* W, int ldw, GemmParams& p,
+                         cudaStream_t stream) {
+  if (p.N <= 64) return launch_gemm<64>(tmA, tmS, W, ldw, p, stream);
+  if (wide_tiles(p)) return launch_gemm<256>(tmA, tmS, W, ldw, p, stream);
+  return launch_gemm<128>(tmA, tmS, W, ldw, p, stream);
 }
 
 static int fill_epilogue(GemmParams& p, const pgt_epilogue* ep) {
@@ -1122,7 +1209,7 @@
   uint32_t box[2] = {BK, BM};
   rc = encode_map(&tmA, A, 2, dims, str, box);
   if (rc != PGT_OK) return rc;
-  return dispatch_gemm(tmA, W, ldw, p, static_cast<cudaStream_t>(stream));
+  return dispatch_gemm(tmA, tmA, W, ldw, p, static_cast<cudaStream_t>(stream));
 }
 
 static bool conv_tile_shape(int Hin, int Win, int Cout, int ksize, int stride, int pad_lo, int& tw, int& th) {
@@ -1139,25 +1226,32 @@
   return halo;
 }
 
-static int conv_impl(const void* x, int F, int Hin, int Win, int Cin, int ldx, const void* Wp, int ldw, int Cout,
-                     int ksize, int stride, int pad_y, int pad_x, int up_phase, const pgt_epilogue* ep, void* stream) {
+static int conv_impl(const void* x, int F, int Hin, int Win, int Cin, int ldx, const void* xs, int Cs, int ldxs,
+                     const float* sc_bias, const void* Wp, int ldw, int Cout, int ksize, int stride, int pad_y, int pad_x, int up_phase,
+                     const pgt_epilogue* ep, void* stream) {
   const int pad_lo = pad_y;
   PGT_CHECK_ARG(x && Wp && F > 0 && Hin > 0 && Win > 0 && Cin > 0 && Cout > 0);
   PGT_CHECK_ARG((ksize >= 1 && ksize <= 3) && (stride == 1 || stride == 2) && pad_y >= 0 && pad_y <= 1 && pad_x >= 0 && pad_x <= 1);
   PGT_CHECK_ARG(stride == 1 || (ksize != 2 && pad_x == pad_y));
   PGT_CHECK_ARG((ldx % 8) == 0 && (ldw % 8) == 0 && aligned16(x) && aligned16(Wp) && ldx >= Cin);
+  if (xs != nullptr)
+    PGT_CHECK_ARG(ksize == 3 && stride == 1 && pad_y == 1 && pad_x == 1 && up_phase < 0 && Cs > 0 && (ldxs % 8) == 0 &&
+                  aligned16(xs) && ldxs >= Cs);
   const int cin_pad = ceil_div(Cin, BK) * BK;
-  PGT_CHECK_ARG(ldw >= ksize * ksize * cin_pad);
+  const int cs_pad = xs != nullptr ? ceil_div(Cs, BK) * BK : 0;
+  PGT_CHECK_ARG(ldw >= ksize * ksize * cin_pad + cs_pad);
   GemmParams p{};
   p.N = Cout;
   p.ksize = ksize;
   p.pad_lo = pad_lo;
   p.pad_x = pad_x; p.pad_y = pad_y;
   p.cin_blocks = cin_pad / BK;
-  p.K = ksize * ksize * cin_pad;
-  p.num_kb = ksize * ksize * p.cin_blocks;
+  p.sc_blocks = cs_pad / BK;
+  p.sc_bias = sc_bias;
+  p.K = ksize * ksize * cin_pad + cs_pad;
+  p.num_kb = ksize * ksize * p.cin_blocks + p.sc_blocks;
   p.F = F;
-  CUtensorMap tmA;
+  CUtensorMap tmA, tmS;
   int rc;
   if (stride == 1) {
     p.mode = MODE_CONV_S1;
@@ -1170,6 +1264,9 @@
   }
   rc = fill_epilogue(p, ep);
   if (rc != PGT_OK) return rc;
+  if (xs != nullptr && (p.out_dtype != PGT_BF16 || p.out_layout != PGT_OUT_NHWC || p.epi_mode != PGT_EPI_PLAIN ||
+                        p.residual != nullptr || (Cout % 64) != 0 || (sc_bias != nullptr && !aligned16(sc_bias))))
+    return PGT_ERR_UNSUPPORTED;
   if (up_phase >= 0) {
     if (stride != 1 || p.out_layout != PGT_OUT_NHWC || p.epi_mode != PGT_EPI_PLAIN || p.residual != nullptr)
       return PGT_ERR_UNSUPPORTED;
@@ -1190,7 +1287,7 @@
   p.tiles_y = ceil_div(p.H, th);
   p.m_tiles = p.tiles_x * p.tiles_y * ceil_div(F, tn);
   p.M = F * p.H * p.W;
-  p.flops = 2.0 * p.M * (double)Cout * (ksize * ksize * Cin);
+  p.flops = 2.0 * p.M * (double)Cout * (ksize * ksize * Cin + (xs != nullptr ? Cs : 0));
   if (up_phase >= 0 && p.gn_stats != nullptr) {
     if (tn != 1) return PGT_ERR_UNSUPPORTED;
     const int tpf = p.tiles_x * p.tiles_y;
@@ -1203,9 +1300,15 @@
     uint64_t str[3] = {(uint64_t)ldx * 2, (uint64_t)Win * ldx * 2, (uint64_t)Hin * Win * ldx * 2};
     uint32_t box[4] = {BK, (uint32_t)(halo ? tw + 2 : tw), (uint32_t)(halo ? th + 2 : th), (uint32_t)tn};
     rc = encode_map(&tmA, x, 4, dims, str, box);
+    tmS = tmA;
+    if (rc == PGT_OK && xs != nullptr) {
+      uint64_t sdims[4] = {(uint64_t)Cs, (uint64_t)Win, (uint64_t)Hin, (uint64_t)F};
+      uint64_t sstr[3] = {(uint64_t)ldxs * 2, (uint64_t)Win * ldxs * 2, (uint64_t)Hin * Win * ldxs * 2};
+      rc = encode_map(&tmS, xs, 4, sdims, sstr, box);
+    }
     if (rc == PGT_OK && halo) {
       cudaStream_t st = static_cast<cudaStream_t>(stream);
-      return Cout <= 64 ? launch_halo<64>(tmA, Wp, ldw, p, st) : launch_halo<128>(tmA, Wp, ldw, p, st);
+      return Cout <= 64 ? launch_halo<64>(tmA, tmS, Wp, ldw, p, st) : launch_halo<128>(tmA, tmS, Wp, ldw, p, st);
     }
   } else {
     uint64_t dims[5] = {(uint64_t)2 * ldx, (uint64_t)Win / 2, 2, (uint64_t)Hin / 2, (uint64_t)F};
@@ -1213,13 +1316,14 @@
                        (uint64_t)Hin * Win * ldx * 2};
     uint32_t box[5] = {BK, (uint32_t)tw, 1, (uint32_t)th, (uint32_t)tn};
     rc = encode_map(&tmA, x, 5, dims, str, box);
+    tmS = tmA;
   }
   if (rc != PGT_OK) return rc;
   if (up_phase >= 0) {
     const int esz = p.out_dtype == PGT_BF16 ? 2 : 4;
     if (!aligned16(p.out) || ((long long)p.ldo * esz) % 16 != 0) return PGT_ERR_UNSUPPORTED;
   }
-  return dispatch_gemm(tmA, Wp, ldw, p, static_cast<cudaStream_t>(stream));
+  return dispatch_gemm(tmA, tmS, Wp, ldw, p, static_cast<cudaStream_t>(stream));
 }
 
 extern "C" int pgt_conv_tiles_per_frame(int Hin, int Win, int Cout, int ksize, int stride, int pad_lo) {
@@ -1240,7 +1344,15 @@
 extern "C" int pgt_conv_bf16(const void* x, int F, int Hin, int Win, int Cin, int ldx, const void* Wp, int ldw,
                              int Cout, int ksize, int stride, int pad_lo, const pgt_epilogue* ep, void* stream) {
   PGT_CHECK_ARG(ksize == 1 || ksize == 3);
-  return conv_impl(x, F, Hin, Win, Cin, ldx, Wp, ldw, Cout, ksize, stride, pad_lo, pad_lo, -1, ep, stream);
+  return conv_impl(x, F, Hin, Win, Cin, ldx, nullptr, 0, 0, nullptr, Wp, ldw, Cout, ksize, stride, pad_lo, pad_lo, -1, ep,
+                   stream);
+}
+
+extern "C" int pgt_conv_sc_bf16(const void* x, int F, int Hin, int Win, int Cin, int ldx, const void* xs, int Cs, int ldxs,
+                                const float* bsc, const void* Wp, int ldw, int Cout, const pgt_epilogue* ep,
+                                void* stream) {
+  PGT_CHECK_ARG(xs != nullptr);
+  return conv_impl(x, F, Hin, Win, Cin, ldx, xs, Cs, ldxs, bsc, Wp, ldw, Cout, 3, 1, 1, 1, -1, ep, stream);
 }
 
 extern "C" int pgt_conv_up2x_bf16(const void* x, int F, int Hin, int Win, int Cin, int ldx, const void* Wp4, int ldw,
@@ -1251,7 +1363,7 @@
   for (int ph = 0; ph < 4; ++ph) {
     const int py = ph >> 1, px = ph & 1;
     const void* w = static_cast<const char*>(Wp4) + (size_t)ph * Cout * ldw * 2;
-    int rc = conv_impl(x, F, Hin, Win, Cin, ldx, w, ldw, Cout, 2, 1, 1 - py, 1 - px, ph, ep, stream);
+    int rc = conv_impl(x, F, Hin, Win, Cin, ldx, nullptr, 0, 0, nullptr, w, ldw, Cout, 2, 1, 1 - py, 1 - px, ph, ep, stream);
     if (rc != PGT_OK) return rc;
   }
   return PGT_OK;
diff --git a/pgtformer_b200/engine.py b/pgtformer_b200/engine.py
--- a/pgtformer_b200/engine.py
+++ b/pgtformer_b200/engine.py
@@ -119,6 +119,16 @@
                     wg, bg = fold_layernorm_affine(wf, w[p + '.qkv.bias'], sd[blk + '.norm1.weight'], sd[blk + '.norm1.bias'])
                     w[p + '.qkv_ln.weight'], w[p + '.qkv_ln.bias'] = _pack_lin(wg), bg
         for name in names:
+            if name.endswith('.conv2.weight') and sd[name].dim() == 4 and sd[name].shape[2] == 3 and \
+                    max(sd[name].shape[:2]) > 64:
+                p = name[:-len('.conv2.weight')]
+                sc = next((p + '.' + s for s in ('nin_shortcut', 'conv_out') if (p + '.' + s + '.weight') in sd), None)
+                if sc is None:
+                    continue
+                ws = sd[sc + '.weight'].float().flatten(1)
+                ws = F.pad(ws, (0, (-ws.shape[1]) % 64))
+                w[p + '.conv2_sc.weight'] = torch.cat([_pack_conv(sd[name].float()), ws.to(BF)], 1).contiguous()
+        for name in names:
             if name.endswith('.proj_out.weight'):
                 p = name[:-len('.proj_out.weight')]
                 w[p + '.qkv.weight'] = _pack_lin(torch.cat([sd[p + '.%s.weight' % n] for n in 'qkv'], 0).float())
@@ -183,7 +193,9 @@
         if gn_out:
             stats = self._gn_stats(out, 4 * self._stats_tiles(H, W, cout, kw.get('ksize', 3), stride, kw.get('pad_lo', 1)),
                                    gn_into)
-        return ops.conv(x, self.w[p + '.weight'], cout, out, bias=self.w.get(p + '.bias'), gn_stats=stats, **kw)
+        if 'bias' not in kw:
+            kw['bias'] = self.w.get(p + '.bias')
+        return ops.conv(x, self.w[p + '.weight'], cout, out, gn_stats=stats, **kw)
 
     def _lin(self, x, p, n, out=None, out_dtype=BF, gn_out=False, **kw):
         if out is None:
@@ -195,8 +207,15 @@
 
     def td_resblock(self, x, p, cout, gn_next=False, out=None, shortcut='nin_shortcut'):
         h = self._conv3(x, p + '.conv1', cout, gn=p + '.norm1', gn_out=True)
-        sc = self._lin(x, p + '.' + shortcut, cout) if (p + '.' + shortcut + '.weight') in self.w else x
-        return self._conv3(h, p + '.conv2', cout, gn=p + '.norm2', residual=sc, gn_out=gn_next, out=out)
+        return self._conv2(h, x, p, cout, shortcut, gn_out=gn_next, out=out)
+
+    def _conv2(self, h, x, p, cout, shortcut, **kw):
+        if (p + '.conv2_sc.weight') in self.w:
+            return self._conv3(h, p + '.conv2_sc', cout, gn=p + '.norm2', bias=self.w[p + '.conv2.bias'], shortcut=x,
+                               shortcut_bias=self.w.get(p + '.' + shortcut + '.bias'), **kw)
+        if (p + '.' + shortcut + '.weight') in self.w:
+            x = self._lin(x, p + '.' + shortcut, cout)
+        return self._conv3(h, p + '.conv2', cout, gn=p + '.norm2', residual=x, **kw)
 
     def swin_block(self, x, p, heads, shift, gn_next=False, out=None):
         Fr, H, W, C = x.shape
@@ -256,8 +275,7 @@
         C = dec.shape[-1]
         e = p + '.encode_enc'
         h = self._conv3(cat, e + '.conv1', C, gn=e + '.norm1', gn_out=True)
-        sc = self._lin(cat, e + '.conv_out', C)
-        ef = self._conv3(h, e + '.conv2', C, gn=e + '.norm2', residual=sc)
+        ef = self._conv2(h, cat, e, C, 'conv_out')
         scale = self._conv3(self._conv3(ef, p + '.scale.0', C, act=ops.ACT_LRELU02), p + '.scale.2', C)
         sh = self._conv3(ef, p + '.shift.0', C, act=ops.ACT_LRELU02)
         return self._conv3(sh, p + '.shift.2', C, residual=dec, sft_scale=scale, sft_w=wgt, gn_out=gn_next)
diff --git a/pgtformer_b200/ops.py b/pgtformer_b200/ops.py
--- a/pgtformer_b200/ops.py
+++ b/pgtformer_b200/ops.py
@@ -90,15 +90,23 @@
 
 
 def conv(x, wp, cout, out, ksize=3, stride=1, pad_lo=1, bias=None, act=ACT_NONE, residual=None, sft_scale=None,
-         sft_w=0.0, nchw=False, relu_after_res=False, gn_stats=None):
+         sft_w=0.0, nchw=False, relu_after_res=False, gn_stats=None, shortcut=None, shortcut_bias=None):
     lib = L.load()
     F, H, W, Cin = x.shape
     assert not torch.is_tensor(sft_w) or sft_w.numel() == F
     assert x.dtype == torch.bfloat16 and x.stride(3) == 1 and x.stride(1) == W * x.stride(2) and \
         (F == 1 or x.stride(0) == H * x.stride(1))
     ep = make_epilogue(out, bias, act, residual, sft_scale, sft_w, nchw, relu_after_res, gn_stats)
-    L.check(lib.pgt_conv_bf16(_p(x), F, H, W, Cin, x.stride(2), _p(wp), wp.stride(0), cout, ksize, stride, pad_lo,
-                              ctypes.byref(ep), _stream()))
+    if shortcut is None:
+        L.check(lib.pgt_conv_bf16(_p(x), F, H, W, Cin, x.stride(2), _p(wp), wp.stride(0), cout, ksize, stride, pad_lo,
+                                  ctypes.byref(ep), _stream()))
+        return out
+    xs = shortcut
+    assert (ksize, stride, pad_lo) == (3, 1, 1) and tuple(xs.shape[:3]) == (F, H, W)
+    assert xs.dtype == torch.bfloat16 and xs.stride(3) == 1 and xs.stride(1) == W * xs.stride(2) and \
+        (F == 1 or xs.stride(0) == H * xs.stride(1))
+    L.check(lib.pgt_conv_sc_bf16(_p(x), F, H, W, Cin, x.stride(2), _p(xs), xs.shape[3], xs.stride(2), _p(shortcut_bias),
+                                 _p(wp), wp.stride(0), cout, ctypes.byref(ep), _stream()))
     return out
 
 
```
